# ParaGroup/WindFlow

Measured on NVIDIA H100. Metric: tuples/sec, Map_GPU->Filter_GPU->Ffat_Windows_GPU (CB win 4096 slide 64) pipeline, higher is better.
Workload: dtype i64+f64

## Files before the change

### windflow_b200/csrc/wfb_kernels.cuh

```cuda
#pragma once
#include <type_traits>
#include <cstdint>
#include <cstring>
#include <cuda.h>
#include <cuda_runtime.h>
#include "wfb_ptx.cuh"
#include "wfb_keys.cuh"

namespace wfb {

template <class P> using key_codec = KeyCodec<typename P::key_t>;
template <class P> using key_words_t = typename key_codec<P>::words_t;
template <class P>
__host__ __device__ __forceinline__ key_words_t<P> key_words(const typename P::tuple_t &t, const typename P::params_t &prm)
{
    return key_codec<P>::encode(P::key(t, prm));
}

constexpr int TILE = 256;
constexpr uint32_t OSW_TILE_POS = 4096;
#ifndef WFB_STAGES
#define WFB_STAGES 4
#endif
constexpr int STAGES = WFB_STAGES;
// ... 811 lines not shown
    __shared__ uint32_t cntw[OS_THREADS / 32][256];
    __shared__ uint32_t dig_off[256];
    __shared__ uint32_t bin_base[256];
    __shared__ uint32_t wsum[OS_THREADS / 32];
    __shared__ uint32_t s_tile;
    constexpr int OS_TILE = OS_THREADS * OS_ITEMS;
    __shared__ K skeys[OS_TILE];
    __shared__ uint32_t svals[OS_TILE];

    const uint32_t tid = threadIdx.x, lane = tid & 31, warp = tid >> 5;
    const uint32_t n = n_ptr ? *n_ptr : n_host;
    const uint32_t num_tiles = (n + OS_TILE - 1) / OS_TILE;
    const uint32_t shift = base_shift + 8 * pass;
    if (tid == 0) s_tile = atomicAdd(&ctl[passes * 256 + pass], 1u);
#pragma unroll
    for (int w = 0; w < OS_THREADS / 32; w++) cntw[w][tid] = 0;
    __syncthreads();
    const uint32_t tile = s_tile;
    if (tile >= num_tiles) return;
    const uint32_t start = tile * OS_TILE;

    K k[OS_ITEMS];
    uint32_t rk[OS_ITEMS];
#pragma unroll
    for (int r = 0; r < OS_ITEMS; r++) {
        const uint32_t idx = start + warp * (32 * OS_ITEMS) + r * 32 + lane;
        const bool valid = idx < n;
        k[r] = valid ? keys_in[idx] : K(0);
        const uint32_t d = valid ? (static_cast<uint32_t>(k[r] >> shift) & 255u) : 256u;
        const uint32_t mask = __match_any_sync(FULL, d);
        rk[r] = valid ? (cntw[warp][d] + __popc(mask & lanemask_lt())) : 0u;
        __syncwarp();
        if (valid && lane == static_cast<uint32_t>(__ffs(mask) - 1)) cntw[warp][d] += __popc(mask);
        __syncwarp();
    }
    __syncthreads();

    uint32_t total = 0;
#pragma unroll
    for (int w = 0; w < OS_THREADS / 32; w++) { const uint32_t c = cntw[w][tid]; cntw[w][tid] = total; total += c; }
    uint64_t *my_state = tile_state + static_cast<size_t>(tile) * 256 + tid;
    st_relaxed_u64(my_state, pack_state(epoch, tile == 0 ? ST_PREFIX : ST_AGG, total));
    const uint32_t gcount = ctl[pass * 256 + tid];
    uint32_t incl = gcount;
#pragma unroll
    for (int o = 1; o < 32; o <<= 1) { const uint32_t v = __shfl_up_sync(FULL, incl, o); if (lane >= o) incl += v; }
    if (lane == 31) wsum[warp] = incl;
    uint32_t tincl = total;
#pragma unroll
    for (int o = 1; o < 32; o <<= 1) { const uint32_t v = __shfl_up_sync(FULL, tincl, o); if (lane >= o) tincl += v; }
    __shared__ uint32_t twsum[OS_THREADS / 32];
    if (lane == 31) twsum[warp] = tincl;
    __syncthreads();
    uint32_t gbase = incl - gcount, tbase = tincl - total;
#pragma unroll
    for (uint32_t w = 0; w < OS_THREADS / 32; w++) if (w < warp) { gbase += wsum[w]; tbase += twsum[w]; }
    uint32_t excl = 0;
    if (tile > 0) {
        int64_t t2 = static_cast<int64_t>(tile) - 1;
        bool found = false;
        while (!found) {
            uint64_t w[8];
#pragma unroll
            for (int q = 0; q < 8; q++) w[q] = (t2 - q >= 0) ? ld_relaxed_u64(tile_state + static_cast<size_t>(t2 - q) * 256 + tid) : 0ull;
#pragma unroll
            for (int q = 0; q < 8; q++) {
                if (found || t2 - q < 0) continue;
                if ((w[q] >> 34) != (epoch & 0x3fffffffu) || ((w[q] >> 32) & 3u) == 0) { t2 -= q; goto next_round; }
                excl += static_cast<uint32_t>(w[q]);
                if (((w[q] >> 32) & 3u) == ST_PREFIX) found = true;
            }
            t2 -= 8;
        next_round:;
        }
        st_relaxed_u64(my_state, pack_state(epoch, ST_PREFIX, excl + total));
    }
    dig_off[tid] = tbase;
    bin_base[tid] = gbase + excl;
    __syncthreads();

#pragma unroll
    for (int r = 0; r < OS_ITEMS; r++) {
        const uint32_t idx = start + warp * (32 * OS_ITEMS) + r * 32 + lane;
        if (idx < n) {
            const uint32_t d = static_cast<uint32_t>(k[r] >> shift) & 255u;
            const uint32_t lp = dig_off[d] + cntw[warp][d] + rk[r];
            skeys[lp] = k[r];
            svals[lp] = vals_in ? vals_in[idx] : idx;
        }
    }
    __syncthreads();
    const uint32_t cnt = min(static_cast<uint32_t>(OS_TILE), n - start);
    for (uint32_t i = tid; i < cnt; i += OS_THREADS) {
        const K kk = skeys[i];
        const uint32_t d = static_cast<uint32_t>(kk >> shift) & 255u;
        const uint32_t dst = bin_base[d] + (i - dig_off[d]);
        keys_out[dst] = kk;
        vals_out[dst] = svals[i];
        if (seg_first != nullptr && static_cast<uint64_t>(kk) < seg_first_n) atomicMin(&seg_first[static_cast<uint32_t>(kk)], dst);
    }
}

template <class P>
__global__ void __launch_bounds__(256) k_slots_inplace(const TileArgs a, const typename P::params_t prm)
{
    using T = typename P::tuple_t;
    __shared__ uint32_t s_h[512];
    const uint32_t tid = threadIdx.x;
    const uint32_t npos = a.num_tiles * TILE;
    if (blockIdx.x == 0 && tid == 0 && a.ff.n_trig != nullptr) { *a.ff.n_trig = 0; *a.ff.n_heavy = 0; }
    auto slot_at = [&](uint32_t p) -> uint32_t {
        const uint32_t t = p / TILE;
        uint32_t lo = 0, hi = a.nbatches - 1;
        while (lo < hi) { const uint32_t mid = (lo + hi + 1) >> 1; if (a.batches[mid].tile_begin <= t) lo = mid; else hi = mid - 1; }
        const DevBatch &b = a.batches[lo];
        const uint32_t local = p - b.tile_begin * TILE;
        uint32_t slot = INVALID_SLOT;
        if (local < b.n) {
            if (a.ext_slots != nullptr) { slot = a.ext_slots[p]; if (slot >= a.ff.max_keys) slot = INVALID_SLOT; }
            else {
                const T *rec = reinterpret_cast<const T *>(b.tuples + static_cast<size_t>(local) * sizeof(T));
                slot = slot_of_key(a.ff, key_words<P>(*rec, prm));
            }
            if (slot != INVALID_SLOT && a.count_keys) atomicAdd(&a.ff.seg_cnt[slot], 1u);
        }
        return slot;
    };
    const uint32_t nwide = (npos + OSW_TILE_POS - 1) / OSW_TILE_POS;
    for (uint32_t wt = blockIdx.x; wt < nwide; wt += gridDim.x) {
        for (uint32_t i = tid; i < 512; i += blockDim.x) s_h[i] = 0;
        __syncthreads();
        for (uint32_t p = wt * OSW_TILE_POS + tid; p < min(npos, (wt + 1) * OSW_TILE_POS); p += blockDim.x) {
            uint32_t slot = slot_at(p);
            if (slot != INVALID_SLOT) {
                const uint32_t d = (slot >> a.sort_shift) & 1023u;
                const uint32_t before = atomicAdd(&s_h[d >> 1], 1u << ((d & 1u) * 16u));
                if (a.pack_rank) slot |= ((before >> ((d & 1u) * 16u)) & 0xffffu) << 16;
            }
            a.slots[p] = slot;
        }
        __syncthreads();
        for (uint32_t i = tid; i < 512; i += blockDim.x) reinterpret_cast<uint32_t *>(a.wide_h16 + static_cast<size_t>(wt) * 1024u)[i] = s_h[i];
        __syncthreads();
    }
}

#ifndef WFB_OSW_MINBLOCKS
#define WFB_OSW_MINBLOCKS 5
#endif
constexpr uint32_t OSW_BITS = 10, OSW_DIGITS = 1u << OSW_BITS;
constexpr uint32_t OSW_THREADS = 256, OSW_ITEMS = 16, OSW_TILE = OSW_THREADS * OSW_ITEMS;
static_assert(OSW_TILE == OSW_TILE_POS, "the tile pass files its digit counts per wide tile");
constexpr uint32_t OSR_GROUP = 4, OSR_GROUP_POS = OSR_GROUP * OSW_TILE;

template <class K>
__global__ void __launch_bounds__(OSW_THREADS) k_wide_tile_hist(const K *__restrict__ keys, const uint32_t *__restrict__ n_ptr, uint32_t n_host,
                                                                uint32_t shift, uint32_t chunk_shift, uint16_t *__restrict__ H,
                                                                uint32_t *__restrict__ C, uint32_t *__restrict__ ctl_counts, uint32_t skip_invalid)
{
    static_assert(OSW_THREADS * 4 == OSW_DIGITS, "four digits per thread");
    __shared__ __align__(16) uint32_t h[OSW_DIGITS];
    const uint32_t tid = threadIdx.x, tile = blockIdx.x;
    const uint32_t n = n_ptr ? *n_ptr : n_host;
    const uint32_t start = tile * OSW_TILE;
    if (start >= n) return;
    reinterpret_cast<uint4 *>(h)[tid] = make_uint4(0, 0, 0, 0);
    __syncthreads();
#pragma unroll
    for (uint32_t r = 0; r < OSW_ITEMS; r++) {
        const uint32_t idx = start + r * OSW_THREADS + tid;
        if (idx < n) { const K kk = keys[idx]; if (!(skip_invalid && kk == static_cast<K>(~K(0)))) atomicAdd(&h[static_cast<uint32_t>(kk >> shift) & (OSW_DIGITS - 1u)], 1u); }
    }
    __syncthreads();
    const uint4 c = reinterpret_cast<const uint4 *>(h)[tid];
    reinterpret_cast<ushort4 *>(H + static_cast<size_t>(tile) * OSW_DIGITS)[tid] =
        make_ushort4(static_cast<uint16_t>(c.x), static_cast<uint16_t>(c.y), static_cast<uint16_t>(c.z), static_cast<uint16_t>(c.w));
    uint32_t *crow = C + static_cast<size_t>(tile >> chunk_shift) * OSW_DIGITS + tid * 4;
    if (c.x) atomicAdd(crow + 0, c.x);
    if (c.y) atomicAdd(crow + 1, c.y);
    if (c.z) atomicAdd(crow + 2, c.z);
    if (c.w) atomicAdd(crow + 3, c.w);
    if (ctl_counts != nullptr) {
        if (c.x) atomicAdd(ctl_counts + tid * 4 + 0, c.x);
        if (c.y) atomicAdd(ctl_counts + tid * 4 + 1, c.y);
        if (c.z) atomicAdd(ctl_counts + tid * 4 + 2, c.z);
        if (c.w) atomicAdd(ctl_counts + tid * 4 + 3, c.w);
    }
}

static __global__ void __launch_bounds__(OSW_THREADS) k_wide_chunk_sums16(const uint16_t *__restrict__ H, uint32_t tiles, uint32_t chunk_shift, uint32_t *__restrict__ C,
                                                                          uint32_t *__restrict__ ctl_counts = nullptr)
{
    const uint32_t chunk = blockIdx.x, tid = threadIdx.x;
    const uint32_t t0 = chunk << chunk_shift, t1 = min(tiles, t0 + (1u << chunk_shift));
    uint4 acc = make_uint4(0, 0, 0, 0);
    const ushort4 *row = reinterpret_cast<const ushort4 *>(H) + tid;
#pragma unroll 16
    for (uint32_t t = t0; t < t1; t++) { const ushort4 v = row[static_cast<size_t>(t) * (OSW_DIGITS / 4)]; acc.x += v.x; acc.y += v.y; acc.z += v.z; acc.w += v.w; }
    reinterpret_cast<uint4 *>(C + static_cast<size_t>(chunk) * OSW_DIGITS)[tid] = acc;
    if (ctl_counts != nullptr) {
        if (acc.x) atomicAdd(ctl_counts + tid * 4 + 0, acc.x);
        if (acc.y) atomicAdd(ctl_counts + tid * 4 + 1, acc.y);
        if (acc.z) atomicAdd(ctl_counts + tid * 4 + 2, acc.z);
        if (acc.w) atomicAdd(ctl_counts + tid * 4 + 3, acc.w);
    }
}

static __global__ void __launch_bounds__(OSW_THREADS) k_wide_tile_bases(const uint16_t *__restrict__ H, uint32_t tiles, uint32_t chunk_shift, uint32_t chunks,
                                                                        uint32_t *__restrict__ C, uint32_t *__restrict__ T, uint32_t *__restrict__ ctl_counts,
                                                                        uint32_t *__restrict__ done, uint32_t gshift)
{
    static_assert(OSW_THREADS * 4 == OSW_DIGITS, "four digits per thread");
    constexpr uint32_t NW = OSW_THREADS / 32;
    __shared__ uint32_t wsum[NW];
    __shared__ uint32_t s_last;
    const uint32_t chunk = blockIdx.x, tid = threadIdx.x, lane = tid & 31, warp = tid >> 5;
    const uint32_t t0 = chunk << chunk_shift, t1 = min(tiles, t0 + (1u << chunk_shift));
    uint4 acc = make_uint4(0, 0, 0, 0);
    const ushort4 *row = reinterpret_cast<const ushort4 *>(H) + tid;
    uint4 *trow = reinterpret_cast<uint4 *>(T) + tid;
#pragma unroll 8
    for (uint32_t t = t0; t < t1; t++) {
        const ushort4 v = row[static_cast<size_t>(t) * (OSW_DIGITS / 4)];
        if ((t & ((1u << gshift) - 1u)) == 0) trow[static_cast<size_t>(t >> gshift) * (OSW_DIGITS / 4)] = acc;
        acc.x += v.x; acc.y += v.y; acc.z += v.z; acc.w += v.w;
    }
    uint4 *C4 = reinterpret_cast<uint4 *>(C);
    C4[static_cast<size_t>(chunk) * (OSW_DIGITS / 4) + tid] = acc;
    __threadfence();
    __syncthreads();
    if (tid == 0) s_last = atomicAdd(done, 1u) == chunks - 1u;
    __syncthreads();
    if (!s_last) return;
    __threadfence();
    uint4 tot = make_uint4(0, 0, 0, 0);
#pragma unroll 8
    for (uint32_t c = 0; c < chunks; c++) { const uint4 v = __ldcg(C4 + static_cast<size_t>(c) * (OSW_DIGITS / 4) + tid); tot.x += v.x; tot.y += v.y; tot.z += v.z; tot.w += v.w; }
    reinterpret_cast<uint4 *>(ctl_counts)[tid] = tot;
    const uint32_t sum = tot.x + tot.y + tot.z + tot.w;
    uint32_t incl = sum;
#pragma unroll
    for (int o = 1; o < 32; o <<= 1) { const uint32_t v = __shfl_up_sync(FULL, incl, o); if (lane >= static_cast<uint32_t>(o)) incl += v; }
    if (lane == 31) wsum[warp] = incl;
    __syncthreads();
    uint32_t base = incl - sum;
#pragma unroll
    for (uint32_t q = 0; q < NW; q++) if (q < warp) base += wsum[q];
    uint4 run = make_uint4(base, base + tot.x, base + tot.x + tot.y, base + tot.x + tot.y + tot.z);
#pragma unroll 8
    for (uint32_t c = 0; c < chunks; c++) {
        uint4 *p = C4 + static_cast<size_t>(c) * (OSW_DIGITS / 4) + tid;
        const uint4 v = __ldcg(p);
        *p = run;
        run.x += v.x; run.y += v.y; run.z += v.z; run.w += v.w;
    }
    if (tid == 0) *done = 0;
}

constexpr uint32_t OSR_SMEM = OSR_GROUP_POS * 2u * 2u + OSW_DIGITS * 8u + OSW_DIGITS * 2u;
static_assert(OSR_GROUP == 4 && OSR_GROUP_POS <= 0x8000u, "one ushort4 of part sizes per digit; 16-bit packed position compare");
static __global__ void __launch_bounds__(OSW_THREADS, 3) k_wide_scatter_ranked(const uint32_t *__restrict__ packed, uint32_t *__restrict__ keys_out,
                                                                            uint32_t *__restrict__ vals_out, uint32_t n, uint32_t shift, uint32_t chunk_shift,
                                                                            uint32_t tiles, const uint16_t *__restrict__ H, const uint32_t *__restrict__ Cx,
                                                                            const uint32_t *__restrict__ T)
{
    constexpr uint32_t NW = OSW_THREADS / 32;
    static_assert(OSW_THREADS * 4 == OSW_DIGITS, "four digits per thread");
    extern __shared__ __align__(16) unsigned char osr_smem_buf[];
    uint16_t *lpos = reinterpret_cast<uint16_t *>(osr_smem_buf);
    uint16_t *lslot = lpos + OSR_GROUP_POS;
    ushort4 *part = reinterpret_cast<ushort4 *>(lslot + OSR_GROUP_POS);
    uint16_t *cell = reinterpret_cast<uint16_t *>(part + OSW_DIGITS);
    __shared__ uint32_t wsum[NW];
    __shared__ uint32_t s_total;
    const uint32_t tid = threadIdx.x, lane = tid & 31, warp = tid >> 5, group = blockIdx.x, tile0 = group * OSR_GROUP;
    const uint32_t start = tile0 * OSW_TILE;
    if (start >= n) return;
    {
        ushort4 h[OSR_GROUP];
#pragma unroll
        for (uint32_t k = 0; k < OSR_GROUP; k++)
            h[k] = tile0 + k < tiles ? reinterpret_cast<const ushort4 *>(H)[static_cast<size_t>(tile0 + k) * (OSW_DIGITS / 4) + tid] : make_ushort4(0, 0, 0, 0);
        part[4 * tid + 0] = make_ushort4(h[0].x, h[1].x, h[2].x, h[3].x);
        part[4 * tid + 1] = make_ushort4(h[0].y, h[1].y, h[2].y, h[3].y);
        part[4 * tid + 2] = make_ushort4(h[0].z, h[1].z, h[2].z, h[3].z);
        part[4 * tid + 3] = make_ushort4(h[0].w, h[1].w, h[2].w, h[3].w);
        uint32_t c0 = 0, c1 = 0, c2 = 0, c3 = 0;
#pragma unroll
        for (uint32_t k = 0; k < OSR_GROUP; k++) { c0 += h[k].x; c1 += h[k].y; c2 += h[k].z; c3 += h[k].w; }
        const uint32_t sum = c0 + c1 + c2 + c3;
        uint32_t incl = sum;
#pragma unroll
        for (int o = 1; o < 32; o <<= 1) { const uint32_t v = __shfl_up_sync(FULL, incl, o); if (lane >= static_cast<uint32_t>(o)) incl += v; }
        if (lane == 31) wsum[warp] = incl;
        __syncthreads();
        uint32_t base = incl - sum;
#pragma unroll
        for (uint32_t q = 0; q < NW; q++) if (q < warp) base += wsum[q];
        if (tid == OSW_THREADS - 1) s_total = base + sum;
        reinterpret_cast<ushort4 *>(cell)[tid] = make_ushort4(static_cast<uint16_t>(base), static_cast<uint16_t>(base + c0), static_cast<uint16_t>(base + c0 + c1),
                                                               static_cast<uint16_t>(base + c0 + c1 + c2));
    }
    __syncthreads();
    auto part_start = [&](uint32_t d, uint32_t k, uint32_t *size) {
        const ushort4 p = part[d];
        *size = k == 0 ? p.x : k == 1 ? p.y : k == 2 ? p.z : p.w;
        return (k > 0 ? p.x : 0u) + (k > 1 ? p.y : 0u) + (k > 2 ? p.z : 0u);
    };
#pragma unroll 1
    for (uint32_t k = 0; k < OSR_GROUP; k++) {
        uint32_t w[OSW_ITEMS];
#pragma unroll
        for (uint32_t r = 0; r < OSW_ITEMS; r++) {
            const uint32_t idx = start + k * OSW_TILE + r * OSW_THREADS + tid;
            w[r] = idx < n ? packed[idx] : INVALID_SLOT;
        }
#pragma unroll
        for (uint32_t r = 0; r < OSW_ITEMS; r++)
            if (w[r] != INVALID_SLOT) {
                const uint32_t slot = w[r] & 0xffffu, d = (slot >> shift) & (OSW_DIGITS - 1u);
                uint32_t size;
                const uint32_t i = cell[d] + part_start(d, k, &size) + (w[r] >> 16);
                lpos[i] = static_cast<uint16_t>(k * OSW_TILE + r * OSW_THREADS + tid);
                lslot[i] = static_cast<uint16_t>(slot);
            }
    }
    __syncthreads();
    const uint32_t total = s_total;
    const uint32_t *cbase = Cx + static_cast<size_t>(tile0 >> chunk_shift) * OSW_DIGITS, *tbase = T + static_cast<size_t>(group) * OSW_DIGITS;
#pragma unroll 2
    for (uint32_t e = tid; e < total; e += OSW_THREADS) {
        const uint32_t mine = lpos[e], slot = lslot[e], d = (slot >> shift) & (OSW_DIGITS - 1u);
        uint32_t size;
        const uint32_t before = part_start(d, mine / OSW_TILE, &size);
        uint32_t j = cell[d] + before;
        const uint32_t end = j + size;
        uint32_t less = 0;
        if (j & 1u) { less += lpos[j] < mine ? 1u : 0u; j++; }
        const uint32_t mm = (mine | (mine << 16)) + 0x7fff7fffu;
        for (; j + 1 < end; j += 2) less += __popc((mm - *reinterpret_cast<const uint32_t *>(lpos + j)) & 0x80008000u);
        if (j < end) less += lpos[j] < mine ? 1u : 0u;
        const uint32_t dst = __ldg(cbase + d) + __ldg(tbase + d) + before + less;
        keys_out[dst] = slot;
        vals_out[dst] = start + mine;
    }
}

#ifndef WFB_OSR_MINBLOCKS
#define WFB_OSR_MINBLOCKS 6
#endif
template <int RBYTES>
static __global__ void __launch_bounds__(OSW_THREADS, WFB_OSR_MINBLOCKS) k_wide_scatter_ranked_tile(const uint32_t *__restrict__ packed, uint32_t *__restrict__ keys_out,
                                                                            uint32_t *__restrict__ vals_out, uint32_t n, uint32_t shift, uint32_t chunk_shift,
                                                                            const uint16_t *__restrict__ H, const uint32_t *__restrict__ Cx, const uint32_t *__restrict__ T,
                                                                            const unsigned char *__restrict__ payload_in, unsigned char *__restrict__ payload_out)
{
    constexpr uint32_t NW = OSW_THREADS / 32;
    constexpr uint32_t LPOS = OSW_TILE + OSW_DIGITS;
    constexpr uint32_t LPAD = 0x0fffu;
    static_assert(OSW_TILE <= 4096 && LPOS % (2 * OSW_THREADS) == 0, "16-bit packed position compare");
    __shared__ __align__(16) uint32_t sw[OSW_TILE];
    __shared__ __align__(16) uint32_t bin_base[OSW_DIGITS];
    __shared__ __align__(8) uint16_t cnt_row[OSW_DIGITS], cell_start[OSW_DIGITS];
    __shared__ __align__(4) uint16_t lpos[LPOS];
    __shared__ uint32_t wsum[NW];
    const uint32_t tid = threadIdx.x, lane = tid & 31, warp = tid >> 5, tile = blockIdx.x;
    const uint32_t start = tile * OSW_TILE;
    if (start >= n) return;
#pragma unroll
    for (uint32_t r = 0; r < OSW_ITEMS; r++) {
        const uint32_t i = r * OSW_THREADS + tid, idx = start + i;
        const uint32_t w = idx < n ? packed[idx] : INVALID_SLOT;
        sw[i] = w;
        if constexpr (RBYTES != 0)
            if (w != INVALID_SLOT) asm volatile("prefetch.global.L2 [%0];" ::"l"(payload_in + static_cast<size_t>(idx) * RBYTES));
    }
    {
        const uint4 cb = reinterpret_cast<const uint4 *>(Cx)[static_cast<size_t>(tile >> chunk_shift) * (OSW_DIGITS / 4) + tid];
        const uint4 tb = reinterpret_cast<const uint4 *>(T)[static_cast<size_t>(tile) * (OSW_DIGITS / 4) + tid];
        reinterpret_cast<uint4 *>(bin_base)[tid] = make_uint4(cb.x + tb.x, cb.y + tb.y, cb.z + tb.z, cb.w + tb.w);
        const ushort4 c = reinterpret_cast<const ushort4 *>(H)[static_cast<size_t>(tile) * (OSW_DIGITS / 4) + tid];
        reinterpret_cast<ushort4 *>(cnt_row)[tid] = c;
        const uint32_t p0 = (c.x + 1u) & ~1u, p1 = (c.y + 1u) & ~1u, p2 = (c.z + 1u) & ~1u, p3 = (c.w + 1u) & ~1u;
        const uint32_t sum = p0 + p1 + p2 + p3;
        uint32_t incl = sum;
#pragma unroll
        for (int o = 1; o < 32; o <<= 1) { const uint32_t v = __shfl_up_sync(FULL, incl, o); if (lane >= static_cast<uint32_t>(o)) incl += v; }
        if (lane == 31) wsum[warp] = incl;
#pragma unroll
        for (uint32_t i = 0; i < LPOS / (2 * OSW_THREADS); i++) reinterpret_cast<uint32_t *>(lpos)[i * OSW_THREADS + tid] = LPAD | (LPAD << 16);
        __syncthreads();
        uint32_t base = incl - sum;
#pragma unroll
        for (uint32_t q = 0; q < NW; q++) if (q < warp) base += wsum[q];
        reinterpret_cast<ushort4 *>(cell_start)[tid] = make_ushort4(static_cast<uint16_t>(base), static_cast<uint16_t>(base + p0), static_cast<uint16_t>(base + p0 + p1),
                                                                     static_cast<uint16_t>(base + p0 + p1 + p2));
    }
    __syncthreads();
#pragma unroll
    for (uint32_t r = 0; r < OSW_ITEMS; r++) {
        const uint32_t i = r * OSW_THREADS + tid, w = sw[i];
        if (w != INVALID_SLOT) lpos[cell_start[((w & 0xffffu) >> shift) & (OSW_DIGITS - 1u)] + (w >> 16)] = static_cast<uint16_t>(i);
    }
    __syncthreads();
#pragma unroll 2
    for (uint32_t e = tid; e < LPOS; e += OSW_THREADS) {
        const uint32_t mine = lpos[e], w = sw[mine];
        if (w == INVALID_SLOT) continue;
        const uint32_t slot = w & 0xffffu, d = (slot >> shift) & (OSW_DIGITS - 1u);
        const uint32_t cs = cell_start[d], cnt = cnt_row[d];
        if (e - cs >= cnt) continue;
        const uint32_t mm = (mine | (mine << 16)) + 0x7fff7fffu;
        const uint32_t *cell = reinterpret_cast<const uint32_t *>(lpos + cs);
        uint32_t less = 0;
        for (uint32_t j = 0; j < cnt; j += 2) less += __popc((mm - cell[j >> 1]) & 0x80008000u);
        const uint32_t dst = bin_base[d] + less;
        keys_out[dst] = slot;
        if (RBYTES == 0 || vals_out != nullptr) vals_out[dst] = start + mine;
        if constexpr (RBYTES != 0) {
            static_assert(RBYTES % 8 == 0, "record size");
            using W = typename std::conditional<RBYTES % 16 == 0, uint4, uint2>::type;
            const W *src = reinterpret_cast<const W *>(payload_in + static_cast<size_t>(start + mine) * RBYTES);
            W *dstp = reinterpret_cast<W *>(payload_out + static_cast<size_t>(dst) * RBYTES);
            W v[RBYTES / sizeof(W)];
#pragma unroll
            for (uint32_t q = 0; q < RBYTES / sizeof(W); q++) v[q] = src[q];
#pragma unroll
            for (uint32_t q = 0; q < RBYTES / sizeof(W); q++) dstp[q] = v[q];
        }
    }
}

static __global__ void k_shard_bin_counts(const uint32_t *__restrict__ bin_counts, uint32_t nshards, uint32_t bps, uint32_t *__restrict__ counts_out,
                                          uint64_t *__restrict__ send_meta, uint64_t watermark)
{
    const uint32_t d = threadIdx.x >> 5, lane = threadIdx.x & 31;
    uint32_t c = 0;
    if (d < nshards) for (uint32_t b = lane; b < bps; b += 32) c += bin_counts[d * bps + b];
#pragma unroll
    for (int o = 16; o > 0; o >>= 1) c += __shfl_xor_sync(FULL, c, o);
    if (lane == 0 && d < MAX_SHARDS) counts_out[d] = d < nshards ? c : 0u;
    if (lane == 0 && d < nshards && send_meta != nullptr) { send_meta[2 * d] = c; send_meta[2 * d + 1] = watermark; }
}

struct MgRuns { uint32_t off[MAX_SHARDS + 1]; };
constexpr uint32_t MG_THREADS = 256;
__device__ __forceinline__ uint32_t mg_run_start(const uint32_t *__restrict__ cnt, uint32_t s, uint32_t bps, uint32_t b, uint32_t *sh)
{
    uint32_t c = 0;
    for (uint32_t q = threadIdx.x; q < b; q += MG_THREADS) c += cnt[s * bps + q];
#pragma unroll
    for (int o = 16; o > 0; o >>= 1) c += __shfl_xor_sync(FULL, c, o);
    if ((threadIdx.x & 31) == 0) sh[threadIdx.x >> 5] = c;
    __syncthreads();
    uint32_t t = 0;
#pragma unroll
    for (uint32_t w = 0; w < MG_THREADS / 32; w++) t += sh[w];
    __syncthreads();
    return t;
}
static __global__ void __launch_bounds__(MG_THREADS) k_mg_count(const uint32_t *__restrict__ cnt, uint32_t nsrc, uint32_t bps, const MgRuns runs,
                                                                const uint32_t *__restrict__ recv_slots, uint32_t slot_mask, uint32_t shift2, uint32_t nsub,
                                                                uint32_t *__restrict__ cnt3, uint32_t *__restrict__ run_starts,
                                                                uint32_t *__restrict__ n_trig, uint32_t *__restrict__ n_heavy)
{
    __shared__ uint32_t sh[8], c[MAX_SHARDS];
    const uint32_t b = blockIdx.x, s = blockIdx.y, tid = threadIdx.x, lane = tid & 31;
    if (b == 0 && s == 0 && tid == 0) { *n_trig = 0; *n_heavy = 0; }
    if (tid < MAX_SHARDS) c[tid] = 0;
    const uint32_t rs = mg_run_start(cnt, s, bps, b, sh), m = cnt[s * bps + b];
    if (tid == 0) run_starts[s * bps + b] = rs;
    const uint32_t *sl = recv_slots + runs.off[s] + rs;
    for (uint32_t i0 = 0; i0 < m; i0 += MG_THREADS) {
        const uint32_t i = i0 + tid;
        const uint32_t j = i < m ? ((sl[i] & slot_mask) >> shift2) & (nsub - 1u) : nsub;
        for (uint32_t jj = 0; jj < nsub; jj++) { const uint32_t bal = __ballot_sync(FULL, j == jj); if (lane == 0 && bal) atomicAdd(&c[jj], __popc(bal)); }
    }
    __syncthreads();
    if (tid < nsub) cnt3[(b * nsub + tid) * nsrc + s] = c[tid];
}
static __global__ void __launch_bounds__(1024) k_mg_scan(const uint32_t *__restrict__ cnt3, uint32_t n, uint32_t nsrc, uint32_t *__restrict__ off3,
                                                         uint32_t *__restrict__ digit_counts)
{
    __shared__ uint32_t wsum[32];
    const uint32_t tid = threadIdx.x, lane = tid & 31, warp = tid >> 5;
    const uint32_t per = (n + 1023u) / 1024u, lo = tid * per;
    uint32_t v[MAX_SHARDS], sum = 0;
#pragma unroll
    for (uint32_t q = 0; q < MAX_SHARDS; q++) { v[q] = (q < per && lo + q < n) ? cnt3[lo + q] : 0u; sum += v[q]; }
    uint32_t incl = sum;
#pragma unroll
    for (int o = 1; o < 32; o <<= 1) { const uint32_t x = __shfl_up_sync(FULL, incl, o); if (lane >= static_cast<uint32_t>(o)) incl += x; }
    if (lane == 31) wsum[warp] = incl;
    __syncthreads();
    if (warp == 0) {
        uint32_t w = wsum[lane], wi = w;
#pragma unroll
        for (int o = 1; o < 32; o <<= 1) { const uint32_t x = __shfl_up_sync(FULL, wi, o); if (lane >= static_cast<uint32_t>(o)) wi += x; }
        wsum[lane] = wi - w;
    }
    __syncthreads();
    uint32_t run = wsum[warp] + incl - sum;
#pragma unroll
    for (uint32_t q = 0; q < MAX_SHARDS; q++) if (q < per && lo + q < n) { off3[lo + q] = run; run += v[q]; }
    for (uint32_t d = tid; d * nsrc < n; d += 1024) { uint32_t t = 0; for (uint32_t q = 0; q < nsrc; q++) t += cnt3[d * nsrc + q]; digit_counts[d] = t; }
}
static __global__ void __launch_bounds__(MG_THREADS) k_mg_split(const uint32_t *__restrict__ cnt, uint32_t nsrc, uint32_t bps, const MgRuns runs,
                                                                const uint32_t *__restrict__ recv_slots, uint32_t slot_mask, uint32_t shift2, uint32_t nsub,
                                                                const uint32_t *__restrict__ off3, const uint32_t *__restrict__ run_starts,
                                                                uint32_t *__restrict__ out_slots, uint32_t *__restrict__ out_pos)
{
    __shared__ uint32_t wc[MG_THREADS / 32][MAX_SHARDS], fill[MAX_SHARDS];
    const uint32_t b = blockIdx.x, s = blockIdx.y, tid = threadIdx.x, lane = tid & 31, warp = tid >> 5;
    const uint32_t m = cnt[s * bps + b], src0 = runs.off[s] + run_starts[s * bps + b];
    if (tid < nsub) fill[tid] = off3[(b * nsub + tid) * nsrc + s];
    __syncthreads();
    for (uint32_t i0 = 0; i0 < m; i0 += MG_THREADS) {
        const uint32_t i = i0 + tid;
        uint32_t slot = 0, j = nsub, before = 0;
        if (i < m) { slot = recv_slots[src0 + i] & slot_mask; j = (slot >> shift2) & (nsub - 1u); }
        for (uint32_t jj = 0; jj < nsub; jj++) {
            const uint32_t bal = __ballot_sync(FULL, j == jj);
            if (lane == 0) wc[warp][jj] = __popc(bal);
            if (j == jj) before = __popc(bal & lanemask_lt());
        }
        __syncthreads();
        if (i < m) {
            uint32_t dst = fill[j] + before;
            for (uint32_t w = 0; w < warp; w++) dst += wc[w][j];
            out_slots[dst] = slot; out_pos[dst] = src0 + i;
        }
        __syncthreads();
        if (tid < nsub) { uint32_t t = 0; for (uint32_t w = 0; w < MG_THREADS / 32; w++) t += wc[w][tid]; fill[tid] += t; }
        __syncthreads();
    }
}

template <class K, int RBYTES>
__global__ void __launch_bounds__(OSW_THREADS, WFB_OSW_MINBLOCKS) k_wide_scatter(const K *__restrict__ keys_in, K *__restrict__ keys_out, uint32_t *__restrict__ vals_out,
                                                              const uint32_t *__restrict__ n_ptr, uint32_t n_host, uint32_t shift,
                                                              uint32_t chunk_shift, const uint16_t *__restrict__ H, const uint32_t *__restrict__ C,
                                                              const uint32_t *__restrict__ ctl_counts,
                                                              const unsigned char *__restrict__ payload_in, unsigned char *__restrict__ payload_out,
                                                              uint32_t payload_bytes, uint32_t skip_invalid, uint32_t region_stride)
{
    constexpr uint32_t NW = OSW_THREADS / 32;
    __shared__ __align__(16) uint16_t cntw[NW][OSW_DIGITS];
    __shared__ uint32_t bin_base[OSW_DIGITS];
    __shared__ uint32_t wsum[NW];
    const uint32_t tid = threadIdx.x, lane = tid & 31, warp = tid >> 5, tile = blockIdx.x;
    const uint32_t n = n_ptr ? *n_ptr : n_host;
    const uint32_t start = tile * OSW_TILE;
    if (start >= n) return;
    {
        uint4 *z = reinterpret_cast<uint4 *>(&cntw[0][0]);
        for (uint32_t i = tid; i < NW * OSW_DIGITS / 8; i += OSW_THREADS) z[i] = make_uint4(0, 0, 0, 0);
    }
    uint32_t acc[4] = {0, 0, 0, 0};
    {
        const uint32_t chunk = tile >> chunk_shift;
        const uint4 *crow = reinterpret_cast<const uint4 *>(C) + tid;
#pragma unroll 8
        for (uint32_t c = 0; c < chunk; c++) { const uint4 v = crow[static_cast<size_t>(c) * (OSW_DIGITS / 4)]; acc[0] += v.x; acc[1] += v.y; acc[2] += v.z; acc[3] += v.w; }
        const ushort4 *hrow = reinterpret_cast<const ushort4 *>(H) + tid;
#pragma unroll 16
        for (uint32_t t = chunk << chunk_shift; t < tile; t++) { const ushort4 v = hrow[static_cast<size_t>(t) * (OSW_DIGITS / 4)]; acc[0] += v.x; acc[1] += v.y; acc[2] += v.z; acc[3] += v.w; }
    }
    const uint4 g4 = reinterpret_cast<const uint4 *>(ctl_counts)[tid];
    const uint32_t gsum = g4.x + g4.y + g4.z + g4.w;
    uint32_t incl = gsum;
#pragma unroll
    for (int o = 1; o < 32; o <<= 1) { const uint32_t v = __shfl_up_sync(FULL, incl, o); if (lane >= static_cast<uint32_t>(o)) incl += v; }
    if (lane == 31) wsum[warp] = incl;
    __syncthreads();

    K k[OSW_ITEMS];
    uint32_t rk[OSW_ITEMS];
#pragma unroll
    for (uint32_t r = 0; r < OSW_ITEMS; r++) {
        const uint32_t idx = start + warp * (32 * OSW_ITEMS) + r * 32 + lane;
        k[r] = idx < n ? keys_in[idx] : K(0);
    }
#pragma unroll
    for (uint32_t r = 0; r < OSW_ITEMS; r++) {
        const uint32_t idx = start + warp * (32 * OSW_ITEMS) + r * 32 + lane;
        const bool valid = idx < n && !(skip_invalid && k[r] == static_cast<K>(~K(0)));
        rk[r] = 0xffffffffu;
        if (!__any_sync(FULL, valid)) continue;
        const uint32_t d = valid ? (static_cast<uint32_t>(k[r] >> shift) & (OSW_DIGITS - 1u)) : OSW_DIGITS + lane;
        const uint32_t mask = __match_any_sync(FULL, d);
        const uint32_t leader = static_cast<uint32_t>(__ffs(mask) - 1);
        uint32_t before = 0;
        if (valid && lane == leader) { before = cntw[warp][d]; cntw[warp][d] = static_cast<uint16_t>(before + __popc(mask)); }
        before = __shfl_sync(FULL, before, leader);
        if (valid) rk[r] = before + __popc(mask & lanemask_lt());
        __syncwarp();
    }
    __syncthreads();
    {
        uint32_t gb = incl - gsum;
#pragma unroll
        for (uint32_t w = 0; w < NW; w++) if (w < warp) gb += wsum[w];
        uint32_t run[4] = {0, 0, 0, 0};
#pragma unroll
        for (uint32_t w = 0; w < NW; w++) {
            ushort4 *row = reinterpret_cast<ushort4 *>(&cntw[w][0]);
            const ushort4 c = row[tid];
            row[tid] = make_ushort4(static_cast<uint16_t>(run[0]), static_cast<uint16_t>(run[1]), static_cast<uint16_t>(run[2]), static_cast<uint16_t>(run[3]));
            run[0] += c.x; run[1] += c.y; run[2] += c.z; run[3] += c.w;
        }
        const uint32_t gc[4] = {g4.x, g4.y, g4.z, g4.w};
#pragma unroll
        for (int q = 0; q < 4; q++) { bin_base[tid * 4 + q] = (region_stride ? (tid * 4 + q) * region_stride : gb) + acc[q]; gb += gc[q]; }
    }
    __syncthreads();
#pragma unroll
    for (uint32_t r = 0; r < OSW_ITEMS; r++) {
        const uint32_t idx = start + warp * (32 * OSW_ITEMS) + r * 32 + lane;
        if (rk[r] != 0xffffffffu) {
            const uint32_t d = static_cast<uint32_t>(k[r] >> shift) & (OSW_DIGITS - 1u);
            const uint32_t dst = bin_base[d] + cntw[warp][d] + rk[r];
            if (region_stride && dst - d * region_stride >= region_stride) { rk[r] = 0xffffffffu; continue; }
            if (keys_out != nullptr) keys_out[dst] = k[r];
            if (vals_out != nullptr) vals_out[dst] = idx;
            rk[r] = dst;
        }
    }
    if constexpr (RBYTES > 0) {
        using V = typename std::conditional<RBYTES % 16 == 0, uint4, uint2>::type;
        constexpr uint32_t NV = RBYTES / sizeof(V);
#pragma unroll
        for (uint32_t r = 0; r < OSW_ITEMS; r++) {
            const uint32_t idx = start + warp * (32 * OSW_ITEMS) + r * 32 + lane;
            if (rk[r] != 0xffffffffu) {
                const V *src = reinterpret_cast<const V *>(payload_in + static_cast<size_t>(idx) * RBYTES);
                V *dstp = reinterpret_cast<V *>(payload_out + static_cast<size_t>(rk[r]) * RBYTES);
                V tmp[NV];
#pragma unroll
                for (uint32_t q = 0; q < NV; q++) tmp[q] = src[q];
#pragma unroll
                for (uint32_t q = 0; q < NV; q++) dstp[q] = tmp[q];
            }
        }
    } else if constexpr (RBYTES < 0) {
#pragma unroll 1
        for (uint32_t r = 0; r < OSW_ITEMS; r++) {
            const uint32_t idx = start + warp * (32 * OSW_ITEMS) + r * 32 + lane;
            if (rk[r] != 0xffffffffu) {
                const uint64_t *src = reinterpret_cast<const uint64_t *>(payload_in + static_cast<size_t>(idx) * payload_bytes);
                uint64_t *dstp = reinterpret_cast<uint64_t *>(payload_out + static_cast<size_t>(rk[r]) * payload_bytes);
                for (uint32_t q = 0; q < payload_bytes / 8; q++) dstp[q] = src[q];
            }
        }
    }
}

template <int RBYTES>
__global__ void __launch_bounds__(OSW_THREADS) k_shard_scatter(const uint32_t *__restrict__ dest, uint32_t n, uint32_t nbins, uint32_t chunk_shift,
                                                               const uint16_t *__restrict__ H, const uint32_t *__restrict__ C,
                                                               const unsigned char *__restrict__ payload_in, unsigned char *__restrict__ payload_out,
                                                               uint32_t region_stride)
{
    constexpr uint32_t NW = OSW_THREADS / 32;
    __shared__ uint32_t base[32];
    __shared__ uint32_t wtot[NW][32];
    const uint32_t tid = threadIdx.x, lane = tid & 31, warp = tid >> 5, tile = blockIdx.x;
    const uint32_t start = tile * OSW_TILE;
    if (start >= n) return;
    if (tid < 32) {
        uint32_t acc = 0;
        if (tid < nbins) {
            const uint32_t chunk = tile >> chunk_shift;
            for (uint32_t c = 0; c < chunk; c++) acc += C[static_cast<size_t>(c) * OSW_DIGITS + tid];
            for (uint32_t t = chunk << chunk_shift; t < tile; t++) acc += H[static_cast<size_t>(t) * OSW_DIGITS + tid];
        }
        base[tid] = tid * region_stride + acc;
    }
    uint32_t running = 0;
    uint16_t code[OSW_ITEMS];
#pragma unroll
    for (uint32_t r = 0; r < OSW_ITEMS; r++) {
        const uint32_t idx = start + warp * (32 * OSW_ITEMS) + r * 32 + lane;
        const uint32_t d = idx < n ? dest[idx] : INVALID_SLOT;
// ... 75 lines not shown
    if (d < MAX_SHARDS) counts_out[d] = c;
    const uint32_t over = __ballot_sync(FULL, c > region_cap);
    if (d == 0) counts_out[MAX_SHARDS] = over ? 1u : 0u;
}


__device__ __forceinline__ uint32_t level_off(uint32_t n_leaves, uint32_t level);
__device__ __forceinline__ uint64_t batch_watermark(const uint32_t *__restrict__ batch_off, const DevBatch *__restrict__ batches,
                                                    uint32_t nbatches, uint32_t pos);
template <class P>
__device__ __forceinline__ void ffat_eval_window(const FfatDev &ff, const unsigned char *tree, key_words_t<P> key, uint64_t gwid, uint64_t wm,
                                                 uint32_t opos, unsigned char *__restrict__ out_res, uint64_t *__restrict__ out_ts,
                                                 uint32_t out_cap, const typename P::params_t &prm);

template <class P>
__global__ void __launch_bounds__(128) k_ffat_update_lanes(const FfatDev ff, const unsigned char *__restrict__ lifted,
                                                           const uint32_t *__restrict__ sorted_pos,
                                                           const uint32_t *__restrict__ batch_off, const DevBatch *__restrict__ batches,
                                                           uint32_t nbatches, unsigned char *__restrict__ out_res,
                                                           uint64_t *__restrict__ out_ts, uint32_t out_cap, uint32_t *__restrict__ n_out,
                                                           const typename P::params_t prm)
{
    using R = typename P::result_t;
    constexpr uint32_t RB = sizeof(R);
    constexpr uint32_t U = 4;
    const uint32_t nslots = ff.dense ? ff.max_keys : min(*ff.n_slots, ff.max_keys);
    const uint32_t n = ff.n_leaves, logn = ff.log_leaves;
    const uint64_t P_ = ff.pane;
    const uint64_t group_items = ff.slide * ff.nb;
    const size_t tree_stride = static_cast<size_t>(2 * n - 1) * RB;

    for (uint32_t base = blockIdx.x * blockDim.x; base < nslots; base += gridDim.x * blockDim.x) {
        const uint32_t slot = base + threadIdx.x;
        uint32_t m = (slot < nslots) ? ff.seg_cnt[slot] : 0u;
        if (m > ff.light_max) {
            const uint32_t hi = atomicAdd(ff.n_heavy, 1u);
            if (hi < ff.max_keys) ff.heavy[hi] = slot;
            m = 0;
        }
        const bool act = m > 0;
        uint32_t off = 0; uint64_t c = 0, g = 0, trig = 0;
        key_words_t<P> key{};
        alignas(16) R acc;
        unsigned char *tree = ff.tree + static_cast<size_t>(slot) * tree_stride;
        if (act) {
            off = ff.seg_off[slot]; c = ff.cnt[slot];
            key = key_of_slot<P>(ff, slot);
            if (c % P_ != 0) ld_rec<R>(ff.acc + static_cast<size_t>(slot) * RB, acc);
            g = (c < ff.B) ? 0 : 1 + (c - ff.B) / group_items;
            trig = ff.B + g * group_items;
        }
        uint32_t j = 0;
        while (__any_sync(FULL, act && j < m)) {
            bool completed = false;
            while (act && j < m && !completed) {
                uint32_t p[U];
                alignas(16) R it[U];
                const uint32_t k = min(U, m - j);
#pragma unroll
                for (uint32_t q = 0; q < U; q++) if (q < k) p[q] = sorted_pos[off + j + q];
#pragma unroll
                for (uint32_t q = 0; q < U; q++) if (q < k) ld_rec<R>(lifted + static_cast<size_t>(p[q]) * RB, it[q]);
#pragma unroll
                for (uint32_t q = 0; q < U; q++) {
                    if (q < k && !completed) {
                        if (c % P_ == 0) acc = it[q]; else P::comb(acc, it[q], acc, prm);
                        c++; j++;
                        completed = (c % P_ == 0);
                    }
                }
            }
            if (completed) {
                const uint32_t leaf = static_cast<uint32_t>((c / P_ - 1) & (n - 1));
                const uint32_t plev = ff.lazy ? 0u : logn;
                for (uint32_t l = 0; l < plev; l++)
                    asm volatile("prefetch.global.L2 [%0];" ::"l"(tree + static_cast<size_t>(level_off(n, l) + ((leaf >> l) ^ 1u)) * RB));
                alignas(16) R cur = acc;
                st_rec<R>(tree + static_cast<size_t>(leaf) * RB, cur);
                for (uint32_t l = 0; l < plev; l++) {
                    alignas(16) R s;
                    ld_rec<R>(tree + static_cast<size_t>(level_off(n, l) + ((leaf >> l) ^ 1u)) * RB, s);
                    alignas(16) R parent = cur;
                    if ((leaf >> l) & 1u) P::comb(s, cur, parent, prm); else P::comb(cur, s, parent, prm);
                    cur = parent;
                    st_rec<R>(tree + static_cast<size_t>(level_off(n, l + 1) + (leaf >> (l + 1))) * RB, cur);
                }
                if (c == trig) {
                    const uint32_t last_pos = sorted_pos[off + j - 1];
                    const uint32_t obase = atomicAdd(n_out, ff.nb);
                    bool deferred = (m - j) < ff.defer_items;
                    if (deferred) {
                        const uint32_t ti = atomicAdd(ff.n_trig, 1u);
                        if (ti < ff.trig_cap) { Trigger tr; tr.key = trig_word(key); tr.g = g; tr.slot = slot; tr.last_pos = last_pos; tr.obase = obase; tr.pad = 0; ff.trig[ti] = tr; }
                        else deferred = false;
                    }
                    if (!deferred) {
                        const uint64_t wm = batch_watermark(batch_off, batches, nbatches, last_pos);
                        for (uint32_t i = 0; i < ff.nb; i++)
                            ffat_eval_window<P>(ff, tree, key, g * ff.nb + i, wm, obase + i, out_res, out_ts, out_cap, prm);
                    }
                    g++; trig += group_items;
                }
            }
        }
        if (act) {
            ff.cnt[slot] = c;
            if (c % P_ != 0) st_rec<R>(ff.acc + static_cast<size_t>(slot) * RB, acc);
            ff.seg_cnt[slot] = 0;
            ff.seg_off[slot] = 0xffffffffu;
        }
    }
}

#ifdef WFB_BK_TRACE
__device__ unsigned long long g_bk_trace[1024 * 8];
__device__ __forceinline__ unsigned long long bk_now() { unsigned long long t; asm volatile("mov.u64 %0, %%globaltimer;" : "=l"(t)); return t; }
#define BK_TRACE_STATE unsigned long long bk_t = 0
#define BK_MARK(i) do { if (threadIdx.x == 0) { const unsigned long long t_ = bk_now(); unsigned long long *r_ = g_bk_trace + blockIdx.x * 8; \
    if ((i) == 0) { r_[0] = t_; for (int q_ = 1; q_ < 8; q_++) r_[q_] = 0; } else if ((i) == 7) r_[7] = t_; else r_[i] += t_ - bk_t; bk_t = t_; } } while (0)
#else
#define BK_TRACE_STATE do { } while (0)
#define BK_MARK(i) do { } while (0)
#endif
constexpr uint32_t BK_KEYS = 64;
constexpr uint32_t BK_THREADS = 128;
#ifndef WFB_BK_REC_BYTES
#define WFB_BK_REC_BYTES 16384
#endif
constexpr uint32_t BK_REC_BYTES = WFB_BK_REC_BYTES;
constexpr uint32_t BK_CNT_U = 16;
__device__ __forceinline__ uint32_t bk_opaque(uint32_t v) { asm volatile("" : "+r"(v)); return v; }
template <uint32_t RB>
constexpr uint32_t bk_items_per_thread() { return BK_REC_BYTES / (BK_THREADS * RB) < 1 ? 1 : (BK_REC_BYTES / (BK_THREADS * RB) > 8 ? 8 : BK_REC_BYTES / (BK_THREADS * RB)); }
template <uint32_t RB>
constexpr uint32_t bk_sibl_levels() { return RB <= 32 ? 8 : (RB <= 48 ? 4 : (RB <= 128 ? 2 : 1)); }
template <uint32_t RB, bool LAZY>
constexpr uint32_t bk_smem_bytes()
{
    constexpr uint32_t IT = bk_items_per_thread<RB>(), CAP = BK_THREADS * IT, CS = IT * (BK_THREADS / 32) + 2;
    return CAP * RB + 3 * CAP * 4 + BK_KEYS * CS * 2 + 5 * BK_KEYS * 4 + 3 * BK_KEYS * 8 + BK_KEYS * RB
         + (LAZY ? 16 : BK_KEYS * bk_sibl_levels<RB>() * RB) + 2 * BK_KEYS * 4 + BK_THREADS * 4 + (BK_THREADS / 32 + 5) * 4 + 64;
}
template <uint32_t RB>
constexpr bool bk_fits() { return bk_smem_bytes<RB, false>() <= (48u << 10) && bk_smem_bytes<RB, true>() <= (48u << 10); }
#ifndef WFB_BK_MINBLOCKS
#define WFB_BK_MINBLOCKS 4
#endif
#ifndef WFB_BK_MINBLOCKS_LAZY
#define WFB_BK_MINBLOCKS_LAZY 4
#endif

template <class P, bool LAZY>
__global__ void __launch_bounds__(BK_THREADS, LAZY ? WFB_BK_MINBLOCKS_LAZY : WFB_BK_MINBLOCKS) k_ffat_update_buckets(const FfatDev ff, const unsigned char *__restrict__ lifted,
                                                                       const uint32_t *__restrict__ bk_slots, const uint32_t *__restrict__ bk_pos,
                                                                       const uint32_t *__restrict__ digit_counts, uint32_t shift, uint32_t moved,
                                                                       const uint32_t *__restrict__ batch_off, const DevBatch *__restrict__ batches,
                                                                       uint32_t nbatches, unsigned char *__restrict__ out_res,
                                                                       uint64_t *__restrict__ out_ts, uint32_t out_cap, uint32_t *__restrict__ n_out,
                                                                       const typename P::params_t prm)
{
    using R = typename P::result_t;
    constexpr uint32_t RB = sizeof(R);
    constexpr uint32_t NW = BK_THREADS / 32;
    constexpr uint32_t DPT = OSW_DIGITS / BK_THREADS;
    constexpr uint32_t IT = bk_items_per_thread<RB>();
    constexpr uint32_t CAP = BK_THREADS * IT;
    constexpr uint32_t NCOL = IT * NW;
    constexpr uint32_t CS = NCOL + 2;
    constexpr uint32_t CPB = (RB % 16 == 0) ? 16 : 8;
    constexpr uint32_t BK_SIBL = bk_sibl_levels<RB>();
    static_assert(DPT % 4 == 0 && BK_KEYS == 64 && BK_THREADS == 128 && RB % 8 == 0, "layout");
    static_assert(bk_fits<RB>(), "the arrays below exceed 48 KB of static shared memory (bk_smem_bytes)");
    __shared__ __align__(16) unsigned char s_rec[CAP * RB];
    __shared__ uint32_t s_idx[CAP];
    __shared__ uint32_t s_lslot[CAP], s_lpos[CAP];
    __shared__ __align__(16) uint16_t s_col[BK_KEYS][CS];
    __shared__ uint32_t kcnt[BK_KEYS], koff[BK_KEYS];
    __shared__ uint32_t kleft[BK_KEYS];
    __shared__ uint32_t kcp[BK_KEYS], kleaf[BK_KEYS];
    __shared__ uint64_t kc[BK_KEYS], kg[BK_KEYS], ktt[BK_KEYS];
    __shared__ __align__(16) unsigned char kacc[BK_KEYS * RB];
    __shared__ __align__(16) unsigned char s_sib[LAZY ? 16 : BK_KEYS * BK_SIBL * RB];
    __shared__ uint32_t s_heavy[BK_KEYS];
    __shared__ uint32_t ksegb[BK_KEYS];
    __shared__ uint32_t seg_desc[BK_THREADS];
    __shared__ uint32_t misc[NW], s_boff[2], s_nheavy, s_hnext, s_nseg;

    const uint32_t tid = threadIdx.x, lane = tid & 31, warp = tid >> 5;
    const uint32_t bucket = blockIdx.x;
    const uint32_t kpc = min(BK_KEYS, 1u << shift);
    const uint32_t key_lo = bucket << shift;
    const uint32_t n = ff.n_leaves, logn = ff.log_leaves;
    const uint32_t P32 = static_cast<uint32_t>(ff.pane);
    const uint64_t group_items = ff.slide * ff.nb;
    const size_t tree_stride = static_cast<size_t>(2 * n - 1) * RB;
    BK_TRACE_STATE;

    BK_MARK(0);
    uint32_t my_total = 0;
    uint64_t st_c = 0;
    const bool has_key = tid < kpc && key_lo + tid < ff.max_keys;
    if (has_key) {
        const uint32_t slot = key_lo + tid;
        st_c = ff.cnt[slot];
#pragma unroll
        for (uint32_t q = 0; q < RB / CPB; q++) cp_async<CPB>(kacc + tid * RB + q * CPB, ff.acc + static_cast<size_t>(slot) * RB + q * CPB);
    }
    if (tid < BK_KEYS) kleft[tid] = 0;
    {
        uint32_t cc[DPT];
#pragma unroll
        for (uint32_t q = 0; q < DPT / 4; q++) {
            const uint4 v = reinterpret_cast<const uint4 *>(digit_counts)[tid * (DPT / 4) + q];
            cc[4 * q] = v.x; cc[4 * q + 1] = v.y; cc[4 * q + 2] = v.z; cc[4 * q + 3] = v.w;
        }
        uint32_t sum = 0;
#pragma unroll
        for (uint32_t q = 0; q < DPT; q++) sum += cc[q];
        uint32_t incl = sum;
#pragma unroll
        for (int o = 1; o < 32; o <<= 1) { const uint32_t v = __shfl_up_sync(FULL, incl, o); if (lane >= static_cast<uint32_t>(o)) incl += v; }
        if (lane == 31) misc[warp] = incl;
        __syncthreads();
        if (tid == bucket / DPT) {
            uint32_t base = incl - sum;
            for (uint32_t w = 0; w < warp; w++) base += misc[w];
            for (uint32_t q = bucket - bucket % DPT; q < bucket; q++) base += digit_counts[q];
            s_boff[0] = base; s_boff[1] = base + digit_counts[bucket];
        }
        __syncthreads();
    }
    const uint32_t bbeg = s_boff[0], bend = s_boff[1];
    const auto fetch_list = [&](uint32_t at, uint32_t end) {
#pragma unroll
        for (uint32_t r = 0; r < IT; r++) {
            const uint32_t i = r * BK_THREADS + tid;
            if (at + i < end) {
                cp_async<4>(s_lslot + i, bk_slots + at + i);
                if (!moved) cp_async<4>(s_lpos + i, bk_pos + at + i);
            }
        }
    };
    fetch_list(bbeg, bend);
    for (uint32_t base = bbeg; base < bend; base += BK_CNT_U * BK_THREADS) {
        uint32_t lk[BK_CNT_U];
#pragma unroll
        for (uint32_t q = 0; q < BK_CNT_U; q++) {
            const uint32_t i = base + q * BK_THREADS + tid;
            lk[q] = i < bend ? bk_slots[i] - key_lo : 0xffffffffu;
        }
#pragma unroll
        for (uint32_t q = 0; q < BK_CNT_U; q++) if (lk[q] < kpc) atomicAdd(&kleft[lk[q]], 1u);
    }
    __syncthreads();
    if (tid < BK_KEYS) {
        const uint32_t m = has_key ? kleft[tid] : 0u;
        my_total = m;
        const uint64_t c = st_c;
        uint64_t g = 0, tt = 0; uint32_t cp = 0, leaf = 0;
        if (m) {
            cp = static_cast<uint32_t>(c % P32); leaf = static_cast<uint32_t>((c / P32) & (n - 1));
            if (c < ff.B) { g = 0; tt = ff.B - c; }
            else { g = 1 + (c - ff.B) / group_items; tt = ff.B + g * group_items - c; }
        }
        kleft[tid] = m; kc[tid] = c; kg[tid] = g; ktt[tid] = tt; kcp[tid] = cp; kleaf[tid] = leaf;
    }
    const uint32_t any_items = __syncthreads_or(my_total != 0);
    BK_MARK(1);
    if (!any_items) { cp_async_wait_all(); BK_MARK(7); return; }
    if (moved)
        for (size_t o = static_cast<size_t>(tid) * 128; o < static_cast<size_t>(bend - bbeg) * RB; o += BK_THREADS * 128)
            asm volatile("prefetch.global.L2 [%0];" ::"l"(lifted + static_cast<size_t>(bbeg) * RB + o));

    for (uint32_t cursor = s_boff[0]; cursor < s_boff[1]; cursor = s_boff[0]) {
        const uint32_t nsel = min(CAP, s_boff[1] - cursor);
        uint32_t ek[IT], ep[IT];
        cp_async_wait_all();
#pragma unroll
        for (uint32_t r = 0; r < IT; r++) {
            const uint32_t i = r * BK_THREADS + tid;
            ek[r] = BK_KEYS; ep[r] = cursor + i;
            if (i < nsel) {
                const uint32_t lk = s_lslot[i] - key_lo;
                if (!moved) ep[r] = s_lpos[i];
                if (lk < kpc) ek[r] = lk;
            }
        }
        {
            uint32_t *z = reinterpret_cast<uint32_t *>(&s_col[0][0]);
            for (uint32_t i = tid; i < BK_KEYS * CS / 2; i += BK_THREADS) z[i] = 0;
        }
        __syncthreads();
        fetch_list(cursor + CAP, s_boff[1]);
#pragma unroll
        for (uint32_t r = 0; r < IT; r++) {
            const uint32_t k = ek[r];
            const uint32_t peers = __match_any_sync(FULL, k);
            const uint32_t rank = __popc(peers & lanemask_lt());
            if (k < BK_KEYS && rank == 0) s_col[k][r * NW + warp] = static_cast<uint16_t>(__popc(peers));
            ek[r] = k | rank << 8;
        }
        __syncthreads();
        BK_MARK(2);
        if (warp == 0) {
            uint32_t a0 = 0, a1 = 0;
#pragma unroll
            for (uint32_t c = 0; c < NCOL; c++) {
                const uint32_t v0 = s_col[lane][c], v1 = s_col[lane + 32][c];
                s_col[lane][c] = static_cast<uint16_t>(a0); s_col[lane + 32][c] = static_cast<uint16_t>(a1);
                a0 += v0; a1 += v1;
            }
            uint32_t i0 = a0, i1 = a1;
#pragma unroll
            for (int o = 1; o < 32; o <<= 1) {
                const uint32_t v0 = __shfl_up_sync(FULL, i0, o), v1 = __shfl_up_sync(FULL, i1, o);
                if (lane >= static_cast<uint32_t>(o)) { i0 += v0; i1 += v1; }
            }
            const uint32_t t0 = __shfl_sync(FULL, i0, 31);
            kcnt[lane] = a0; kcnt[lane + 32] = a1;
            koff[lane] = i0 - a0; koff[lane + 32] = t0 + i1 - a1;
            const uint32_t c0 = kcp[lane], c1 = kcp[lane + 32];
            const uint32_t f0 = min(a0, P32 - c0), f1 = min(a1, P32 - c1);
            const uint32_t n0 = a0 ? 1u + (a0 - f0 + P32 - 1) / P32 : 0u, n1 = a1 ? 1u + (a1 - f1 + P32 - 1) / P32 : 0u;
            uint32_t s0 = n0, s1 = n1;
#pragma unroll
            for (int o = 1; o < 32; o <<= 1) {
                const uint32_t v0 = __shfl_up_sync(FULL, s0, o), v1 = __shfl_up_sync(FULL, s1, o);
                if (lane >= static_cast<uint32_t>(o)) { s0 += v0; s1 += v1; }
            }
            const uint32_t st0 = __shfl_sync(FULL, s0, 31), nseg = st0 + __shfl_sync(FULL, s1, 31);
            ksegb[lane] = s0 - n0; ksegb[lane + 32] = st0 + s1 - n1;
            const bool fallback = nseg > BK_THREADS;
            const bool h0 = fallback && a0 != 0, h1 = fallback && a1 != 0;
            const uint32_t b0 = __ballot_sync(FULL, h0), b1 = __ballot_sync(FULL, h1);
            if (h0) s_heavy[__popc(b0 & lanemask_lt())] = lane;
            if (h1) s_heavy[__popc(b0) + __popc(b1 & lanemask_lt())] = lane + 32;
            if (lane == 0) { s_nheavy = __popc(b0) + __popc(b1); s_hnext = 0; s_nseg = fallback ? 0u : nseg; }
        }
        __syncthreads();
#pragma unroll
        for (uint32_t r = 0; r < IT; r++) {
            const uint32_t k = ek[r] & 255u;
            if (k < BK_KEYS) {
                const uint32_t at = koff[k] + s_col[k][r * NW + warp] + (ek[r] >> 8);
                s_idx[at] = ep[r];
                const unsigned char *src = lifted + static_cast<size_t>(ep[r]) * RB;
#pragma unroll
                for (uint32_t q = 0; q < RB / CPB; q++) {
                    if constexpr (CPB == 16) cp_async_cg16(s_rec + at * RB + q * CPB, src + q * CPB);
                    else cp_async<CPB>(s_rec + at * RB + q * CPB, src + q * CPB);
                }
            }
        }
        const uint32_t nseg = s_nseg;
        bool sib_staged = false;
        if (tid < BK_KEYS && nseg != 0) {
            const uint32_t m = kcnt[tid];
            if (m != 0) {
                const uint32_t cp0 = kcp[tid], first = min(m, P32 - cp0), ns = 1u + (m - first + P32 - 1) / P32, sb = ksegb[tid];
                for (uint32_t j = 0; j < ns; j++) seg_desc[sb + j] = tid | (j << 8);
                if (!LAZY && cp0 + first == P32) {
                    const uint32_t leaf = kleaf[tid];
                    const unsigned char *tr = ff.tree + static_cast<size_t>(key_lo + tid) * tree_stride;
                    for (uint32_t l = 0; l < min(logn, BK_SIBL); l++) {
                        const unsigned char *src = tr + static_cast<size_t>(level_off(n, l) + ((leaf >> l) ^ 1u)) * RB;
                        unsigned char *dst = s_sib + (tid * BK_SIBL + l) * RB;
#pragma unroll
                        for (uint32_t q = 0; q < RB / CPB; q++) cp_async<CPB>(dst + q * CPB, src + q * CPB);
                    }
                    sib_staged = true;
                }
            }
        }
        cp_async_wait_all();
        __syncthreads();
        BK_MARK(3);
        if (tid < nseg) {
            const uint32_t d = seg_desc[tid], k = d & 255u, j = d >> 8;
            const uint32_t m = kcnt[k], cp0 = kcp[k], first = min(m, P32 - cp0);
            const uint32_t start = j == 0 ? 0u : first + (j - 1) * P32;
            const uint32_t seg = j == 0 ? first : min(P32, m - start);
            unsigned char *rp = s_rec + (koff[k] + start) * RB;
            alignas(16) R acc;
            uint32_t i = 1;
            if (j == 0 && cp0 != 0) { ld_rec<R>(kacc + k * RB, acc); i = 0; }
            else ld_rec<R>(rp, acc);
#pragma unroll 4
            for (; i < seg; i++) { alignas(16) R it; ld_rec<R>(rp + i * RB, it); P::comb(acc, it, acc, prm); }
            st_rec<R>(rp, acc);
        }
        __syncthreads();
        BK_MARK(4);
        if (tid < BK_KEYS && nseg != 0) {
            const uint32_t k = bk_opaque(tid), m = kcnt[k];
            const uint32_t cp0 = kcp[k];
            uint32_t leafi = kleaf[k], new_cp = cp0, consumed = 0;
            uint64_t g = kg[k], tt = ktt[k];
            while (__any_sync(FULL, consumed < m)) {
                bool eval_now = false;
                uint32_t ev_obase = 0, ev_pos = 0;
                uint64_t ev_g = 0;
                if (consumed < m) {
                    const uint32_t open = consumed == 0 ? cp0 : 0u;
                    const uint32_t len = min(m - consumed, P32 - open);
                    alignas(16) R cur;
                    ld_rec<R>(s_rec + (koff[k] + consumed) * RB, cur);
                    consumed += len;
                    const bool completes = open + len == P32;
                    if (!completes) { st_rec<R>(kacc + k * RB, cur); new_cp = open + len; }
                    else {
                        new_cp = 0;
                        const uint32_t slot = key_lo + k, leaf = leafi;
                        unsigned char *tree = ff.tree + static_cast<size_t>(slot) * tree_stride;
                        leafi = (leafi + 1) & (n - 1);
                        st_rec<R>(tree + static_cast<size_t>(leaf) * RB, cur);
                        for (uint32_t l0 = 0; l0 < (LAZY ? 0u : logn); l0 += 4) {
                            alignas(16) R sbl[4];
#pragma unroll
                            for (uint32_t q = 0; q < 4; q++) {
                                const uint32_t l = l0 + q;
                                if (l < logn) {
                                    if (sib_staged && l < BK_SIBL) ld_rec<R>(s_sib + (k * BK_SIBL + l) * RB, sbl[q]);
                                    else ld_rec<R>(tree + static_cast<size_t>(level_off(n, l) + ((leaf >> l) ^ 1u)) * RB, sbl[q]);
                                }
                            }
#pragma unroll
                            for (uint32_t q = 0; q < 4; q++) {
                                const uint32_t l = l0 + q;
                                if (l < logn) {
                                    alignas(16) R parent = cur;
                                    if ((leaf >> l) & 1u) P::comb(sbl[q], cur, parent, prm); else P::comb(cur, sbl[q], parent, prm);
                                    cur = parent;
                                    st_rec<R>(tree + static_cast<size_t>(level_off(n, l + 1) + (leaf >> (l + 1))) * RB, cur);
                                }
                            }
                        }
                        sib_staged = false;
                        if (consumed == tt) {
                            const uint32_t lp = s_idx[koff[k] + consumed - 1];
                            const uint32_t last_pos = moved ? bk_pos[lp] : lp;
                            const uint32_t obase = atomicAdd(n_out, ff.nb);
                            bool deferred = (kleft[k] - consumed) < ff.defer_items;
                            if (deferred) {
                                const uint32_t ti = atomicAdd(ff.n_trig, 1u);
                                if (ti < ff.trig_cap) { Trigger tr; tr.key = trig_word(key_of_slot<P>(ff, slot)); tr.g = g; tr.slot = slot; tr.last_pos = last_pos; tr.obase = obase; tr.pad = 0; ff.trig[ti] = tr; }
                                else deferred = false;
                            }
                            if (!deferred) { eval_now = true; ev_obase = obase; ev_pos = last_pos; ev_g = g; }
                            g++; tt += group_items;
                        }
                    }
                }
                uint32_t pend = __ballot_sync(FULL, eval_now);
                while (pend) {
                    const int src = __ffs(pend) - 1;
                    pend &= pend - 1;
                    const uint32_t e_slot = key_lo + (warp << 5) + src, e_obase = __shfl_sync(FULL, ev_obase, src), e_pos = __shfl_sync(FULL, ev_pos, src);
                    const key_words_t<P> e_key = key_of_slot<P>(ff, e_slot);
                    const uint64_t e_g = __shfl_sync(FULL, ev_g, src);
                    const unsigned char *e_tree = ff.tree + static_cast<size_t>(e_slot) * tree_stride;
                    const uint64_t wm = batch_watermark(batch_off, batches, nbatches, e_pos);
                    for (uint32_t i = lane; i < ff.nb; i += 32)
                        ffat_eval_window<P>(ff, e_tree, e_key, e_g * ff.nb + i, wm, e_obase + i, out_res, out_ts, out_cap, prm);
                }
                __syncwarp();
            }
            if (m != 0) { kc[k] += m; kg[k] = g; ktt[k] = tt - m; kcp[k] = new_cp; kleaf[k] = leafi; kleft[k] -= m; }
        }
        BK_MARK(5);
        if (s_nheavy != 0) {
            __syncthreads();
            for (;;) {
                uint32_t h = 0;
                if (lane == 0) h = atomicAdd(&s_hnext, 1u);
                h = __shfl_sync(FULL, h, 0);
                if (h >= s_nheavy) break;
                const uint32_t k = s_heavy[h];
                const uint32_t m = kcnt[k], off = koff[k], slot = key_lo + k;
                uint64_t g = kg[k], tt = ktt[k];
                uint32_t cp = kcp[k], leafi = kleaf[k], left = kleft[k];
                unsigned char *tree = ff.tree + static_cast<size_t>(slot) * tree_stride;
                alignas(16) R acc;
                if (cp) ld_rec<R>(kacc + k * RB, acc);
                uint32_t j = 0;
                while (j < m) {
                    const uint32_t cnt = min(32u, m - j);
                    alignas(16) R cur_rec;
                    if (lane < cnt) ld_rec<R>(s_rec + (off + j + lane) * RB, cur_rec);
                    uint32_t lo = 0;
                    while (lo < cnt) {
                        const uint32_t hi = min(cnt, lo + (P32 - cp));
                        alignas(16) R r = cur_rec;
#pragma unroll
                        for (uint32_t o = 1; o < 32; o <<= 1) {
                            const R other = shfl_down_rec<R>(r, o);
                            if (lane >= lo && lane + o < hi) P::comb(r, other, r, prm);
                        }
                        r = shfl_rec<R>(r, lo);
                        if (cp == 0) acc = r; else P::comb(acc, r, acc, prm);
                        const uint32_t take = hi - lo;
                        cp += take; left -= take; tt -= take;
                        if (cp == P32) {
                            cp = 0;
                            const uint32_t leaf = leafi;
                            leafi = (leafi + 1) & (n - 1);
                            alignas(16) R sib;
                            const uint32_t plev = LAZY ? 0u : logn;
                            if (lane < plev) ld_rec<R>(tree + static_cast<size_t>(level_off(n, lane) + ((leaf >> lane) ^ 1u)) * RB, sib);
                            alignas(16) R cur = acc;
                            if (lane == 0) st_rec<R>(tree + static_cast<size_t>(leaf) * RB, cur);
                            for (uint32_t l = 0; l < plev; l++) {
                                const R sb = shfl_rec<R>(sib, l);
                                alignas(16) R parent = cur;
                                if ((leaf >> l) & 1u) P::comb(sb, cur, parent, prm); else P::comb(cur, sb, parent, prm);
                                cur = parent;
                                if (lane == 0) st_rec<R>(tree + static_cast<size_t>(level_off(n, l + 1) + (leaf >> (l + 1))) * RB, cur);
                            }
                            __syncwarp();
                            if (tt == 0) {
                                const uint32_t last_pos = moved ? bk_pos[s_idx[off + j + hi - 1]] : s_idx[off + j + hi - 1];
                                uint32_t obase = 0;
                                if (lane == 0) obase = atomicAdd(n_out, ff.nb);
                                obase = __shfl_sync(FULL, obase, 0);
                                bool deferred = left < ff.defer_items;
                                if (deferred) {
                                    uint32_t ti = 0;
                                    if (lane == 0) ti = atomicAdd(ff.n_trig, 1u);
                                    ti = __shfl_sync(FULL, ti, 0);
                                    if (ti < ff.trig_cap) {
                                        if (lane == 0) { Trigger tr; tr.key = trig_word(key_of_slot<P>(ff, slot)); tr.g = g; tr.slot = slot; tr.last_pos = last_pos; tr.obase = obase; tr.pad = 0; ff.trig[ti] = tr; }
                                    } else deferred = false;
                                }
                                if (!deferred) {
                                    const uint64_t wm = batch_watermark(batch_off, batches, nbatches, last_pos);
                                    const key_words_t<P> key = key_of_slot<P>(ff, slot);
                                    for (uint32_t i = lane; i < ff.nb; i += 32)
                                        ffat_eval_window<P>(ff, tree, key, g * ff.nb + i, wm, obase + i, out_res, out_ts, out_cap, prm);
                                }
                                g++; tt = group_items;
                                __syncwarp();
                            }
                        }
                        lo = hi;
                    }
                    j += cnt;
                }
                if (lane == 0) {
                    kc[k] += m; kg[k] = g; ktt[k] = tt; kcp[k] = cp; kleaf[k] = leafi; kleft[k] = left;
                    if (cp) st_rec<R>(kacc + k * RB, acc);
                }
            }
        }
        if (tid == 0) s_boff[0] += CAP;
        __syncthreads();
        BK_MARK(6);
    }
    if (tid < kpc && key_lo + tid < ff.max_keys) {
        const uint32_t k = bk_opaque(tid), slot = key_lo + k;
        ff.cnt[slot] = kc[k];
        if (kcp[k]) { alignas(16) R a; ld_rec<R>(kacc + k * RB, a); st_rec<R>(ff.acc + static_cast<size_t>(slot) * RB, a); }
    }
    BK_MARK(7);
}

__device__ __forceinline__ uint32_t level_off(uint32_t n_leaves, uint32_t level) { return 2u * n_leaves - ((2u * n_leaves) >> level); }

__device__ __forceinline__ uint64_t batch_watermark(const uint32_t *__restrict__ batch_off, const DevBatch *__restrict__ batches,
                                                    uint32_t nbatches, uint32_t pos)
{
    uint32_t lo = 0, hi = nbatches - 1;
    while (lo < hi) { const uint32_t mid = (lo + hi + 1) >> 1; if (batch_off[mid] <= pos) lo = mid; else hi = mid - 1; }
    return batches[lo].watermark;
}

template <class P>
__device__ __forceinline__ void ffat_eval_window(const FfatDev &ff, const unsigned char *tree, key_words_t<P> key, uint64_t gwid, uint64_t wm,
                                                 uint32_t opos, unsigned char *__restrict__ out_res, uint64_t *__restrict__ out_ts,
                                                 uint32_t out_cap, const typename P::params_t &prm)
{
    using R = typename P::result_t;
    constexpr uint32_t RB = sizeof(R);
    const uint32_t n = ff.n_leaves;
    alignas(16) R res = P::make_result(key_codec<P>::decode(key), gwid, prm);
    uint32_t ws = static_cast<uint32_t>((gwid * ff.sp) & (n - 1));
    uint32_t remaining = ff.wp;
    if (ff.lazy) {
        for (; remaining > 0; remaining--) {
            alignas(16) R node;
            ld_rec<R>(tree + static_cast<size_t>(ws) * RB, node);
            P::comb(res, node, res, prm);
            ws = (ws + 1) & (n - 1);
        }
    }
    while (remaining > 0) {
        uint32_t range = (ws == 0) ? n : (ws & (0u - ws));
        const uint32_t pw = 1u << (31 - __clz(remaining));
        range = min(range, pw);
        const uint32_t level = 31 - __clz(range);
        alignas(16) R node;
        ld_rec<R>(tree + static_cast<size_t>(level_off(n, level) + (ws >> level)) * RB, node);
        P::comb(res, node, res, prm);
        ws = (ws + range) & (n - 1);
        remaining -= range;
    }
    if (opos < out_cap) {
        st_rec<R>(out_res + static_cast<size_t>(opos) * RB, res);
        if (out_ts != nullptr) out_ts[opos] = wm;
    } else atomicOr(ff.err_flags, 2u);
}

template <class P>
__global__ void __launch_bounds__(256) k_ffat_windows(const FfatDev ff, const uint32_t *__restrict__ batch_off,
                                                      const DevBatch *__restrict__ batches, uint32_t nbatches,
                                                      unsigned char *__restrict__ out_res, uint64_t *__restrict__ out_ts, uint32_t out_cap,
                                                      const typename P::params_t prm, uint32_t *__restrict__ n_out)
{
    using R = typename P::result_t;
    if (blockIdx.x == 0 && threadIdx.x == 0 && n_out != nullptr) {
        if (*n_out > out_cap) { *n_out = out_cap; atomicOr(ff.err_flags, 2u); }
        if (ff.results_total != nullptr) *ff.results_total += *n_out;
    }
    const uint32_t nt = min(*ff.n_trig, ff.trig_cap);
    const uint64_t total = static_cast<uint64_t>(nt) * ff.nb;
    const size_t tree_stride = static_cast<size_t>(2 * ff.n_leaves - 1) * sizeof(R);
    for (uint64_t w = blockIdx.x * static_cast<uint64_t>(blockDim.x) + threadIdx.x; w < total; w += static_cast<uint64_t>(gridDim.x) * blockDim.x) {
        const uint32_t ti = static_cast<uint32_t>(w / ff.nb), i = static_cast<uint32_t>(w % ff.nb);
        const Trigger tr = ff.trig[ti];
        const uint64_t wm = batch_watermark(batch_off, batches, nbatches, tr.last_pos);
        ffat_eval_window<P>(ff, ff.tree + static_cast<size_t>(tr.slot) * tree_stride, trig_key<P>(ff, tr), tr.g * ff.nb + i, wm, tr.obase + i,
                            out_res, out_ts, out_cap, prm);
    }
}

template <class P>
__global__ void __launch_bounds__(128) k_ffat_windows_lazy(const FfatDev ff, const uint32_t *__restrict__ batch_off,
                                                           const DevBatch *__restrict__ batches, uint32_t nbatches,
                                                           unsigned char *__restrict__ out_res, uint64_t *__restrict__ out_ts, uint32_t out_cap,
                                                           const typename P::params_t prm, uint32_t *__restrict__ n_out)
{
    using R = typename P::result_t;
    constexpr uint32_t RB = sizeof(R);
    extern __shared__ __align__(16) unsigned char lazy_smem[];
    if (blockIdx.x == 0 && threadIdx.x == 0 && n_out != nullptr) {
        if (*n_out > out_cap) { *n_out = out_cap; atomicOr(ff.err_flags, 2u); }
        if (ff.results_total != nullptr) *ff.results_total += *n_out;
    }
    const uint32_t lane = threadIdx.x & 31, warp = threadIdx.x >> 5, wpb = blockDim.x >> 5;
    const uint32_t n = ff.n_leaves, logn = ff.log_leaves;
    unsigned char *t = lazy_smem + static_cast<size_t>(warp) * 2u * n * RB;
    const uint32_t nt = min(*ff.n_trig, ff.trig_cap);
    const size_t tree_stride = static_cast<size_t>(2 * n - 1) * RB;
    FfatDev fs = ff; fs.lazy = 0;
    for (uint32_t ti = blockIdx.x * wpb + warp; ti < nt; ti += gridDim.x * wpb) {
        const Trigger tr = ff.trig[ti];
        const unsigned char *leaves = ff.tree + static_cast<size_t>(tr.slot) * tree_stride;
        for (uint32_t i = lane; i < n * (RB / 8); i += 32) reinterpret_cast<uint64_t *>(t)[i] = reinterpret_cast<const uint64_t *>(leaves)[i];
        __syncwarp();
        for (uint32_t l = 0; l < logn; l++) {
            const unsigned char *src = t + static_cast<size_t>(level_off(n, l)) * RB;
            unsigned char *dst = t + static_cast<size_t>(level_off(n, l + 1)) * RB;
            for (uint32_t i = lane; i < (n >> (l + 1)); i += 32) {
                alignas(16) R a, b, o;
                ld_rec<R>(src + static_cast<size_t>(2 * i) * RB, a); ld_rec<R>(src + static_cast<size_t>(2 * i + 1) * RB, b);
                o = a;
                P::comb(a, b, o, prm);
                st_rec<R>(dst + static_cast<size_t>(i) * RB, o);
            }
            __syncwarp();
        }
        const uint64_t wm = batch_watermark(batch_off, batches, nbatches, tr.last_pos);
        for (uint32_t i = lane; i < ff.nb; i += 32)
            ffat_eval_window<P>(fs, t, trig_key<P>(ff, tr), tr.g * ff.nb + i, wm, tr.obase + i, out_res, out_ts, out_cap, prm);
        __syncwarp();
// ... 972 lines not shown
```

### windflow_b200/csrc/wfb_launch.cuh

```cuda
#pragma once
#include <type_traits>
#include <algorithm>
#include <cstring>
#include <cuda.h>
#include <cuda_runtime.h>
#include "../../include/wfb200.h"
#include "wfb_kernels.cuh"

#define WFB_CK(call) do { cudaError_t e__ = (call); if (e__ != cudaSuccess) return static_cast<int>(e__); } while (0)

namespace wfb {

inline int num_sms()
{
    static int n = 0;
    if (n == 0) { int dev = 0; if (cudaGetDevice(&dev) == cudaSuccess) cudaDeviceGetAttribute(&n, cudaDevAttrMultiProcessorCount, dev); }
    return n;
}


typedef CUresult (*PFN_encodeTiled)(CUtensorMap *, CUtensorMapDataType, cuuint32_t, void *, const cuuint64_t *, const cuuint64_t *,
                                    const cuuint32_t *, const cuuint32_t *, CUtensorMapInterleave, CUtensorMapSwizzle,
                                    CUtensorMapL2promotion, CUtensorMapFloatOOBfill);
inline PFN_encodeTiled get_encode_tiled()
{
    static PFN_encodeTiled fn = nullptr;
    static bool tried = false;
    if (!tried) {
        tried = true;
        void *p = nullptr;
        cudaDriverEntryPointQueryResult q;
        if (cudaGetDriverEntryPoint("cuTensorMapEncodeTiled", &p, cudaEnableDefault, &q) == cudaSuccess && q == cudaDriverEntryPointSuccess)
            fn = reinterpret_cast<PFN_encodeTiled>(p);
        cudaGetLastError();
    }
    return fn;
}

inline bool make_tuple_tmap(CUtensorMap *m, uint64_t base, uint64_t end)
{
    std::memset(m, 0, sizeof(*m));
    PFN_encodeTiled enc = get_encode_tiled();
    if (!enc || (base & 63u) || end <= base) return false;
    const uint64_t rows = (end - base) / 64;
    if (rows == 0 || rows > 0xffffffffull) return false;
    cuuint64_t gdim[2] = {64, rows};
    cuuint64_t gstr[1] = {64};
    cuuint32_t box[2] = {64, TILE};
    cuuint32_t estr[2] = {1, 1};
    return enc(m, CU_TENSOR_MAP_DATA_TYPE_UINT8, 2, reinterpret_cast<void *>(base), gdim, gstr, box, estr, CU_TENSOR_MAP_INTERLEAVE_NONE,
               CU_TENSOR_MAP_SWIZZLE_64B, CU_TENSOR_MAP_L2_PROMOTION_L2_128B, CU_TENSOR_MAP_FLOAT_OOB_FILL_NONE) == CUDA_SUCCESS;
}

struct ProgramOps {
    uint32_t tuple_bytes, result_bytes, params_bytes, reserved;
    int (*tile_pass)(int mode, TileArgs &a, const void *params, uint32_t want_grid, cudaStream_t s, uint32_t *grid_used,
                     uint64_t span_begin, uint64_t span_end);
    int (*ffat_update)(const FfatDev &ff, const unsigned char *lifted, const uint32_t *sorted_pos, const uint32_t *batch_off,
                       const DevBatch *batches, uint32_t nbatches, unsigned char *out_res, uint64_t *out_ts,
                       uint32_t out_cap, uint32_t *n_out, uint32_t grid, cudaStream_t s, const void *params, uint32_t lanes_grid);
    int (*ffat_buckets)(const FfatDev &ff, const unsigned char *lifted, const uint32_t *bk_slots, const uint32_t *bk_pos,
                        const uint32_t *digit_counts, uint32_t shift, uint32_t moved, const uint32_t *batch_off, const DevBatch *batches,
                        uint32_t nbatches, unsigned char *out_res, uint64_t *out_ts, uint32_t out_cap, uint32_t *n_out, cudaStream_t s,
                        const void *params);
    int (*ffat_windows)(const FfatDev &ff, const uint32_t *batch_off, const DevBatch *batches, uint32_t nbatches,
                        unsigned char *out_res, uint64_t *out_ts, uint32_t out_cap, uint32_t grid, cudaStream_t s, const void *params, uint32_t *n_out);
    int (*extract_keys)(const unsigned char *tuples, uint32_t n, uint64_t *keys, uint32_t *dest, uint32_t num_shards, cudaStream_t s,
                        const void *params);
    int (*reduce_segments)(const unsigned char *tuples, const uint64_t *ts, const uint32_t *sidx, const uint32_t *seg_begin,
                           const uint32_t *n_keys, unsigned char *out_tuples, uint64_t *out_ts, uint32_t n, cudaStream_t s, const void *params);
    int (*reduce_all)(const unsigned char *tuples, const uint64_t *ts, uint32_t n, unsigned char *out_tuple, uint64_t *out_ts, cudaStream_t s,
                      const void *params);
    int (*gather)(const unsigned char *tuples, const uint64_t *ts, const uint32_t *perm, uint32_t n, unsigned char *out_tuples,
                  uint64_t *out_ts, cudaStream_t s);
    int (*tb_lift)(const unsigned char *tuples, const uint64_t *ts, uint32_t n, const FfatDev &ff, const TbDev &tb, uint64_t first_incomplete,
                   unsigned char *lifted, uint64_t *ckeys, cudaStream_t s, const void *params);
    int (*tb_reduce)(const unsigned char *lifted, const uint64_t *skeys, const uint32_t *sidx, const uint32_t *seg_begin, const uint32_t *n_segs,
                     unsigned char *part, uint32_t n, uint32_t kbits, uint32_t max_keys, cudaStream_t s, const void *params);
    int (*tb_merge)(const uint64_t *skeys, const uint32_t *seg_begin, const uint32_t *n_segs, const unsigned char *part, const FfatDev &ff,
                    const TbDev &tb, uint32_t n, cudaStream_t s, const void *params);
    int (*tb_pop_write)(const FfatDev &ff, const TbDev &tb, uint64_t first_incomplete, const uint32_t *offs, unsigned char *popped,
                        uint32_t *popped_slots, uint32_t popped_cap, uint32_t max_present, cudaStream_t s, const void *params);
    const void *(*lifted_ops)();
    int (*slots_inplace)(const TileArgs &a, const void *params, cudaStream_t s);
    uint32_t state_bytes, reserved2;
    int (*ks_slots)(const DevBatch *batches, const uint32_t *boff, uint32_t nb, uint32_t total, const FfatDev &ff, uint32_t *slots, cudaStream_t s,
                    const void *params);
    int (*ks_apply)(int filter, const FfatDev &ff, const DevBatch *batches, const uint32_t *boff, uint32_t nb, const uint32_t *bk_slots,
                    const uint32_t *bk_pos, const uint32_t *digit_counts, uint32_t shift, unsigned char *states, unsigned char *keep, cudaStream_t s,
                    const void *params);
    int (*ks_apply_runs)(int filter, const FfatDev &ff, const DevBatch *batches, const uint32_t *boff, uint32_t nb, uint32_t n,
                         const uint32_t *sorted_slots, const uint32_t *sorted_pos, unsigned char *states, unsigned char *keep, cudaStream_t s,
                         const void *params);
    int (*flag_scatter)(const unsigned char *keep, const uint32_t *tile_base, const uint32_t *boff, uint32_t nb, uint32_t n,
                        const uint32_t *rank_start, const DevBatch *batches, cudaStream_t s);
    int (*extract_keys_batches)(const DevBatch *batches, const uint32_t *boff, uint32_t nb, uint32_t total, uint32_t key_bits, uint64_t *keys,
                                cudaStream_t s, const void *params);
    int (*reduce_segments_batches)(const DevBatch *batches, const uint32_t *boff, const uint64_t *skeys, const uint32_t *sidx,
                                   const uint32_t *seg_begin, const uint32_t *first_seg, const uint32_t *n_segs, uint32_t key_bits,
                                   uint32_t total, uint32_t *long_list, uint32_t *n_long, cudaStream_t s, const void *params);
    uint32_t key_bytes, key_kind, key_size;
    int (*key_order_words)(const DevBatch *batches, const uint32_t *boff, uint32_t nb, const unsigned char *tuples, uint32_t total, uint64_t *lo,
                           uint64_t *hi, cudaStream_t s, const void *params);
    int (*flatmap)(TileArgs &a, const void *params, uint32_t want_grid, cudaStream_t s, uint32_t *grid_used, uint64_t span_begin, uint64_t span_end);
};

template <class P, class = void> struct program_passthrough : std::false_type {};
template <class P> struct program_passthrough<P, std::void_t<decltype(P::passthrough)>> : std::integral_constant<bool, P::passthrough && std::is_same<typename P::tuple_t, typename P::result_t>::value> {};

template <class P>
inline typename P::params_t load_params(const void *params)
{
    typename P::params_t prm;
    if (params) std::memcpy(&prm, params, sizeof(prm)); else std::memset(&prm, 0, sizeof(prm));
    return prm;
}

template <class P, int MODE>
int launch_tile_pass(TileArgs &a, const void *params, uint32_t want_grid, cudaStream_t s, uint32_t *grid_used,
                     uint64_t span_begin, uint64_t span_end)
{
    static_assert(TilePassSmem<P, MODE>::total <= TP_SMEM_MAX, "tuple_t / result_t too large for the tile pass: two stages of 256 records "
                  "must fit TP_SMEM_MAX (232448 bytes) of shared memory (records of up to about 430 bytes)");
    static int max_grid = -1;
    constexpr uint32_t smem = TilePassSmem<P, MODE>::total;
    if (max_grid < 0) {
        WFB_CK(cudaFuncSetAttribute(k_tile_pass<P, MODE>, cudaFuncAttributeMaxDynamicSharedMemorySize, static_cast<int>(smem)));
        int per_sm = 0;
        WFB_CK(cudaOccupancyMaxActiveBlocksPerMultiprocessor(&per_sm, k_tile_pass<P, MODE>, TP_THREADS, smem));
        if (per_sm < 1) per_sm = 1;
        max_grid = per_sm * wfb::num_sms();
    }
    uint32_t grid = std::max(1u, std::min(want_grid, static_cast<uint32_t>(max_grid)));
    if (a.max_ctas_per_sm) grid = std::max(1u, std::min(grid, a.max_ctas_per_sm * static_cast<uint32_t>(wfb::num_sms())));
    const typename P::params_t prm = load_params<P>(params);
    alignas(64) CUtensorMap tmap;
    a.use_tmap = 0; a.tmap_base = span_begin;
    if (sizeof(typename P::tuple_t) == 64 && make_tuple_tmap(&tmap, span_begin, span_end)) a.use_tmap = 1;
    else std::memset(&tmap, 0, sizeof(tmap));
    k_tile_pass<P, MODE><<<grid, TP_THREADS, smem, s>>>(tmap, a, prm);
    WFB_CK(cudaGetLastError());
    *grid_used = grid;
    return 0;
}

template <class P>
int tile_pass_dispatch(int mode, TileArgs &a, const void *params, uint32_t want_grid, cudaStream_t s, uint32_t *grid_used,
                       uint64_t span_begin, uint64_t span_end)
{
    switch (mode) {
    case MODE_MAP: return launch_tile_pass<P, MODE_MAP>(a, params, want_grid, s, grid_used, span_begin, span_end);
    case MODE_FILTER: return launch_tile_pass<P, MODE_FILTER>(a, params, want_grid, s, grid_used, span_begin, span_end);
    case MODE_INGEST: return launch_tile_pass<P, MODE_INGEST>(a, params, want_grid, s, grid_used, span_begin, span_end);
    }
    return WFB_E_BADARG;
}

template <class P>
int ffat_update_dispatch(const FfatDev &ff, const unsigned char *lifted, const uint32_t *sorted_pos, const uint32_t *batch_off,
                         const DevBatch *batches, uint32_t nbatches, unsigned char *out_res, uint64_t *out_ts,
                         uint32_t out_cap, uint32_t *n_out, uint32_t grid, cudaStream_t s, const void *params, uint32_t lanes_grid)
{
    const typename P::params_t prm = load_params<P>(params);
    k_ffat_update_lanes<P><<<lanes_grid, 128, 0, s>>>(ff, lifted, sorted_pos, batch_off, batches, nbatches, out_res, out_ts, out_cap, n_out, prm);
    k_ffat_update<P><<<std::max(1u, std::min(grid, static_cast<uint32_t>(wfb::num_sms()) * 2u)), 256, 0, s>>>(
        ff, lifted, sorted_pos, batch_off, batches, nbatches, out_res, out_ts, out_cap, n_out, prm);
    WFB_CK(cudaGetLastError());
    return 0;
}

template <class P>
int ffat_buckets_dispatch(const FfatDev &ff, const unsigned char *lifted, const uint32_t *bk_slots, const uint32_t *bk_pos,
                          const uint32_t *digit_counts, uint32_t shift, uint32_t moved, const uint32_t *batch_off, const DevBatch *batches,
                          uint32_t nbatches, unsigned char *out_res, uint64_t *out_ts, uint32_t out_cap, uint32_t *n_out, cudaStream_t s,
                          const void *params)
{
    if (ff.lazy) k_ffat_update_buckets<P, true><<<OSW_DIGITS, BK_THREADS, 0, s>>>(ff, lifted, bk_slots, bk_pos, digit_counts, shift, moved, batch_off, batches,
                                                                                 nbatches, out_res, out_ts, out_cap, n_out, load_params<P>(params));
    else k_ffat_update_buckets<P, false><<<OSW_DIGITS, BK_THREADS, 0, s>>>(ff, lifted, bk_slots, bk_pos, digit_counts, shift, moved, batch_off, batches,
                                                                          nbatches, out_res, out_ts, out_cap, n_out, load_params<P>(params));
    WFB_CK(cudaGetLastError());
    return 0;
}
template <class P>
constexpr decltype(ProgramOps::ffat_buckets) ffat_buckets_of()
{
    if constexpr (bk_fits<sizeof(typename P::result_t)>()) return &ffat_buckets_dispatch<P>; else return nullptr;
}

template <class P>
int ffat_windows_dispatch(const FfatDev &ff, const uint32_t *batch_off, const DevBatch *batches, uint32_t nbatches,
                          unsigned char *out_res, uint64_t *out_ts, uint32_t out_cap, uint32_t grid, cudaStream_t s, const void *params, uint32_t *n_out)
{
    if (ff.lazy) {
        const size_t per_warp = static_cast<size_t>(2) * ff.n_leaves * sizeof(typename P::result_t);
        const uint32_t wpb = static_cast<uint32_t>(std::max<size_t>(1, std::min<size_t>(4, (32u << 10) / per_warp)));
        k_ffat_windows_lazy<P><<<grid, 32 * wpb, wpb * per_warp, s>>>(ff, batch_off, batches, nbatches, out_res, out_ts, out_cap, load_params<P>(params), n_out);
    } else
    k_ffat_windows<P><<<grid, 256, 0, s>>>(ff, batch_off, batches, nbatches, out_res, out_ts, out_cap, load_params<P>(params), n_out);
    WFB_CK(cudaGetLastError());
    return 0;
}

inline uint32_t grid_for(uint32_t n, uint32_t per_block) { return std::max(1u, std::min((n + per_block - 1) / per_block, static_cast<uint32_t>(wfb::num_sms()) * 16u)); }

template <class P>
int extract_keys_dispatch(const unsigned char *tuples, uint32_t n, uint64_t *keys, uint32_t *dest, uint32_t num_shards, cudaStream_t s,
                          const void *params)
{
    k_extract_keys<P><<<grid_for(n, 256), 256, 0, s>>>(tuples, n, keys, dest, num_shards, load_params<P>(params));
    WFB_CK(cudaGetLastError());
    return 0;
}
template <class P>
int reduce_segments_dispatch(const unsigned char *tuples, const uint64_t *ts, const uint32_t *sidx, const uint32_t *seg_begin,
                             const uint32_t *n_keys, unsigned char *out_tuples, uint64_t *out_ts, uint32_t n, cudaStream_t s,
                             const void *params)
{
    k_reduce_segments<P><<<grid_for(n, 8), 256, 0, s>>>(tuples, ts, sidx, seg_begin, n_keys, out_tuples, out_ts, load_params<P>(params));
    WFB_CK(cudaGetLastError());
    return 0;
}
template <class P>
int slots_inplace_dispatch(const TileArgs &a, const void *params, cudaStream_t s)
{
    const uint32_t npos = a.num_tiles * TILE;
    k_slots_inplace<P><<<std::max(1u, std::min((npos + 2047u) / 2048u, static_cast<uint32_t>(wfb::num_sms()) * 8u)), 256, 0, s>>>(a, load_params<P>(params));
    WFB_CK(cudaGetLastError());
    return 0;
}

template <class P, class = void> struct program_has_state : std::false_type {};
template <class P> struct program_has_state<P, std::void_t<typename P::state_t>> : std::true_type {};

template <class P>
int ks_slots_dispatch(const DevBatch *batches, const uint32_t *boff, uint32_t nb, uint32_t total, const FfatDev &ff, uint32_t *slots, cudaStream_t s,
                      const void *params)
{
    k_ks_slots<P><<<grid_for(total, 256), 256, 0, s>>>(batches, boff, nb, total, ff, slots, load_params<P>(params));
    WFB_CK(cudaGetLastError());
    return 0;
}
template <class P>
int ks_apply_dispatch(int filter, const FfatDev &ff, const DevBatch *batches, const uint32_t *boff, uint32_t nb, const uint32_t *bk_slots,
                      const uint32_t *bk_pos, const uint32_t *digit_counts, uint32_t shift, unsigned char *states, unsigned char *keep, cudaStream_t s,
                      const void *params)
{
    if constexpr (program_has_state<P>::value) {
        if (filter) k_ks_apply<P, true><<<OSW_DIGITS, KS_THREADS, 0, s>>>(ff, batches, boff, nb, bk_slots, bk_pos, digit_counts, shift, states, keep, load_params<P>(params));
        else k_ks_apply<P, false><<<OSW_DIGITS, KS_THREADS, 0, s>>>(ff, batches, boff, nb, bk_slots, bk_pos, digit_counts, shift, states, keep, load_params<P>(params));
        WFB_CK(cudaGetLastError());
        return 0;
    } else return WFB_E_UNSUPPORTED;
}
template <class P>
int ks_apply_runs_dispatch(int filter, const FfatDev &ff, const DevBatch *batches, const uint32_t *boff, uint32_t nb, uint32_t n,
                           const uint32_t *sorted_slots, const uint32_t *sorted_pos, unsigned char *states, unsigned char *keep, cudaStream_t s,
                           const void *params)
{
    if constexpr (program_has_state<P>::value) {
        if (filter) k_ks_apply_runs<P, true><<<grid_for(n, 256), 256, 0, s>>>(ff, batches, boff, nb, n, sorted_slots, sorted_pos, states, keep, load_params<P>(params));
        else k_ks_apply_runs<P, false><<<grid_for(n, 256), 256, 0, s>>>(ff, batches, boff, nb, n, sorted_slots, sorted_pos, states, keep, load_params<P>(params));
        WFB_CK(cudaGetLastError());
        return 0;
    } else return WFB_E_UNSUPPORTED;
}
template <class P>
int flag_scatter_dispatch(const unsigned char *keep, const uint32_t *tile_base, const uint32_t *boff, uint32_t nb, uint32_t n,
                          const uint32_t *rank_start, const DevBatch *batches, cudaStream_t s)
{
    k_flag_scatter<P><<<(n + SEGT - 1) / SEGT, 256, 0, s>>>(keep, tile_base, boff, nb, n, rank_start, batches);
    WFB_CK(cudaGetLastError());
    return 0;
}
template <class P> constexpr uint32_t program_state_bytes() { if constexpr (program_has_state<P>::value) return sizeof(typename P::state_t); else return 0; }

template <class P, class = void> struct program_has_flatmap : std::false_type {};
template <class P> struct program_has_flatmap<P, std::void_t<decltype(P::flatmap(std::declval<const typename P::tuple_t &>(),
    std::declval<Shipper<typename P::result_t> &>(), std::declval<const typename P::params_t &>()))>> : std::true_type {};
template <class P>
int flatmap_dispatch(TileArgs &a, const void *params, uint32_t want_grid, cudaStream_t s, uint32_t *grid_used, uint64_t span_begin, uint64_t span_end)
{
    return launch_tile_pass<P, MODE_FLATMAP>(a, params, want_grid, s, grid_used, span_begin, span_end);
}

template <class P>
int tb_lift_dispatch(const unsigned char *tuples, const uint64_t *ts, uint32_t n, const FfatDev &ff, const TbDev &tb, uint64_t first_incomplete,
                     unsigned char *lifted, uint64_t *ckeys, cudaStream_t s, const void *params)
{
    k_tb_lift<P><<<grid_for(n, 256), 256, 0, s>>>(tuples, ts, n, ff, tb, first_incomplete, lifted, ckeys, load_params<P>(params));
    WFB_CK(cudaGetLastError());
    return 0;
}
template <class P>
int tb_reduce_dispatch(const unsigned char *lifted, const uint64_t *skeys, const uint32_t *sidx, const uint32_t *seg_begin, const uint32_t *n_segs,
                       unsigned char *part, uint32_t n, uint32_t kbits, uint32_t max_keys, cudaStream_t s, const void *params)
{
    k_tb_reduce<P><<<grid_for(n, 128), 128, 0, s>>>(lifted, skeys, sidx, seg_begin, n_segs, part, kbits, max_keys, load_params<P>(params));
    WFB_CK(cudaGetLastError());
    return 0;
}
template <class P>
int tb_merge_dispatch(const uint64_t *skeys, const uint32_t *seg_begin, const uint32_t *n_segs, const unsigned char *part, const FfatDev &ff,
                      const TbDev &tb, uint32_t n, cudaStream_t s, const void *params)
{
    k_tb_merge<P><<<grid_for(n, 128), 128, 0, s>>>(skeys, seg_begin, n_segs, part, ff, tb, load_params<P>(params));
    WFB_CK(cudaGetLastError());
    return 0;
}
template <class P>
int tb_pop_write_dispatch(const FfatDev &ff, const TbDev &tb, uint64_t first_incomplete, const uint32_t *offs, unsigned char *popped,
                          uint32_t *popped_slots, uint32_t popped_cap, uint32_t max_present, cudaStream_t s, const void *params)
{
    k_tb_pop_write<P><<<grid_for(max_present, 128), 128, 0, s>>>(ff, tb, first_incomplete, offs, popped, popped_slots, popped_cap, load_params<P>(params));
    WFB_CK(cudaGetLastError());
    return 0;
}
template <class P>
int extract_keys_batches_dispatch(const DevBatch *batches, const uint32_t *boff, uint32_t nb, uint32_t total, uint32_t key_bits, uint64_t *keys,
                                  cudaStream_t s, const void *params)
{
    k_extract_keys_batches<P><<<grid_for(total, 256), 256, 0, s>>>(batches, boff, nb, total, key_bits, keys, load_params<P>(params));
    WFB_CK(cudaGetLastError());
    return 0;
}
template <class P>
int key_order_words_dispatch(const DevBatch *batches, const uint32_t *boff, uint32_t nb, const unsigned char *tuples, uint32_t total, uint64_t *lo,
                             uint64_t *hi, cudaStream_t s, const void *params)
{
    k_key_order_words<P><<<grid_for(total, 256), 256, 0, s>>>(batches, boff, nb, tuples, total, lo, hi, load_params<P>(params));
    WFB_CK(cudaGetLastError());
    return 0;
// ... 115 lines not shown
```

### windflow_b200/csrc/wfb_lib.cu

```cuda
#include <cstdio>
#include <cstdlib>
#include <cstring>
#include <ctime>
#include <mutex>
#include <vector>
#include <algorithm>
#include <atomic>
#include <new>
#include <cuda.h>
#include <cuda_runtime.h>
#include "../../include/wfb200.h"
#include "wfb_kernels.cuh"
#include "wfb_launch.cuh"
#include "wfb_programs.cuh"
#include "wfb_scratch.h"

using namespace wfb;

#define CK(call) do { cudaError_t e__ = (call); if (e__ != cudaSuccess) return static_cast<int>(e__); } while (0)

namespace {

int g_num_sms = 0;

// ... 6 lines not shown
        if (cudaGetDevice(&dev) != cudaSuccess) return WFB_E_NOGPU;
        cudaDeviceGetAttribute(&g_num_sms, cudaDevAttrMultiProcessorCount, dev);
    }
    return 0;
}

std::mutex &registry_mutex() { static std::mutex m; return m; }

std::vector<ProgramOps> &registry()
{
    static std::vector<ProgramOps> table; if (table.empty()) { table.reserve(4096); table = { make_ops<ProgTuple64>(), make_ops<ProgWfTest16>(), make_ops<ProgWfWin24>(), make_ops<ProgLifted32>(),
                                                                 make_ops<ProgTuple64FKey>(), make_ops<ProgTuple64K16>() }; table.reserve(4096); }
    return table;
}

const ProgramOps *program(int prog)
{
    std::lock_guard<std::mutex> lock(registry_mutex());
    std::vector<ProgramOps> &t = registry();
    if (prog < 0 || prog >= static_cast<int>(t.size())) return nullptr;
    return &t[prog];
}

struct PinnedStage {
    static constexpr int SLOTS = 8;
    PinnedScratch<unsigned char> buf[SLOTS]; cudaEvent_t ev[SLOTS] = {}; bool used[SLOTS] = {}; int next = 0;
    int h2d(void *dst, const void *src, size_t bytes, cudaStream_t s)
    {
        if (bytes == 0) return 0;
        const int i = next; next = (next + 1) % SLOTS;
        if (used[i]) CK(cudaEventSynchronize(ev[i]));
        CK(buf[i].ensure(bytes, ScratchWaits(), std::max<size_t>(bytes, 4096) * 2));
        if (!ev[i]) CK(cudaEventCreateWithFlags(&ev[i], cudaEventDisableTiming));
        std::memcpy(buf[i], src, bytes);
        CK(cudaMemcpyAsync(dst, buf[i], bytes, cudaMemcpyHostToDevice, s));
        CK(cudaEventRecord(ev[i], s)); used[i] = true;
        return 0;
    }
    void destroy() { for (int i = 0; i < SLOTS; i++) { if (ev[i]) cudaEventDestroy(ev[i]); ev[i] = nullptr; } }
};

struct StreamOrder {
    cudaStream_t last_stream = nullptr; bool used = false; cudaEvent_t ev = nullptr;

    int init() { CK(cudaEventCreateWithFlags(&ev, cudaEventDisableTiming)); return 0; }
    void destroy() { if (ev) cudaEventDestroy(ev); ev = nullptr; }
    int enter(cudaStream_t s)
    {
        if (used && s != last_stream) { CK(cudaEventRecord(ev, last_stream)); CK(cudaStreamWaitEvent(s, ev, 0)); }
        last_stream = s; used = true;
        return 0;
    }
};

struct TileScratch {
    PinnedStage stage;
    Scratch<uint64_t> tile_state;
    Scratch<uint32_t> ticket; uint32_t ticket_base = 0; uint32_t epoch = 0;
    Scratch<DevBatch> d_batches;
    StreamOrder order;

    int init()
    {
        CK(ticket.ensure(1));
        CK(cudaMemset(ticket, 0, sizeof(uint32_t)));
        return order.init();
    }
    void destroy()
    {
        stage.destroy();
        order.destroy();
    }
    int enter(cudaStream_t s) { return order.enter(s); }
    int ensure_tiles(uint32_t num_tiles) { return tile_state.ensure_zeroed(num_tiles, order.last_stream, order.last_stream); }
    int ensure_batches(uint32_t nb) { return d_batches.ensure(nb, order.last_stream); }
    void next_launch(TileArgs &a) { epoch = (epoch + 1) & 0x3fffffffu; if (epoch == 0) epoch = 1; a.epoch = epoch; a.ticket = ticket; a.ticket_base = ticket_base; a.tile_state = tile_state; }
    void launched(uint32_t num_claims, uint32_t grid) { ticket_base += num_claims + grid; }
};

inline uint32_t tiles_of(uint32_t n) { return (n + TILE - 1) / TILE; }

inline uint32_t osr_group(uint32_t tiles, bool payload) { return !payload && tiles >= OSR_GROUP * static_cast<uint32_t>(g_num_sms) ? OSR_GROUP : 1u; }

cudaError_t osr_smem_attr()
{
    static std::atomic<uint64_t> done{0};
    int dev = 0;
    cudaError_t e = cudaGetDevice(&dev);
    if (e != cudaSuccess) return e;
    const uint64_t bit = 1ull << (dev & 63);
    if (done.load(std::memory_order_relaxed) & bit) return cudaSuccess;
    e = cudaFuncSetAttribute(k_wide_scatter_ranked, cudaFuncAttributeMaxDynamicSharedMemorySize, static_cast<int>(OSR_SMEM));
    if (e == cudaSuccess) done.fetch_or(bit, std::memory_order_relaxed);
    return e;
}

struct RadixSorter {
    Scratch<uint32_t> ctl;
    Scratch<uint64_t> state;
    uint32_t epoch = 0;
    uint64_t launches = 0;

    static constexpr size_t CTL_WORDS = OS_MAX_PASSES * 256 + OS_MAX_PASSES > OSW_DIGITS + 1 ? OS_MAX_PASSES * 256 + OS_MAX_PASSES : OSW_DIGITS + 1;
    static int prepare(uint32_t *ctl_buf, uint32_t passes, cudaStream_t s)
    {
        passes = std::min<uint32_t>(std::max(1u, passes), OS_MAX_PASSES);
        WFB_CK(cudaMemsetAsync(ctl_buf, 0, sizeof(uint32_t) * (passes * 256 + passes), s));
        return 0;
    }

    static int prepare_wide(uint32_t *ctl_buf, cudaStream_t s)
    {
        WFB_CK(cudaMemsetAsync(ctl_buf, 0, sizeof(uint32_t) * (OSW_DIGITS + 1), s));
        return 0;
    }
    Scratch<uint16_t> wideH; Scratch<uint32_t> wideC;
    Scratch<uint32_t> wideT;
    Scratch<uint32_t> wideDone;
    static void wide_geometry(uint32_t cap, bool prefix, uint32_t *tiles, uint32_t *chunk_shift, uint32_t *chunks)
    {
        *tiles = std::max(1u, (cap + OSW_TILE - 1) / OSW_TILE);
        uint32_t cs = prefix ? 5 : 4;
        if (!prefix) while ((1u << (2 * cs)) < *tiles) cs++;
        *chunk_shift = cs;
        *chunks = (*tiles + (1u << cs) - 1) >> cs;
    }
    int ensure_wide_buffers(uint32_t tiles, uint32_t chunks, ScratchWaits waits)
    {
        const size_t rows = static_cast<size_t>(OSW_DIGITS) * tiles, chunk_rows = static_cast<size_t>(OSW_DIGITS) * chunks;
        CK(wideH.ensure(rows, waits, rows));
        CK(wideT.ensure(rows, waits, rows));
        CK(wideC.ensure(chunk_rows, waits, chunk_rows));
        return 0;
    }
    int ensure_wide(uint32_t cap, ScratchWaits waits, uint16_t **rows)
    {
        uint32_t tiles, chunk_shift, chunks;
        wide_geometry(cap, true, &tiles, &chunk_shift, &chunks);
        { int rc = ensure_wide_buffers(tiles, chunks, waits); if (rc) return rc; }
        *rows = wideH;
        return 0;
    }
    template <class K, int RBYTES>
    void launch_wide_scatter(uint32_t tiles, const K *kin, K *kout, uint32_t *vout, const uint32_t *n_ptr, uint32_t n_host, uint32_t shift,
                             uint32_t chunk_shift, const uint32_t *c, cudaStream_t s, const unsigned char *pin, unsigned char *pout, uint32_t pbytes,
                             uint32_t skip_invalid, uint32_t region_stride)
    {
        k_wide_scatter<K, RBYTES><<<tiles, OSW_THREADS, 0, s>>>(kin, kout, vout, n_ptr, n_host, shift, chunk_shift, wideH, wideC, c, pin, pout, pbytes, skip_invalid, region_stride);
    }
    template <class K>
    int sort_wide(const K *kin, K *kout, uint32_t *vout, const uint32_t *n_ptr, uint32_t n_host, uint32_t cap, uint32_t shift,
                  cudaStream_t s, uint32_t *ready_ctl, const uint32_t **counts, const unsigned char *payload_in = nullptr,
                  unsigned char *payload_out = nullptr, uint32_t payload_bytes = 0, bool skip_invalid = false, uint32_t region_stride = 0, uint32_t few_bins = 0,
                  const uint16_t *h16_rows = nullptr)
    {
        if (payload_in && (payload_bytes == 0 || (payload_bytes & 7u))) return WFB_E_BADARG;
        CK(ctl.ensure(CTL_WORDS));
        const bool ranked = ready_ctl && !few_bins;
        const uint16_t *rows = h16_rows ? h16_rows : wideH;
        uint32_t tiles, chunk_shift, chunks;
        wide_geometry(cap, ranked, &tiles, &chunk_shift, &chunks);
        { int rc = ensure_wide_buffers(tiles, chunks, s); if (rc) return rc; }
        uint32_t *c = ready_ctl ? ready_ctl : ctl;
        if (!ready_ctl) { int rc = prepare_wide(c, s); if (rc) return rc; }
        if (ranked) {
            CK(wideDone.ensure_zeroed(1, s));
            k_wide_tile_bases<<<chunks, OSW_THREADS, 0, s>>>(rows, tiles, chunk_shift, chunks, wideC, wideT, c, wideDone,
                                                             osr_group(tiles, payload_in != nullptr) == OSR_GROUP ? 2u : 0u);
        } else if (ready_ctl) {
            k_wide_chunk_sums16<<<chunks, OSW_THREADS, 0, s>>>(rows, tiles, chunk_shift, wideC, c);
        } else {
            CK(cudaMemsetAsync(wideC, 0, sizeof(uint32_t) * OSW_DIGITS * chunks, s));
            k_wide_tile_hist<K><<<tiles, OSW_THREADS, 0, s>>>(kin, n_ptr, n_host, shift, chunk_shift, wideH, wideC, c, skip_invalid ? 1u : 0u);
        }
        if (region_stride && few_bins && payload_in && few_bins <= 32 && (payload_bytes == 16 || payload_bytes == 24 || payload_bytes == 32 || payload_bytes == 64)) {
            const uint32_t *d32 = reinterpret_cast<const uint32_t *>(kin);
            static_assert(sizeof(K) == 4 || sizeof(K) == 8, "key width");
            if (sizeof(K) == 4) {
                switch (payload_bytes) {
                    case 16: k_shard_scatter<16><<<tiles, OSW_THREADS, 0, s>>>(d32, n_host, few_bins, chunk_shift, wideH, wideC, payload_in, payload_out, region_stride); break;
                    case 24: k_shard_scatter<24><<<tiles, OSW_THREADS, 0, s>>>(d32, n_host, few_bins, chunk_shift, wideH, wideC, payload_in, payload_out, region_stride); break;
                    case 32: k_shard_scatter<32><<<tiles, OSW_THREADS, 0, s>>>(d32, n_host, few_bins, chunk_shift, wideH, wideC, payload_in, payload_out, region_stride); break;
                    default: k_shard_scatter<64><<<tiles, OSW_THREADS, 0, s>>>(d32, n_host, few_bins, chunk_shift, wideH, wideC, payload_in, payload_out, region_stride); break;
                }
                CK(cudaGetLastError());
                launches += 2;
                *counts = c;
                return 0;
            }
        }
        if (ranked) {
            if (sizeof(K) != 4 || !kout || (payload_in ? !payload_out || region_stride : !vout)) return WFB_E_UNSUPPORTED;
            if (!payload_in && osr_group(tiles, false) == OSR_GROUP) {
                CK(osr_smem_attr());
                k_wide_scatter_ranked<<<(tiles + OSR_GROUP - 1) / OSR_GROUP, OSW_THREADS, OSR_SMEM, s>>>(reinterpret_cast<const uint32_t *>(kin), reinterpret_cast<uint32_t *>(kout),
                                                                                                       vout, n_host, shift, chunk_shift, tiles, rows, wideC, wideT);
            }
#define WFB_WSRT(RB_) k_wide_scatter_ranked_tile<RB_><<<tiles, OSW_THREADS, 0, s>>>(reinterpret_cast<const uint32_t *>(kin), reinterpret_cast<uint32_t *>(kout), vout, n_host, shift, \
                                                                                  chunk_shift, rows, wideC, wideT, payload_in, payload_out)
            else if (!payload_in) WFB_WSRT(0);
            else switch (payload_bytes) {
                case 16: WFB_WSRT(16); break; case 24: WFB_WSRT(24); break; case 32: WFB_WSRT(32); break; case 48: WFB_WSRT(48); break; case 64: WFB_WSRT(64); break;
                default: return WFB_E_UNSUPPORTED;
            }
#undef WFB_WSRT
            CK(cudaGetLastError());
            launches += 2;
            *counts = c;
            return 0;
        }
#define WFB_WS(RB_) launch_wide_scatter<K, RB_>(tiles, kin, kout, vout, n_ptr, n_host, shift, chunk_shift, c, s, payload_in, payload_out, payload_bytes, skip_invalid ? 1u : 0u, region_stride)
        if (!payload_in) WFB_WS(0);
        else switch (payload_bytes) {
            case 8: WFB_WS(8); break;   case 16: WFB_WS(16); break; case 24: WFB_WS(24); break; case 32: WFB_WS(32); break;
            case 48: WFB_WS(48); break; case 64: WFB_WS(64); break; default: WFB_WS(-1); break;
        }
#undef WFB_WS
        CK(cudaGetLastError());
        launches += 2;
        *counts = c;
        return 0;
    }

    template <class K>
    int sort(K *kA, K *kB, uint32_t *vA, uint32_t *vB, const uint32_t *n_ptr, uint32_t n_host, uint32_t cap, uint32_t passes,
             cudaStream_t s, const K **skeys, const uint32_t **svals, uint32_t *ready_ctl = nullptr, uint32_t *seg_first = nullptr, uint32_t seg_first_n = 0, uint32_t base_shift = 0)
    {
        const bool hist_ready = ready_ctl != nullptr;
        if (!hist_ready) CK(ctl.ensure(CTL_WORDS));
        uint32_t *const c = hist_ready ? ready_ctl : static_cast<uint32_t *>(ctl);
        const uint32_t TE = OS_THREADS * OS_ITEMS;
        const uint64_t state_words = static_cast<uint64_t>((cap + OS_THREADS * 4 - 1) / (OS_THREADS * 4)) * 256;
        CK(state.ensure_zeroed(state_words, s, s, state_words));
        passes = std::min<uint32_t>(std::max(1u, passes), OS_MAX_PASSES);
        const uint32_t tiles = std::max(1u, (cap + TE - 1) / TE);
        if (!hist_ready) {
            CK(cudaMemsetAsync(c, 0, sizeof(uint32_t) * (passes * 256 + passes), s));
            k_radix_ghist<K><<<std::min(tiles, static_cast<uint32_t>(g_num_sms) * 4u), 256, 0, s>>>(kA, n_ptr, n_host, passes, c, base_shift);
            launches++;
        }
        const K *kin = kA; const uint32_t *vin = nullptr;
        K *kout = kB; uint32_t *vout = vB;
        for (uint32_t p = 0; p < passes; p++) {
            epoch = (epoch + 1) & 0x3fffffffu; if (epoch == 0) epoch = 1;
            uint32_t *sf = (p + 1 == passes) ? seg_first : nullptr;
            k_onesweep_pass<K><<<tiles, OS_THREADS, 0, s>>>(kin, vin, kout, vout, n_ptr, n_host, p, passes, c, state, epoch, sf, seg_first_n, base_shift);
            kin = kout; vin = vout;
            if (kout == kB) { kout = kA; vout = vA; } else { kout = kB; vout = vB; }
        }
        CK(cudaGetLastError());
        launches += passes;
        *skeys = kin; *svals = vin;
        return 0;
    }
};

struct GrowPlan {
    struct Array { void **ptr; size_t old_bytes, bytes; bool copy; int fill; bool counted; void *fresh; };
    std::vector<Array> arrays;
    template <class T> void add(T *&p, size_t old_bytes, size_t bytes, bool copy, int fill, bool counted = true)
    {
        arrays.push_back({reinterpret_cast<void **>(&p), old_bytes, bytes, copy, fill, counted, nullptr});
    }
    template <class T> T *fresh(T *const &p) const
    {
        for (const Array &a : arrays) if (a.ptr == reinterpret_cast<void *const *>(&p)) return static_cast<T *>(a.fresh);
        return nullptr;
    }
    int64_t grown_bytes() const { int64_t d = 0; for (const Array &a : arrays) if (a.counted) d += static_cast<int64_t>(a.bytes) - static_cast<int64_t>(a.old_bytes); return d; }
    int alloc()
    {
        for (Array &a : arrays)
            if (cudaMalloc(&a.fresh, a.bytes) != cudaSuccess) { cudaGetLastError(); release(); return WFB_E_CAPACITY; }
        return 0;
    }
    void release() { for (Array &a : arrays) { cudaFree(a.fresh); a.fresh = nullptr; } }
    int fill(cudaStream_t s)
    {
        for (Array &a : arrays) {
            const size_t keep = a.copy ? a.old_bytes : 0;
            if (keep) CK(cudaMemcpyAsync(a.fresh, *a.ptr, keep, cudaMemcpyDeviceToDevice, s));
            if (a.fill >= 0 && a.bytes > keep) CK(cudaMemsetAsync(static_cast<unsigned char *>(a.fresh) + keep, a.fill, a.bytes - keep, s));
        }
        return 0;
    }
    void commit() { for (Array &a : arrays) { cudaFree(*a.ptr); *a.ptr = a.fresh; a.fresh = nullptr; } }
};

struct GrowCheck {
    uint32_t *host = nullptr; cudaEvent_t ev = nullptr;
    int init() { CK(cudaMallocHost(reinterpret_cast<void **>(&host), 2 * sizeof(uint32_t))); CK(cudaEventCreateWithFlags(&ev, cudaEventDisableTiming)); return 0; }
    void destroy() { if (host) cudaFreeHost(host); if (ev) cudaEventDestroy(ev); host = nullptr; ev = nullptr; }
};

template <class AddState, class Derive>
int grow_keys(FfatDev &ff, uint32_t key_bytes, GrowCheck &gc, uint32_t ceiling, uint32_t limit, cudaStream_t s, bool *grew, AddState add_state,
              Derive derive)
{
    *grew = false;
    CK(cudaMemcpyAsync(gc.host, ff.n_slots, 2 * sizeof(uint32_t), cudaMemcpyDeviceToHost, s));
    CK(cudaEventRecord(gc.ev, s));
    CK(cudaEventSynchronize(gc.ev));
    if (!(gc.host[1] & KEYS_GROW_FLAG)) return 0;
    const uint32_t old = ff.max_keys;
    uint64_t cap = 1; while (cap < 2ull * std::max(gc.host[0], old)) cap <<= 1;
    if (cap > ceiling && old < ceiling && gc.host[0] <= ceiling) cap = ceiling;
    if (cap > limit) return WFB_E_CAPACITY;
    uint64_t entries = 1; while (entries < 2 * cap) entries <<= 1;
    GrowPlan plan;
    plan.add(ff.ht_keys, static_cast<size_t>(key_bytes) * (ff.ht_mask + 1ull), key_bytes * entries, false, 0xff);
    plan.add(ff.ht_slots, sizeof(uint32_t) * (ff.ht_mask + 1ull), sizeof(uint32_t) * entries, false, 0xff);
    plan.add(ff.slot_key, static_cast<size_t>(key_bytes) * old, static_cast<size_t>(key_bytes) * cap, true, -1);
    int rc = add_state(plan, static_cast<uint32_t>(cap)); if (rc) return rc;
    rc = plan.alloc(); if (rc) return rc;
    rc = plan.fill(s);
    if (!rc) {
        k_key_table_rebuild<<<grid_for(ff.ht_mask + 1, 256), 256, 0, s>>>(ff.ht_keys, ff.ht_slots, ff.ht_mask, plan.fresh(ff.ht_keys), plan.fresh(ff.ht_slots),
                                                                        static_cast<uint32_t>(entries - 1), plan.fresh(ff.slot_key), old, key_bytes / 8, ff.err_flags);
        rc = static_cast<int>(cudaGetLastError());
    }
    if (!rc) rc = static_cast<int>(cudaStreamSynchronize(s));
    if (rc) { cudaStreamSynchronize(s); plan.release(); return rc; }
    plan.commit();
    ff.ht_mask = static_cast<uint32_t>(entries - 1); ff.max_keys = static_cast<uint32_t>(cap);
    rc = derive(static_cast<uint32_t>(cap), plan); if (rc) return rc;
    *grew = true;
    return 0;
}

}

struct wfb_engine {
    int prog = 0;
    const ProgramOps *ops = nullptr;
    std::vector<unsigned char> params;
    const void *pp() const { return params.empty() ? nullptr : params.data(); }
    TileScratch ts;
    uint64_t launches = 0;
    uint32_t key_bits = 64;
    Scratch<uint64_t> keysA, keysB;
    Scratch<uint32_t> idxA, idxB, destA, destB;
    Scratch<uint32_t> head, seg_begin;
    Scratch<unsigned char> sh_lifted; Scratch<uint32_t> sh_dest, sh_ctl;
    Scratch<uint32_t> rb_off, rb_first, rb_total;
    Scratch<uint32_t> rb_long;
    RadixSorter sorter;
    Scratch<uint64_t> wlo, whi; Scratch<uint32_t> wperm;

    int ensure_sort(uint32_t n, cudaStream_t s)
    {
        CK(keysA.ensure(n, s));
        const size_t cap = keysA.capacity();
// ... 914 lines not shown
        CK(h->tb_popped.ensure(RB * total));
        const size_t pop_cap = h->tb_popped.capacity() / RB, slots_cap = (pop_cap + TILE - 1) / TILE * TILE;
        CK(h->tb_popped_slots.ensure(slots_cap, ScratchWaits(), slots_cap));
        rc = h->ops->tb_pop_write(h->ff, h->tb, F, h->tb.cnt, h->tb_popped, h->tb_popped_slots, static_cast<uint32_t>(pop_cap), maxp, s, prm); if (rc) return rc;
        h->launches += 10 + (h->sorter.launches - before);
        if (total) {
            wfb_batch_t pb; std::memset(&pb, 0, sizeof(pb));
            pb.tuples = h->tb_popped; pb.ts = nullptr; pb.watermark = wm; pb.n = total;
            const uint64_t lb = h->cb->launches;
            rc = ffat_process_cb_impl(h->cb, prm, &pb, 1, static_cast<unsigned char *>(out_results) + static_cast<size_t>(produced) * RB,
                                      out_ts ? out_ts + produced : nullptr, out_capacity - produced, n_out_dev, s, h->tb_popped_slots);
            if (rc) return rc;
            h->launches += h->cb->launches - lb;
            uint32_t got = 0;
            CK(cudaMemcpyAsync(&got, n_out_dev, sizeof(uint32_t), cudaMemcpyDeviceToHost, s));
            CK(cudaStreamSynchronize(s));
            produced += std::min(got, out_capacity - produced);
        }
    }
    CK(cudaMemcpyAsync(n_out_dev, &produced, sizeof(uint32_t), cudaMemcpyHostToDevice, s));
    CK(cudaStreamSynchronize(s));
    return 0;
}

int wfb_ffat_create(wfb_ffat_t **hh, int prog, uint64_t win, uint64_t slide, uint32_t wins_per_batch,
                    uint32_t max_keys, int win_type, uint64_t lateness, uint32_t flags)
{
    if (!hh || win == 0 || slide == 0 || wins_per_batch == 0 || max_keys == 0) return WFB_E_BADARG;
    if ((flags & WFB_KEYS_GROW) && (flags & (WFB_FFAT_DENSE_KEYS | WFB_FFAT_PIPELINED))) return WFB_E_BADARG;
    if (win_type == 1) return tb_create(hh, prog, win, slide, wins_per_batch, max_keys, lateness, flags);
    if (win_type != 0) return WFB_E_UNSUPPORTED;
    const ProgramOps *o = program(prog);
    if (!o) return WFB_E_NOPROG;
    if ((flags & WFB_FFAT_DENSE_KEYS) && o->key_kind != KEY_KIND_INTEGRAL) return WFB_E_BADARG;
    int rc = device_ready(); if (rc) return rc;
    wfb_ffat *h = new (std::nothrow) wfb_ffat();
    if (!h) return WFB_E_BADARG;
    h->prog = prog; h->ops = o; h->win_type = win_type;
    rc = h->ts.init(); if (rc) { delete h; return rc; }
    FfatDev &ff = h->ff;
    ff.win = win; ff.slide = slide; ff.nb = wins_per_batch;
    ff.B = static_cast<uint64_t>(wins_per_batch - 1) * slide + win;
    const uint64_t pane = gcd_u64(win, slide);
    const uint64_t bp = ff.B / pane;
    if (pane > 0xffffffffull || bp > (1ull << 30)) { delete h; return WFB_E_BADARG; }
    ff.pane = static_cast<uint32_t>(pane); ff.wp = static_cast<uint32_t>(win / pane); ff.sp = static_cast<uint32_t>(slide / pane);
    const uint64_t spare_min = std::min<uint64_t>(bp, 32);
    uint32_t n = 1, lg = 0; while (n < bp + spare_min) { n <<= 1; lg++; }
    ff.n_leaves = n; ff.log_leaves = lg;
    ff.defer_items = (static_cast<uint64_t>(n) - bp + 1) * pane;
    ff.max_keys = max_keys; ff.dense = (flags & WFB_FFAT_DENSE_KEYS) ? 1u : 0u;
    uint32_t cap = 1; while (cap < 2ull * max_keys) cap <<= 1;
    ff.ht_mask = cap - 1;
    const size_t RB = o->result_bytes;
    const size_t tree_bytes = static_cast<size_t>(max_keys) * (2ull * n - 1) * RB;
    size_t total = 0;
#define ALLOC(ptr, bytes) do { cudaError_t e_ = cudaMalloc(reinterpret_cast<void **>(&(ptr)), (bytes)); if (e_ != cudaSuccess) { wfb_ffat_destroy(h); return static_cast<int>(e_); } total += (bytes); } while (0)
    if (!ff.dense) {
        ALLOC(ff.ht_keys, static_cast<size_t>(o->key_bytes) * cap);
        ALLOC(ff.ht_slots, sizeof(uint32_t) * cap);
        CK(cudaMemset(ff.ht_keys, 0xff, static_cast<size_t>(o->key_bytes) * cap));
        CK(cudaMemset(ff.ht_slots, 0xff, sizeof(uint32_t) * cap));
    }
    ALLOC(ff.n_slots, sizeof(uint32_t) * 4);
    h->own_n_slots = ff.n_slots;
    ff.err_flags = ff.n_slots + 1;
    ff.results_total = reinterpret_cast<unsigned long long *>(ff.n_slots + 2);
    CK(cudaMemset(ff.n_slots, 0, sizeof(uint32_t) * 4));
    ALLOC(ff.slot_key, static_cast<size_t>(o->key_bytes) * max_keys);
    ALLOC(ff.cnt, sizeof(uint64_t) * max_keys);
    CK(cudaMemset(ff.cnt, 0, sizeof(uint64_t) * max_keys));
    ALLOC(ff.acc, RB * max_keys);
    CK(cudaMemset(ff.acc, 0, RB * max_keys));
    ALLOC(ff.tree, tree_bytes);
    CK(cudaMemset(ff.tree, 0, tree_bytes));
    ALLOC(ff.seg_off, sizeof(uint32_t) * (static_cast<size_t>(max_keys) + 1));
    CK(cudaMemset(ff.seg_off, 0xff, sizeof(uint32_t) * (static_cast<size_t>(max_keys) + 1)));
    ALLOC(ff.heavy, sizeof(uint32_t) * max_keys);
    ff.light_max = 256;
    h->pipelined = (flags & WFB_FFAT_PIPELINED) != 0;
    for (int p = 0; p < (h->pipelined ? 2 : 1); p++) {
        SegScratch &g = h->seg[p];
        ALLOC(g.seg_cnt, sizeof(uint32_t) * max_keys);
        CK(cudaMemset(g.seg_cnt, 0, sizeof(uint32_t) * max_keys));
        ALLOC(g.n_total, sizeof(uint32_t) * 4);
        CK(cudaMemset(g.n_total, 0, sizeof(uint32_t) * 4));
        g.n_trig = g.n_total + 1; g.res_n = h->pipelined ? g.n_total + 2 : nullptr; g.n_heavy = g.n_total + 3;
        ALLOC(g.sort_ctl, sizeof(uint32_t) * RadixSorter::CTL_WORDS);
        CK(cudaEventCreateWithFlags(&g.ev_ingest, cudaEventDisableTiming));
        CK(cudaEventCreateWithFlags(&g.ev_done, cudaEventDisableTiming));
    }
    if (h->pipelined) CK(cudaStreamCreateWithFlags(&h->s2, cudaStreamNonBlocking));
#undef ALLOC
    if (flags & WFB_KEYS_GROW) { ff.grow = 1; rc = h->growc.init(); if (rc) { wfb_ffat_destroy(h); return rc; } }
    { const char *e = std::getenv("WFB_BUCKET_MOVE"); h->bucket_move = e && std::atoi(e) != 0; }
    ffat_derive_paths(h);
    {
        const bool fits = h->buckets && static_cast<size_t>(2) * ff.n_leaves * RB <= (32u << 10);
        const bool pays = static_cast<uint64_t>(ff.n_leaves) <= 2ull * std::max(1u, ff.log_leaves) * ff.sp * ff.nb;
        ff.lazy = (fits && pays) ? 1u : 0u;
    }
    h->state_bytes = total;
    *hh = h;
    return 0;
}

int wfb_ffat_destroy(wfb_ffat_t *h)
{
    if (!h) return 0;
    cudaDeviceSynchronize();
    FfatDev &ff = h->ff;
    cudaFree(ff.ht_keys); cudaFree(ff.ht_slots); cudaFree(h->own_n_slots); if (!h->shares_slot_key) cudaFree(ff.slot_key); cudaFree(ff.cnt);
    cudaFree(ff.acc); cudaFree(ff.tree); cudaFree(ff.seg_off); cudaFree(ff.heavy);
    for (SegScratch &g : h->seg) { cudaFree(g.n_total); cudaFree(g.seg_cnt); cudaFree(g.sort_ctl); g.destroy(); }
    if (h->cb) wfb_ffat_destroy(h->cb);
    cudaFree(h->tb.first); cudaFree(h->tb.num); cudaFree(h->tb.num_new); cudaFree(h->tb.trig); cudaFree(h->tb.done); cudaFree(h->tb.ring);
    cudaFree(h->tb.present); cudaFree(h->tb.cnt); cudaFree(h->tb_misc);
    if (h->s2) cudaStreamDestroy(h->s2);
    for (auto &e : h->tev) cudaEventDestroy(e);
    h->ts.destroy(); h->growc.destroy();
    delete h;
    cudaGetLastError();
    return 0;
}

uint64_t wfb_ffat_launches(const wfb_ffat_t *h) { return h ? h->launches : 0; }

int wfb_ffat_set_params(wfb_ffat_t *h, const void *params, size_t bytes)
{
    if (!h || !params || bytes != h->ops->params_bytes) return WFB_E_BADARG;
    h->params.assign(static_cast<const unsigned char *>(params), static_cast<const unsigned char *>(params) + bytes);
    if (h->cb) h->cb->params = h->params;
    return 0;
}
uint64_t wfb_ffat_state_bytes(const wfb_ffat_t *h) { return h ? h->state_bytes : 0; }
uint32_t wfb_ffat_key_capacity(const wfb_ffat_t *h) { return h ? h->ff.max_keys : 0; }
int wfb_ffat_set_key_shard(wfb_ffat_t *h, uint32_t num_shards, uint32_t shard)
{
    if (!h || num_shards == 0 || shard >= num_shards || !h->ff.dense || h->call_no != 0) return WFB_E_BADARG;
    if (h->win_type == 1) {
        if (h->cb == nullptr || h->cb->call_no != 0) return WFB_E_BADARG;
        h->cb->ff.key_div = num_shards; h->cb->ff.key_rem = shard;
    }
    h->ff.key_div = num_shards; h->ff.key_rem = shard;
    return 0;
}

static double host_now_us() { timespec t; clock_gettime(CLOCK_MONOTONIC, &t); return t.tv_sec * 1e6 + t.tv_nsec * 1e-3; }
static int ffat_ensure_segment(wfb_ffat *h, SegScratch &g, uint32_t total, uint32_t nbatches, cudaStream_t s)
{
    const ScratchWaits w = h->s2 ? ScratchWaits(s, h->s2) : ScratchWaits(s);
    CK(g.slotsA.ensure(total, w));
    const size_t cap = g.slotsA.capacity(), RB = h->ops->result_bytes;
    CK(g.slotsB.ensure(total, w, cap)); CK(g.posA.ensure(total, w, cap)); CK(g.posB.ensure(total, w, cap));
    CK(g.lifted.ensure(RB * total, w, RB * cap));
    if (h->bucket_move) CK(g.lifted_sorted.ensure(RB * total, w, RB * cap));
    const uint32_t trig_cap = ffat_trig_cap(h, static_cast<uint32_t>(cap), h->ff.max_keys);
    CK(g.trig.ensure(trig_cap, w, trig_cap));
    if (h->pipelined) {
        const size_t res_cap = std::min<uint64_t>(static_cast<uint64_t>(trig_cap) * h->ff.nb, 0x7fffffffull);
        CK(g.res_ts.ensure(res_cap, w, res_cap)); CK(g.res.ensure(RB * res_cap, w, RB * res_cap));
    }
    CK(g.batch_off.ensure(nbatches + 1ull, w));
    CK(g.d_batches.ensure(nbatches + 1ull, w, g.batch_off.capacity()));
    return 0;
}

static int ffat_window_phase(wfb_ffat *h, SegScratch &g, const FfatDev &ff, unsigned char *out, uint64_t *out_ts, uint32_t out_cap,
                             uint32_t *n_out, cudaStream_t s)
{
    const uint32_t *sorted_slots, *sorted_pos;
    const uint64_t before = h->sorter.launches;
    int rc;
    if (h->buckets) {
        const uint32_t *counts = nullptr;
        rc = h->sorter.sort_wide<uint32_t>(g.slotsA, g.slotsB, g.posB, nullptr, g.total, g.total, h->bucket_shift, s, g.sort_ctl, &counts,
                                           h->bucket_move ? static_cast<unsigned char *>(g.lifted) : nullptr,
                                           h->bucket_move ? static_cast<unsigned char *>(g.lifted_sorted) : nullptr,
                                           static_cast<uint32_t>(h->ops->result_bytes), true, 0, 0, h->pipelined ? static_cast<uint16_t *>(g.h16) : nullptr);
        if (rc) return rc;
        h->launches += h->sorter.launches - before;
        h->mark(2, s);
        rc = h->ops->ffat_buckets(ff, h->bucket_move ? g.lifted_sorted : g.lifted_src, g.slotsB, g.posB, counts, h->bucket_shift, h->bucket_move ? 1u : 0u, g.batch_off, g.d_batches, g.nbatches, out, out_ts,
                                  out_cap, n_out, s, h->pp());
        if (rc) return rc;
        h->launches += 1;
    } else {
        rc = h->sorter.sort<uint32_t>(g.slotsA, g.slotsB, g.posA, g.posB, g.n_total, 0, g.total, h->sort_passes, s, &sorted_slots,
                                      &sorted_pos, g.sort_ctl, ff.seg_off, ff.max_keys);
        if (rc) return rc;
        h->launches += h->sorter.launches - before;
        h->mark(2, s);
        uint32_t ugrid = std::max(1u, std::min((ff.max_keys + 7) / 8, static_cast<uint32_t>(g_num_sms) * 8u));
        rc = h->ops->ffat_update(ff, g.lifted, sorted_pos, g.batch_off, g.d_batches, g.nbatches, out, out_ts, out_cap, n_out, ugrid, s, h->pp(),
                                 std::max(1u, std::min((ff.max_keys + 127u) / 128u, static_cast<uint32_t>(g_num_sms) * 16u)));
        if (rc) return rc;
        h->launches += 2;
    }
    rc = h->ops->ffat_windows(ff, g.batch_off, g.d_batches, g.nbatches, out, out_ts, out_cap, static_cast<uint32_t>(g_num_sms) * 4u, s, h->pp(), n_out);
    if (rc) return rc;
    h->launches += 1;
    return 0;
}

static int ffat_deliver(wfb_ffat *h, SegScratch &g, unsigned char *out, uint64_t *out_ts, uint32_t out_cap, uint32_t *n_out, cudaStream_t s)
{
    if (!g.pending) { CK(cudaMemsetAsync(n_out, 0, sizeof(uint32_t), s)); return 0; }
    CK(cudaStreamWaitEvent(s, g.ev_done, 0));
    k_copy_results<<<static_cast<uint32_t>(g_num_sms) * 2u, 256, 0, s>>>(g.res, g.res_ts, g.res_n, h->ops->result_bytes, out, out_ts,
                                                                          out_cap, n_out, h->ff.err_flags);
    CK(cudaGetLastError());
    h->launches++;
    g.pending = false;
    return 0;
}

int wfb_ffat_process_cb(wfb_ffat_t *h, const wfb_functors_t *pre, const wfb_batch_t *batches_h, uint32_t nbatches,
                        void *out_results, uint64_t *out_ts, uint32_t out_capacity, uint32_t *n_out_dev, void *stream)
{
    return ffat_process_cb_impl(h, pre, batches_h, nbatches, out_results, out_ts, out_capacity, n_out_dev, stream, nullptr);
}

static int ffat_process_cb_impl(wfb_ffat_t *h, const void *pre, const wfb_batch_t *batches_h, uint32_t nbatches,
                                void *out_results, uint64_t *out_ts, uint32_t out_capacity, uint32_t *n_out_dev, void *stream,
                                const uint32_t *ext_slots)
{
    if (!h || !n_out_dev || (nbatches && !batches_h) || (out_capacity && !out_results)) return WFB_E_BADARG;
    if (h->win_type != 0) return WFB_E_BADARG;
    cudaStream_t s = static_cast<cudaStream_t>(stream);
    int rc = h->ts.enter(s); if (rc) return rc;
    unsigned char *out = static_cast<unsigned char *>(out_results);
    const uint32_t par = h->pipelined ? static_cast<uint32_t>(h->call_no & 1u) : 0u;
    SegScratch &g = h->seg[par];
    SegScratch &prev = h->seg[h->pipelined ? (par ^ 1u) : 0u];

    std::vector<DevBatch> hb;
    hb.reserve(nbatches);
    uint64_t total = 0; uint32_t tiles = 0;
    uint64_t span_begin = ~0ull, span_end = 0;
    for (uint32_t i = 0; i < nbatches; i++) {
        if (batches_h[i].n == 0) continue;
        if (!batches_h[i].tuples) return WFB_E_BADARG;
        DevBatch b; std::memset(&b, 0, sizeof(b));
        b.tuples = static_cast<const unsigned char *>(batches_h[i].tuples); b.ts = batches_h[i].ts;
        b.watermark = batches_h[i].watermark; b.n = batches_h[i].n; b.tile_begin = tiles;
        tiles += tiles_of(b.n); total += b.n;
        const uint64_t p0 = reinterpret_cast<uint64_t>(b.tuples);
        span_begin = std::min(span_begin, p0); span_end = std::max(span_end, p0 + static_cast<uint64_t>(b.n) * h->ops->tuple_bytes);
        hb.push_back(b);
    }
    if (total > 0x7fffffffull) return WFB_E_BADARG;
    if (total == 0) {
        if (h->pipelined) return ffat_deliver(h, prev, out, out_ts, out_capacity, n_out_dev, s);
        if (!h->append_results) CK(cudaMemsetAsync(n_out_dev, 0, sizeof(uint32_t), s));
        return 0;
    }
    nbatches = static_cast<uint32_t>(hb.size());
    FfatDev ff;
    const auto ingest = [&]() -> int {
        const bool sparse = h->buckets;
        const uint64_t seg_cap = sparse ? static_cast<uint64_t>(tiles) * TILE : total;
        if (seg_cap > 0x7fffffffull) return WFB_E_BADARG;
        rc = ffat_ensure_segment(h, g, static_cast<uint32_t>(seg_cap), nbatches, s); if (rc) return rc;
        rc = h->ts.ensure_tiles(tiles); if (rc) return rc;
        { int rc_ = h->ts.stage.h2d(g.d_batches, hb.data(), sizeof(DevBatch) * nbatches, s); if (rc_) return rc_; }
        g.nbatches = nbatches; g.total = static_cast<uint32_t>(seg_cap);
        if (sparse) {
            std::vector<uint32_t> boff(nbatches + 1);
            for (uint32_t i = 0; i < nbatches; i++) boff[i] = hb[i].tile_begin * TILE;
            boff[nbatches] = tiles * TILE;
            { int rc_ = h->ts.stage.h2d(g.batch_off, boff.data(), sizeof(uint32_t) * (nbatches + 1), s); if (rc_) return rc_; }
        }

        ff = h->ff;
        ff.seg_cnt = g.seg_cnt; ff.trig = g.trig; ff.n_trig = g.n_trig; ff.trig_cap = static_cast<uint32_t>(g.trig.capacity()); ff.n_heavy = g.n_heavy;

        const uint32_t npasses = h->buckets ? 1u : h->sort_passes;
        rc = h->buckets ? RadixSorter::prepare_wide(g.sort_ctl, s) : RadixSorter::prepare(g.sort_ctl, npasses, s); if (rc) return rc;
        h->mark(0, s);
        TileArgs a; std::memset(&a, 0, sizeof(a));
        a.sort_ctl = g.sort_ctl; a.sort_passes = npasses; a.sort_shift = h->buckets ? h->bucket_shift : 0u; a.sort_dbits = h->buckets ? OSW_BITS : 8u;
        a.batches = g.d_batches; a.nbatches = nbatches; a.num_tiles = tiles;
        a.lifted = g.lifted; a.slots = g.slotsA; a.batch_off = g.batch_off; a.n_total = g.n_total; a.ff = ff;
        g.lifted_src = g.lifted;
        if (sparse && !h->pipelined && !h->bucket_move && (h->ops->reserved & 1u)) {
            const unsigned char *base = hb[0].tuples;
            bool ok = (reinterpret_cast<uintptr_t>(base) & 15u) == 0;
            for (uint32_t i = 0; ok && i < nbatches; i++) ok = hb[i].tuples == base + static_cast<size_t>(hb[i].tile_begin) * TILE * h->ops->tuple_bytes;
            if (ok) { a.inplace = 1; g.lifted_src = base; a.ext_slots = ext_slots; }
        }
        if (ext_slots != nullptr && !a.inplace) {
            if (sparse) return WFB_E_UNSUPPORTED;
            if (nbatches != 1 || !(h->ops->reserved & 1u)) return WFB_E_BADARG;
            a.ext_slots = ext_slots;
        }
        h->ts.next_launch(a);
        a.max_ctas_per_sm = h->pipelined ? 2u : 0u;
        a.l2_hints = 1;
        a.sparse = sparse ? 1u : 0u;
        a.count_keys = h->buckets ? 0u : 1u;
        uint32_t claims = tiles;
        if (sparse) {
            const ScratchWaits w = h->pipelined ? ScratchWaits(s, h->s2) : ScratchWaits(s);
            rc = h->sorter.ensure_wide(g.total, w, &a.wide_h16); if (rc) return rc;
            if (h->pipelined) {
                const size_t wt = (g.total + OSW_TILE - 1) / OSW_TILE;
                CK(g.h16.ensure(OSW_DIGITS * wt, w));
                a.wide_h16 = g.h16;
            }
            a.tiles_per_ticket = OSW_TILE_POS / TILE;
            a.sort_ctl = nullptr;
            a.pack_rank = 1;
            claims = (tiles + a.tiles_per_ticket - 1) / a.tiles_per_ticket;
        }
        if (a.inplace && h->ops->slots_inplace) {
            rc = h->ops->slots_inplace(a, pre ? static_cast<const void *>(pre) : h->pp(), s); if (rc) return rc;
        } else {
            uint32_t grid = 0;
            rc = h->ops->tile_pass(MODE_INGEST, a, pre ? static_cast<const void *>(pre) : h->pp(), claims, s, &grid, span_begin, span_end); if (rc) return rc;
            h->ts.launched(claims, grid);
        }
        h->launches++;
        h->mark(1, s);
        return 0;
    };
    rc = ingest(); if (rc) return rc;
    for (bool grew = h->ff.grow != 0; grew; ) {
        rc = ffat_grow(h, s, &grew); if (rc) return rc;
        if (grew) { rc = ingest(); if (rc) return rc; h->launches++; }
    }

    if (!h->pipelined) {
        if (!h->append_results) CK(cudaMemsetAsync(n_out_dev, 0, sizeof(uint32_t), s));
        rc = ffat_window_phase(h, g, ff, out, out_ts, out_capacity, n_out_dev, s); if (rc) return rc;
        h->mark(3, s);
    } else {
        CK(cudaEventRecord(g.ev_ingest, s));
        rc = ffat_deliver(h, prev, out, out_ts, out_capacity, n_out_dev, s); if (rc) return rc;
        CK(cudaStreamWaitEvent(h->s2, g.ev_ingest, 0));
        CK(cudaMemsetAsync(g.res_n, 0, sizeof(uint32_t), h->s2));
        rc = ffat_window_phase(h, g, ff, g.res, g.res_ts, static_cast<uint32_t>(g.res_ts.capacity()), g.res_n, h->s2); if (rc) return rc;
        h->mark(3, h->s2);
        CK(cudaEventRecord(g.ev_done, h->s2));
        g.pending = true;
    }
    if (h->timing && h->tev_used < wfb_ffat::TEV_MAX) h->tev_used++;
    h->call_no++;
    return 0;
}

static int ffat_process_prebucketed(wfb_ffat *h, const unsigned char *records, const uint32_t *recv_slots, const uint32_t *bins, uint32_t nsrc,
                                    uint32_t bps, const uint32_t *offs_h, const uint64_t *wms_h, uint32_t slot_mask, uint32_t shift,
                                    void *out_results, uint64_t *out_ts, uint32_t out_capacity, uint32_t *n_out_dev, cudaStream_t s, bool append, uint32_t items)
{
    if (!h || !n_out_dev || nsrc == 0 || nsrc > MAX_SHARDS || bps == 0 || bps > OSW_DIGITS || (1u << shift) > BK_KEYS) return WFB_E_BADARG;
    if (h->win_type != 0 || h->pipelined || !h->buckets) return WFB_E_UNSUPPORTED;
    int rc = h->ts.enter(s); if (rc) return rc;
    SegScratch &g = h->seg[0];
    const uint32_t total = items;
    if (!append) CK(cudaMemsetAsync(n_out_dev, 0, sizeof(uint32_t), s));
    if (total == 0) return 0;
    rc = ffat_ensure_segment(h, g, total, nsrc, s); if (rc) return rc;
    std::vector<DevBatch> hb(nsrc);
    for (uint32_t i = 0; i < nsrc; i++) {
        std::memset(&hb[i], 0, sizeof(DevBatch));
        hb[i].tuples = records + static_cast<size_t>(offs_h[i]) * h->ops->result_bytes; hb[i].n = offs_h[i + 1] - offs_h[i]; hb[i].watermark = wms_h[i];
    }
    { int rc_ = h->ts.stage.h2d(g.d_batches, hb.data(), sizeof(DevBatch) * nsrc, s); if (rc_) return rc_; }
    { int rc_ = h->ts.stage.h2d(g.batch_off, offs_h, sizeof(uint32_t) * (nsrc + 1), s); if (rc_) return rc_; }
    g.nbatches = nsrc; g.total = total; g.lifted_src = records;
    FfatDev ff = h->ff;
    ff.seg_cnt = g.seg_cnt; ff.trig = g.trig; ff.n_trig = g.n_trig; ff.trig_cap = static_cast<uint32_t>(g.trig.capacity()); ff.n_heavy = g.n_heavy;
    rc = RadixSorter::prepare_wide(g.sort_ctl, s); if (rc) return rc;
    h->mark(0, s); h->mark(1, s);
    MgRuns runs;
    for (uint32_t i = 0; i <= MAX_SHARDS; i++) runs.off[i] = offs_h[std::min(i, nsrc)];
    uint32_t nsub = 1, shift2 = shift;
    while (nsub * 2 * bps <= OSW_DIGITS && nsub * 2 <= MAX_SHARDS && shift2 > 0) { nsub *= 2; shift2--; }
    CK(h->mg_scratch.ensure(3 * OSW_DIGITS * MAX_SHARDS));
    uint32_t *cnt3 = h->mg_scratch, *off3 = cnt3 + OSW_DIGITS * MAX_SHARDS, *run_starts = off3 + OSW_DIGITS * MAX_SHARDS;
    const dim3 grid(bps, nsrc);
    k_mg_count<<<grid, MG_THREADS, 0, s>>>(bins, nsrc, bps, runs, recv_slots, slot_mask, shift2, nsub, cnt3, run_starts, g.n_trig, g.n_heavy);
    k_mg_scan<<<1, 1024, 0, s>>>(cnt3, bps * nsub * nsrc, nsrc, off3, g.sort_ctl);
    k_mg_split<<<grid, MG_THREADS, 0, s>>>(bins, nsrc, bps, runs, recv_slots, slot_mask, shift2, nsub, off3, run_starts, g.slotsB, g.posB);
    CK(cudaGetLastError());
    h->mark(2, s);
    rc = h->ops->ffat_buckets(ff, records, g.slotsB, g.posB, g.sort_ctl, shift2, 0u, g.batch_off, g.d_batches, nsrc, static_cast<unsigned char *>(out_results), out_ts,
                              out_capacity, n_out_dev, s, h->pp());
    if (rc) return rc;
    rc = h->ops->ffat_windows(ff, g.batch_off, g.d_batches, nsrc, static_cast<unsigned char *>(out_results), out_ts, out_capacity, static_cast<uint32_t>(g_num_sms) * 4u, s,
                              h->pp(), n_out_dev);
    if (rc) return rc;
    h->mark(3, s);
    h->launches += 5;
    if (h->timing && h->tev_used < wfb_ffat::TEV_MAX) h->tev_used++;
    h->call_no++;
    return 0;
}

int wfb_ffat_flush(wfb_ffat_t *h, void *out_results, uint64_t *out_ts, uint32_t out_capacity, uint32_t *n_out_dev, void *stream)
{
    if (!h || !n_out_dev || (out_capacity && !out_results)) return WFB_E_BADARG;
    cudaStream_t s = static_cast<cudaStream_t>(stream);
    if (!h->pipelined) { CK(cudaMemsetAsync(n_out_dev, 0, sizeof(uint32_t), s)); return 0; }
    int rc = h->ts.enter(s); if (rc) return rc;
    SegScratch &last = h->seg[(h->call_no + 1) & 1u];
    return ffat_deliver(h, last, static_cast<unsigned char *>(out_results), out_ts, out_capacity, n_out_dev, s);
}

int wfb_ffat_timing(wfb_ffat_t *h, int enable, float *ms_h, uint32_t *calls_h)
{
    if (!h) return WFB_E_BADARG;
    float acc[4] = {0, 0, 0, 0};
    if (h->tev_used) {
        CK(cudaEventSynchronize(h->tev[(h->tev_used - 1) * 4 + 3]));
        for (uint32_t i = 0; i < h->tev_used; i++) {
            float a = 0, b = 0, c = 0, d = 0;
            cudaEvent_t *e = &h->tev[i * 4];
            CK(cudaEventElapsedTime(&a, e[0], e[1]));
            CK(cudaEventElapsedTime(&b, e[1], e[2]));
            CK(cudaEventElapsedTime(&c, e[2], e[3]));
            CK(cudaEventElapsedTime(&d, e[0], e[3]));
            acc[0] += a; acc[1] += b; acc[2] += c; acc[3] += d;
        }
    }
    if (ms_h) for (int i = 0; i < 4; i++) ms_h[i] = acc[i];
    if (calls_h) *calls_h = h->tev_used;
    h->tev_used = 0;
    if (enable && h->tev.empty()) {
        h->tev.resize(wfb_ffat::TEV_MAX * 4);
        for (auto &e : h->tev) CK(cudaEventCreate(&e));
    }
    h->timing = enable != 0;
    return 0;
}

int wfb_ffat_stats(wfb_ffat_t *h, uint32_t *n_keys_h, uint32_t *err_flags_h, void *stream)
{
    if (!h) return WFB_E_BADARG;
    uint32_t v[2] = {0, 0};
    int rc = h->ts.enter(static_cast<cudaStream_t>(stream)); if (rc) return rc;
    if (h->s2) CK(cudaStreamSynchronize(h->s2));
    CK(cudaMemcpyAsync(v, h->ff.n_slots, sizeof(v), cudaMemcpyDeviceToHost, static_cast<cudaStream_t>(stream)));
    CK(cudaStreamSynchronize(static_cast<cudaStream_t>(stream)));
    if (n_keys_h) *n_keys_h = v[0];
    if (err_flags_h) *err_flags_h = v[1];
    if (h->cb && err_flags_h) { uint32_t e2 = 0; rc = wfb_ffat_stats(h->cb, nullptr, &e2, stream); if (rc) return rc; *err_flags_h |= e2; }
    return 0;
}

int wfb_ffat_results_total(wfb_ffat_t *h, uint64_t *total_h, void *stream)
{
    if (!h || !total_h) return WFB_E_BADARG;
    wfb_ffat *src = h->cb ? h->cb : h;
    int rc = h->ts.enter(static_cast<cudaStream_t>(stream)); if (rc) return rc;
    if (src != h) { rc = src->ts.enter(static_cast<cudaStream_t>(stream)); if (rc) return rc; }
    unsigned long long v = 0;
    if (src->s2) CK(cudaStreamSynchronize(src->s2));
    if (src->ff.results_total == nullptr) { *total_h = 0; return 0; }
    CK(cudaMemcpyAsync(&v, src->ff.results_total, sizeof(v), cudaMemcpyDeviceToHost, static_cast<cudaStream_t>(stream)));
    CK(cudaStreamSynchronize(static_cast<cudaStream_t>(stream)));
    *total_h = v;
    return 0;
}

}
#include <dlfcn.h>
namespace {
struct Nccl {
    struct Id { char b[128]; };
    typedef int (*GetUniqueId_t)(void *);
    typedef int (*CommInitRank_t)(void **, int, Id, int);
    typedef int (*CommDestroy_t)(void *);
    typedef int (*SendRecv_t)(void *, size_t, int, int, void *, cudaStream_t);
    typedef int (*Group_t)();
    typedef const char *(*ErrStr_t)(int);
    void *lib = nullptr;
    GetUniqueId_t GetUniqueId = nullptr; CommInitRank_t CommInitRank = nullptr; CommDestroy_t CommDestroy = nullptr;
    SendRecv_t Send = nullptr, Recv = nullptr; Group_t GroupStart = nullptr, GroupEnd = nullptr;
    bool ok = false;
    Nccl()
    {
        const char *names[] = {std::getenv("WFB_NCCL_LIB"), "libnccl.so.2", "libnccl.so"};
        for (const char *n : names) { if (n && (lib = dlopen(n, RTLD_NOW | RTLD_GLOBAL))) break; }
        if (!lib) return;
        GetUniqueId = reinterpret_cast<GetUniqueId_t>(dlsym(lib, "ncclGetUniqueId"));
        CommInitRank = reinterpret_cast<CommInitRank_t>(dlsym(lib, "ncclCommInitRank"));
        CommDestroy = reinterpret_cast<CommDestroy_t>(dlsym(lib, "ncclCommDestroy"));
        Send = reinterpret_cast<SendRecv_t>(dlsym(lib, "ncclSend")); Recv = reinterpret_cast<SendRecv_t>(dlsym(lib, "ncclRecv"));
        GroupStart = reinterpret_cast<Group_t>(dlsym(lib, "ncclGroupStart")); GroupEnd = reinterpret_cast<Group_t>(dlsym(lib, "ncclGroupEnd"));
        ok = GetUniqueId && CommInitRank && CommDestroy && Send && Recv && GroupStart && GroupEnd;
    }
};
Nccl &nccl() { static Nccl n; return n; }
constexpr int NCCL_UINT8 = 1;
#define NK(call) do { int r__ = (call); if (r__ != 0) return 1000 + r__; } while (0)

__global__ void k_mg_meta(const uint32_t *__restrict__ counts, uint64_t watermark, uint32_t nranks, uint64_t *__restrict__ send_meta)
{
    const uint32_t d = threadIdx.x;
    if (d < nranks) { send_meta[2 * d] = counts[d]; send_meta[2 * d + 1] = watermark; }
}

__global__ void k_mg_pre_append(unsigned long long *results_total, const uint32_t *n_out) { if (results_total) *results_total -= *n_out; }

struct MgSlot {
    Scratch<unsigned char> regions;
    uint32_t region_cap = 0;
    Scratch<uint32_t> vslots;
    uint32_t *bins = nullptr;
    uint32_t *recv_slots = nullptr, *recv_bins = nullptr; size_t recv_slots_cap = 0;
    unsigned char *ce_buf = nullptr;
    unsigned char *peer[MAX_SHARDS] = {};
    uint32_t offs[MAX_SHARDS + 1] = {}; uint64_t wms[MAX_SHARDS] = {};
    uint32_t *counts = nullptr;
    uint64_t *send_meta = nullptr, *recv_meta = nullptr;
    uint32_t *h_counts = nullptr; uint64_t *h_recv = nullptr;
    unsigned char *recv = nullptr; size_t recv_bytes = 0;
    cudaEvent_t ev_src = nullptr, ev_meta = nullptr, ev_a2a = nullptr, ev_done = nullptr, ev_self = nullptr, ev_fork = nullptr;
    bool used = false, done_recorded = false, exchanged = false;
    cudaEvent_t tr[8] = {}; bool tr_valid = false;
};
}

struct wfb_mg {
    int nranks = 1, rank = 0;
    void *comm = nullptr;
    wfb_engine_t *eng = nullptr;
    wfb_ffat_t *ffat = nullptr;
    size_t rb = 0;
    MgSlot slot[4];
    cudaStream_t cs = nullptr;
    cudaStream_t cs2 = nullptr;
    uint64_t step_no = 0;
    MgSlot *pend[3] = {nullptr, nullptr, nullptr}; int npend = 0;
    std::vector<wfb_batch_t> chunks;
    bool ce = false, ce_tried = false; uint64_t ce_cap = 0, peer_cap[MAX_SHARDS] = {};
    unsigned char *ce_msg = nullptr;
    cudaEvent_t ev_flush = nullptr;
    static constexpr int CE_STREAMS = 4;
    cudaStream_t ce_s[CE_STREAMS] = {}; cudaEvent_t ce_ev[CE_STREAMS] = {};
    uint32_t *tok = nullptr;
    cudaEvent_t last_done = nullptr;
    double host_acc[3] = {}; uint64_t host_n = 0;
    bool trace = false; double tr_acc[8] = {}; uint64_t tr_n = 0;
    bool bucketed = false;
    uint32_t shard_slots = 0, shard_keys = 0, shift = 0, bps = 0;
};

extern "C" {

int wfb_mg_unique_id(void *id128_h)
{
    if (!id128_h) return WFB_E_BADARG;
    if (!nccl().ok) return WFB_E_UNSUPPORTED;
    NK(nccl().GetUniqueId(id128_h));
    return 0;
}

int wfb_mg_destroy(wfb_mg_t *h)
{
    if (!h) return 0;
    cudaDeviceSynchronize();
    if (h->comm && nccl().ok) nccl().CommDestroy(h->comm);
    if (h->eng) wfb_engine_destroy(h->eng);
    if (h->ffat) wfb_ffat_destroy(h->ffat);
    for (MgSlot &sl : h->slot) {
        cudaFree(sl.counts); cudaFree(sl.send_meta); cudaFree(sl.recv_meta); if (!sl.ce_buf) cudaFree(sl.recv);
        cudaFree(sl.bins);
        if (sl.ce_buf) {
            for (int p = 0; p < h->nranks; p++) if (p != h->rank && sl.peer[p]) cudaIpcCloseMemHandle(sl.peer[p]);
            cudaFree(sl.ce_buf); sl.recv = nullptr;
        } else { cudaFree(sl.recv_slots); cudaFree(sl.recv_bins); }
        if (sl.h_counts) cudaFreeHost(sl.h_counts);
        if (sl.h_recv) cudaFreeHost(sl.h_recv);
        for (cudaEvent_t e : {sl.ev_src, sl.ev_meta, sl.ev_a2a, sl.ev_done, sl.ev_self, sl.ev_fork}) if (e) cudaEventDestroy(e);
        for (cudaEvent_t e : sl.tr) if (e) cudaEventDestroy(e);
    }
    if (h->cs) cudaStreamDestroy(h->cs);
    if (h->cs2) cudaStreamDestroy(h->cs2);
    cudaFree(h->ce_msg); cudaFree(h->tok);
    if (h->ev_flush) cudaEventDestroy(h->ev_flush);
    for (cudaStream_t st : h->ce_s) if (st) cudaStreamDestroy(st);
    for (cudaEvent_t e : h->ce_ev) if (e) cudaEventDestroy(e);
    delete h;
    cudaGetLastError();
    return 0;
}

int wfb_mg_create(wfb_mg_t **hh, int prog, int nranks, int rank, const void *id128_h, uint64_t win, uint64_t slide, uint32_t wins_per_batch,
                  uint32_t max_keys_total)
{
    if (!hh || nranks < 1 || nranks > static_cast<int>(MAX_SHARDS) || rank < 0 || rank >= nranks || (nranks > 1 && !id128_h) || max_keys_total == 0) return WFB_E_BADARG;
    const ProgramOps *o = program(prog);
    if (!o) return WFB_E_NOPROG;
    const int lp = lifted_program_of(prog);
    if (lp < 0 || !(program(lp)->reserved2 & 1u)) return WFB_E_UNSUPPORTED;
    if (o->key_kind != KEY_KIND_INTEGRAL) return WFB_E_UNSUPPORTED;
    int rc = device_ready(); if (rc) return rc;
    if (nranks > 1 && !nccl().ok) return WFB_E_UNSUPPORTED;
    wfb_mg *h = new (std::nothrow) wfb_mg();
    if (!h) return WFB_E_BADARG;
    h->nranks = nranks; h->rank = rank; h->rb = o->result_bytes;
    h->trace = std::getenv("WFB_MG_TRACE") && std::atoi(std::getenv("WFB_MG_TRACE")) != 0;
#define MGCK(call) do { int r__ = (call); if (r__) { wfb_mg_destroy(h); return r__; } } while (0)
    MGCK(wfb_engine_create(&h->eng, prog));
    MGCK(wfb_ffat_create(&h->ffat, lp, win, slide, wins_per_batch, (max_keys_total + nranks - 1) / nranks, 0, 0, WFB_FFAT_DENSE_KEYS));
    if (nranks > 1) MGCK(wfb_ffat_set_key_shard(h->ffat, static_cast<uint32_t>(nranks), static_cast<uint32_t>(rank)));
    MGCK(static_cast<int>(cudaStreamCreateWithFlags(&h->cs, cudaStreamNonBlocking)));
    MGCK(static_cast<int>(cudaStreamCreateWithFlags(&h->cs2, cudaStreamNonBlocking)));
    MGCK(static_cast<int>(cudaEventCreateWithFlags(&h->ev_flush, cudaEventDisableTiming)));
    {
        const uint32_t keys = (max_keys_total + nranks - 1) / nranks;
        uint32_t L = 1; while (L < keys) L <<= 1;
        static const bool off = std::getenv("WFB_MG_BUCKETED") && std::atoi(std::getenv("WFB_MG_BUCKETED")) == 0;
        const size_t rb = o->result_bytes;
        if (!off && static_cast<uint64_t>(L) * nranks <= 65536u && h->ffat->buckets && (rb == 16 || rb == 24 || rb == 32 || rb == 48 || rb == 64)) {
            uint32_t span = 1; while (span < L * static_cast<uint32_t>(nranks)) span <<= 1;
            uint32_t sh = 0; while ((span >> sh) > OSW_DIGITS) sh++;
            if ((L >> sh) >= 1) { h->bucketed = true; h->shard_slots = L; h->shard_keys = keys; h->shift = sh; h->bps = L >> sh; }
        }
    }
    for (MgSlot &sl : h->slot) {
        if (h->bucketed) {
            MGCK(static_cast<int>(cudaMalloc(&sl.bins, sizeof(uint32_t) * (OSW_DIGITS + 1))));
            MGCK(static_cast<int>(cudaMalloc(&sl.recv_bins, sizeof(uint32_t) * MAX_SHARDS * OSW_DIGITS)));
        }
        MGCK(static_cast<int>(cudaMalloc(&sl.counts, sizeof(uint32_t) * (MAX_SHARDS + 1))));
        MGCK(static_cast<int>(cudaMalloc(&sl.send_meta, sizeof(uint64_t) * 2 * MAX_SHARDS)));
        MGCK(static_cast<int>(cudaMalloc(&sl.recv_meta, sizeof(uint64_t) * 2 * MAX_SHARDS)));
        MGCK(static_cast<int>(cudaMallocHost(&sl.h_counts, sizeof(uint32_t) * (MAX_SHARDS + 1))));
        MGCK(static_cast<int>(cudaMallocHost(&sl.h_recv, sizeof(uint64_t) * 2 * MAX_SHARDS)));
        for (cudaEvent_t *e : {&sl.ev_src, &sl.ev_meta, &sl.ev_a2a, &sl.ev_done, &sl.ev_self, &sl.ev_fork}) MGCK(static_cast<int>(cudaEventCreateWithFlags(e, cudaEventDisableTiming)));
        if (h->trace) for (cudaEvent_t &e : sl.tr) MGCK(static_cast<int>(cudaEventCreate(&e)));
    }
    if (nranks > 1) {
        Nccl::Id id; std::memcpy(id.b, id128_h, sizeof(id.b));
        int r = nccl().CommInitRank(&h->comm, nranks, id, rank);
        if (r != 0) { wfb_mg_destroy(h); return 1000 + r; }
    }
#undef MGCK
    *hh = h;
    return 0;
}

int wfb_mg_set_params(wfb_mg_t *h, const void *params, size_t bytes)
{
    if (!h) return WFB_E_BADARG;
    int rc = wfb_engine_set_params(h->eng, params, bytes); if (rc) return rc;
    return wfb_ffat_set_params(h->ffat, params, bytes);
}

struct CeLayout { size_t slots_off, bins_off, bytes; };
static CeLayout ce_layout(uint64_t cap, int n, size_t rb, uint32_t bps)
{
    CeLayout l; l.slots_off = static_cast<size_t>(n) * cap * rb; l.bins_off = (l.slots_off + static_cast<size_t>(n) * cap * 4 + 255) & ~static_cast<size_t>(255);
    l.bytes = l.bins_off + static_cast<size_t>(n) * bps * 4; return l;
// ... 143 lines not shown
        uint64_t tot = 0;
        for (int p = 0; p < n; p++) { sl.offs[p] = static_cast<uint32_t>(tot); tot += sl.h_recv[2 * p]; sl.wms[p] = sl.h_recv[2 * p + 1]; }
        if (tot > 0x7fffffffull) return WFB_E_CAPACITY;
        sl.offs[n] = static_cast<uint32_t>(tot);
        if (h->ce) {
            const uint64_t cap = h->ce_cap;
            if (static_cast<uint64_t>(n) * cap > 0x7fffffffull) return WFB_E_CAPACITY;
            for (int p = 0; p <= n; p++) sl.offs[p] = static_cast<uint32_t>(p * cap);
            size_t send_off[MAX_SHARDS + 1]; send_off[0] = 0;
            for (int p = 0; p < n; p++) {
                send_off[p + 1] = send_off[p] + sl.h_counts[p];
                if (sl.h_recv[2 * p] > cap || sl.h_counts[p] > h->peer_cap[p]) return WFB_E_CAPACITY;
            }
            const int slot_idx = static_cast<int>(&sl - h->slot);
            const size_t bin_bytes = sizeof(uint32_t) * h->bps;
            if (h->trace) CK(cudaEventRecord(sl.tr[4], h->cs));
            CK(cudaStreamWaitEvent(h->cs2, sl.ev_src, 0));
            if (sl.done_recorded) CK(cudaStreamWaitEvent(h->cs2, sl.ev_done, 0));
            static const char *push_env = std::getenv("WFB_MG_PUSH");
            const bool use_sm = push_env && std::strcmp(push_env, "sm") == 0 && h->rb % 16 == 0;
            {
                const int p = h->rank;
                const CeLayout l = ce_layout(h->peer_cap[p], n, h->rb, h->bps);
                unsigned char *dst = h->slot[slot_idx].peer[p];
                const uint64_t me = static_cast<uint64_t>(h->rank), pc = h->peer_cap[p];
                CK(cudaMemcpyAsync(dst + me * pc * h->rb, sl.regions + send_off[p] * h->rb, static_cast<size_t>(sl.h_counts[p]) * h->rb, cudaMemcpyDeviceToDevice, h->cs2));
                CK(cudaMemcpyAsync(dst + l.slots_off + me * pc * 4, sl.vslots + send_off[p], static_cast<size_t>(sl.h_counts[p]) * 4, cudaMemcpyDeviceToDevice, h->cs2));
                CK(cudaMemcpyAsync(dst + l.bins_off + me * bin_bytes, sl.bins + static_cast<size_t>(p) * h->bps, bin_bytes, cudaMemcpyDeviceToDevice, h->cs2));
                CK(cudaEventRecord(sl.ev_self, h->cs2));
            }
            if (use_sm) {
                MgPush a; std::memset(&a, 0, sizeof(a));
                int k = 0;
                for (int p = 0; p < n; p++) {
                    if (p == h->rank) continue;
                    const CeLayout l = ce_layout(h->peer_cap[p], n, h->rb, h->bps);
                    unsigned char *dst = h->slot[slot_idx].peer[p];
                    const uint64_t me = static_cast<uint64_t>(h->rank), pc = h->peer_cap[p];
                    a.rec_src[k] = reinterpret_cast<const uint4 *>(sl.regions + send_off[p] * h->rb); a.rec_dst[k] = reinterpret_cast<uint4 *>(dst + me * pc * h->rb);
                    a.rec_n16[k] = static_cast<uint32_t>(static_cast<size_t>(sl.h_counts[p]) * h->rb / 16);
                    a.slot_src[k] = sl.vslots + send_off[p]; a.slot_dst[k] = reinterpret_cast<uint32_t *>(dst + l.slots_off + me * pc * 4); a.slot_n[k] = sl.h_counts[p];
                    a.bin_src[k] = sl.bins + static_cast<size_t>(p) * h->bps; a.bin_dst[k] = reinterpret_cast<uint32_t *>(dst + l.bins_off + me * bin_bytes);
                    k++;
                }
                a.bin_n = h->bps;
                k_mg_push<<<static_cast<uint32_t>(k) * MG_PUSH_CTAS, MG_PUSH_THREADS, 0, h->cs>>>(a);
                CK(cudaGetLastError());
            } else {
                CK(cudaEventRecord(sl.ev_fork, h->cs));
                const int nst = std::min(wfb_mg::CE_STREAMS, n - 1);
                for (int i = 0; i < nst; i++) CK(cudaStreamWaitEvent(h->ce_s[i], sl.ev_fork, 0));
                int k = 0;
                for (int p = 0; p < n; p++) {
                    if (p == h->rank) continue;
                    const CeLayout l = ce_layout(h->peer_cap[p], n, h->rb, h->bps);
                    unsigned char *dst = h->slot[slot_idx].peer[p];
                    const uint64_t me = static_cast<uint64_t>(h->rank), pc = h->peer_cap[p];
                    cudaStream_t st = h->ce_s[k++ % nst];
                    CK(cudaMemcpyAsync(dst + me * pc * h->rb, sl.regions + send_off[p] * h->rb, static_cast<size_t>(sl.h_counts[p]) * h->rb, cudaMemcpyDeviceToDevice, st));
                    CK(cudaMemcpyAsync(dst + l.slots_off + me * pc * 4, sl.vslots + send_off[p], static_cast<size_t>(sl.h_counts[p]) * 4, cudaMemcpyDeviceToDevice, st));
                    CK(cudaMemcpyAsync(dst + l.bins_off + me * bin_bytes, sl.bins + static_cast<size_t>(p) * h->bps, bin_bytes, cudaMemcpyDeviceToDevice, st));
                }
                for (int i = 0; i < nst; i++) { CK(cudaEventRecord(h->ce_ev[i], h->ce_s[i])); CK(cudaStreamWaitEvent(h->cs, h->ce_ev[i], 0)); }
            }
            if (h->trace) CK(cudaEventRecord(sl.tr[5], h->cs));
            if (h->last_done) CK(cudaStreamWaitEvent(h->cs, h->last_done, 0));
            NK(nccl().GroupStart());
            for (int p = 0; p < n; p++) {
                if (p == h->rank) continue;
                NK(nccl().Send(h->tok, 4, NCCL_UINT8, p, h->comm, h->cs));
                NK(nccl().Recv(h->tok + 1 + p, 4, NCCL_UINT8, p, h->comm, h->cs));
            }
            NK(nccl().GroupEnd());
            CK(cudaEventRecord(sl.ev_a2a, h->cs));
            return 0;
        }
        const size_t need = std::max<size_t>(1, tot);
        if (sl.recv_bytes < need * h->rb || sl.recv_slots_cap < need) {
            CK(cudaDeviceSynchronize());
            cudaFree(sl.recv); cudaFree(sl.recv_slots);
            sl.recv = nullptr; sl.recv_slots = nullptr; sl.recv_bytes = 0; sl.recv_slots_cap = 0;
            const size_t cap = need * 5 / 4;
            CK(cudaMalloc(&sl.recv, cap * h->rb)); sl.recv_bytes = cap * h->rb;
            CK(cudaMalloc(&sl.recv_slots, sizeof(uint32_t) * cap)); sl.recv_slots_cap = cap;
        }
        if (sl.done_recorded) CK(cudaStreamWaitEvent(h->cs, sl.ev_done, 0));
        if (h->trace) CK(cudaEventRecord(sl.tr[4], h->cs));
        size_t send_off[MAX_SHARDS + 1]; send_off[0] = 0;
        for (int p = 0; p < n; p++) send_off[p + 1] = send_off[p] + sl.h_counts[p];
        const size_t bin_bytes = sizeof(uint32_t) * h->bps;
        if (n > 1) {
            {
                const int p = h->rank;
                CK(cudaStreamWaitEvent(h->cs2, sl.ev_src, 0));
                if (sl.done_recorded) CK(cudaStreamWaitEvent(h->cs2, sl.ev_done, 0));
                CK(cudaMemcpyAsync(sl.recv + static_cast<size_t>(sl.offs[p]) * h->rb, sl.regions + send_off[p] * h->rb, static_cast<size_t>(sl.h_counts[p]) * h->rb, cudaMemcpyDeviceToDevice, h->cs2));
                CK(cudaMemcpyAsync(sl.recv_slots + sl.offs[p], sl.vslots + send_off[p], static_cast<size_t>(sl.h_counts[p]) * 4, cudaMemcpyDeviceToDevice, h->cs2));
                CK(cudaMemcpyAsync(sl.recv_bins + static_cast<size_t>(p) * h->bps, sl.bins + static_cast<size_t>(p) * h->bps, bin_bytes, cudaMemcpyDeviceToDevice, h->cs2));
                CK(cudaEventRecord(sl.ev_self, h->cs2));
            }
            NK(nccl().GroupStart());
            for (int p = 0; p < n; p++) {
                if (p == h->rank) continue;
                NK(nccl().Send(sl.regions + send_off[p] * h->rb, static_cast<size_t>(sl.h_counts[p]) * h->rb, NCCL_UINT8, p, h->comm, h->cs));
                NK(nccl().Recv(sl.recv + static_cast<size_t>(sl.offs[p]) * h->rb, static_cast<size_t>(sl.h_recv[2 * p]) * h->rb, NCCL_UINT8, p, h->comm, h->cs));
                NK(nccl().Send(sl.vslots + send_off[p], static_cast<size_t>(sl.h_counts[p]) * 4, NCCL_UINT8, p, h->comm, h->cs));
                NK(nccl().Recv(sl.recv_slots + sl.offs[p], static_cast<size_t>(sl.h_recv[2 * p]) * 4, NCCL_UINT8, p, h->comm, h->cs));
                NK(nccl().Send(sl.bins + static_cast<size_t>(p) * h->bps, bin_bytes, NCCL_UINT8, p, h->comm, h->cs));
                NK(nccl().Recv(sl.recv_bins + static_cast<size_t>(p) * h->bps, bin_bytes, NCCL_UINT8, p, h->comm, h->cs));
            }
            NK(nccl().GroupEnd());
        } else {
            CK(cudaMemcpyAsync(sl.recv, sl.regions, static_cast<size_t>(sl.h_counts[0]) * h->rb, cudaMemcpyDeviceToDevice, h->cs));
            CK(cudaMemcpyAsync(sl.recv_slots, sl.vslots, static_cast<size_t>(sl.h_counts[0]) * 4, cudaMemcpyDeviceToDevice, h->cs));
            CK(cudaMemcpyAsync(sl.recv_bins, sl.bins, bin_bytes, cudaMemcpyDeviceToDevice, h->cs));
        }
        CK(cudaEventRecord(sl.ev_a2a, h->cs));
        if (h->trace) CK(cudaEventRecord(sl.tr[5], h->cs));
        return 0;
    }
    size_t tiles = 0;
    for (int p = 0; p < n; p++) { sl.offs[p] = static_cast<uint32_t>(tiles * TILE); tiles += (static_cast<size_t>(sl.h_recv[2 * p]) + TILE - 1) / TILE; sl.wms[p] = sl.h_recv[2 * p + 1]; }
    if (tiles * TILE > 0x7fffffffull) return WFB_E_CAPACITY;
    const size_t need = std::max<size_t>(1, tiles * TILE) * h->rb;
    if (sl.recv_bytes < need) {
        CK(cudaDeviceSynchronize());
        cudaFree(sl.recv);
        sl.recv = nullptr; sl.recv_bytes = 0;
        CK(cudaMalloc(&sl.recv, need * 5 / 4)); sl.recv_bytes = need * 5 / 4;
    }
    if (sl.done_recorded) CK(cudaStreamWaitEvent(h->cs, sl.ev_done, 0));
    if (h->trace) CK(cudaEventRecord(sl.tr[4], h->cs));
    if (n > 1) {
        NK(nccl().GroupStart());
        for (int p = 0; p < n; p++) {
            NK(nccl().Send(sl.regions + static_cast<size_t>(p) * sl.region_cap * h->rb, static_cast<size_t>(sl.h_counts[p]) * h->rb, NCCL_UINT8, p, h->comm, h->cs));
            NK(nccl().Recv(sl.recv + static_cast<size_t>(sl.offs[p]) * h->rb, static_cast<size_t>(sl.h_recv[2 * p]) * h->rb, NCCL_UINT8, p, h->comm, h->cs));
        }
        NK(nccl().GroupEnd());
    } else CK(cudaMemcpyAsync(sl.recv, sl.regions, static_cast<size_t>(sl.h_counts[0]) * h->rb, cudaMemcpyDeviceToDevice, h->cs));
    CK(cudaEventRecord(sl.ev_a2a, h->cs));
    if (h->trace) CK(cudaEventRecord(sl.tr[5], h->cs));
    return 0;
}

static int mg_update(wfb_mg *h, MgSlot &sl, void *out, uint64_t *out_ts, uint32_t out_cap, uint32_t *n_out_dev, cudaStream_t s, bool append = false)
{
    const int n = h->nranks;
    CK(cudaStreamWaitEvent(s, sl.ev_a2a, 0));
    if (h->bucketed && n > 1) CK(cudaStreamWaitEvent(s, sl.ev_self, 0));
    if (h->trace) CK(cudaEventRecord(sl.tr[2], s));
    uint64_t items = 0;
    for (int p = 0; p < n; p++) items += sl.h_recv[2 * p];
    if (append && items != 0) { k_mg_pre_append<<<1, 1, 0, s>>>(h->ffat->ff.results_total, n_out_dev); CK(cudaGetLastError()); }
    int rc;
    if (h->bucketed) {
        rc = ffat_process_prebucketed(h->ffat, sl.recv, sl.recv_slots, sl.recv_bins, static_cast<uint32_t>(n), h->bps, sl.offs, sl.wms, h->shard_slots - 1u, h->shift,
                                      out, out_ts, out_cap, n_out_dev, s, append, static_cast<uint32_t>(items));
    } else {
        h->chunks.resize(n);
        for (int p = 0; p < n; p++) {
            wfb_batch_t &b = h->chunks[p];
            b.tuples = sl.recv + static_cast<size_t>(sl.offs[p]) * h->rb; b.ts = nullptr; b.watermark = sl.wms[p]; b.n = static_cast<uint32_t>(sl.h_recv[2 * p]); b.reserved = 0;
        }
        h->ffat->append_results = append;
        rc = wfb_ffat_process_cb(h->ffat, nullptr, h->chunks.data(), static_cast<uint32_t>(n), out, out_ts, out_cap, n_out_dev, s);
        h->ffat->append_results = false;
    }
    if (rc) return rc;
    CK(cudaEventRecord(sl.ev_done, s));
    h->last_done = sl.ev_done;
    if (h->trace) { CK(cudaEventRecord(sl.tr[3], s)); sl.tr_valid = true; }
    sl.done_recorded = true;
    return 0;
}

int wfb_mg_step(wfb_mg_t *h, const wfb_functors_t *pre, const wfb_batch_t *batches_h, uint32_t nbatches, uint64_t watermark,
                void *out_results, uint64_t *out_ts, uint32_t out_capacity, uint32_t *n_out_dev, void *stream)
{
    if (!h || !n_out_dev || (nbatches && !batches_h)) return WFB_E_BADARG;
    cudaStream_t s = static_cast<cudaStream_t>(stream);
    MgSlot &cur = h->slot[h->step_no % 4];
    h->step_no++;
    MgSlot *ex = h->npend >= 2 ? h->pend[h->npend - 2] : nullptr, *upd = h->npend == 3 ? h->pend[0] : nullptr;
    int rc;
    const double t0 = h->trace ? host_now_us() : 0;
    if (ex != nullptr && !ex->exchanged) { rc = mg_exchange(h, *ex); if (rc) return rc; ex->exchanged = true; }
    const double t1 = h->trace ? host_now_us() : 0;
    rc = mg_source(h, cur, pre, batches_h, nbatches, watermark, s); if (rc) return rc;
    const double t2 = h->trace ? host_now_us() : 0;
    cur.exchanged = false;
    if (upd != nullptr) { h->pend[0] = h->pend[1]; h->pend[1] = h->pend[2]; h->pend[2] = &cur; } else h->pend[h->npend++] = &cur;
    if (upd == nullptr) { CK(cudaMemsetAsync(n_out_dev, 0, sizeof(uint32_t), s)); return 0; }
    rc = mg_update(h, *upd, out_results, out_ts, out_capacity, n_out_dev, s);
    upd->exchanged = false;
    if (h->trace) {
        const double t3 = host_now_us();
        h->host_acc[0] += t1 - t0; h->host_acc[1] += t2 - t1; h->host_acc[2] += t3 - t2;
        if (++h->host_n % 64 == 0) {
            std::fprintf(stderr, "[wfb_mg rank %d] host us/step over 64 steps: issue exchange %.0f | issue source + sizes %.0f | issue update %.0f\n", h->rank,
                         h->host_acc[0] / 64, h->host_acc[1] / 64, h->host_acc[2] / 64);
            h->host_acc[0] = h->host_acc[1] = h->host_acc[2] = 0;
        }
    }
    return rc;
}

int wfb_mg_flush(wfb_mg_t *h, void *out_results, uint64_t *out_ts, uint32_t out_capacity, uint32_t *n_out_dev, void *stream)
{
    if (!h || !n_out_dev) return WFB_E_BADARG;
    cudaStream_t s = static_cast<cudaStream_t>(stream);
    if (h->npend == 0) { CK(cudaMemsetAsync(n_out_dev, 0, sizeof(uint32_t), s)); return 0; }
    const int n = h->npend; h->npend = 0;
    int rc;
    for (int i = 0; i < n; i++) {
        MgSlot &sl = *h->pend[i];
        if (!sl.exchanged) { rc = mg_exchange(h, sl); if (rc) return rc; }
        rc = mg_update(h, sl, out_results, out_ts, out_capacity, n_out_dev, s, i != 0); if (rc) return rc;
        sl.exchanged = false;
        h->pend[i] = nullptr;
    }
    return 0;
}

uint64_t wfb_mg_launches(const wfb_mg_t *h) { return h ? wfb_engine_launches(h->eng) + wfb_ffat_launches(h->ffat) : 0; }

int wfb_mg_stats(wfb_mg_t *h, uint32_t *err_flags_h, uint64_t *results_total_h, void *stream)
{
    if (!h) return WFB_E_BADARG;
    uint32_t nk = 0, ef = 0; uint64_t tot = 0;
    int rc = wfb_ffat_stats(h->ffat, &nk, &ef, stream); if (rc) return rc;
    rc = wfb_ffat_results_total(h->ffat, &tot, stream); if (rc) return rc;
    if (err_flags_h) *err_flags_h = ef;
    if (results_total_h) *results_total_h = tot;
    return 0;
}

int wfb_gen_tuple64(uint64_t seed, uint64_t start, uint32_t n, int key_mode, uint64_t nkeys, const double *zipf_cdf,
                    void *tuples, uint64_t *ts, void *stream)
{
    int rc = device_ready(); if (rc) return rc;
    if ((n && !tuples) || nkeys == 0 || (key_mode == 2 && !zipf_cdf)) return WFB_E_BADARG;
    if (n == 0) return 0;
    const uint32_t grid = std::min((n + 255) / 256, static_cast<uint32_t>(g_num_sms) * 16u);
    k_gen_tuple64<<<grid, 256, 0, static_cast<cudaStream_t>(stream)>>>(seed, start, n, key_mode, nkeys, zipf_cdf,
                                                                       static_cast<wfb_tuple64_t *>(tuples), ts);
    CK(cudaGetLastError());
    return 0;
}

}

#ifdef WFB_BK_TRACE
extern "C" int wfb_debug_bk_trace(unsigned long long *out) { return cudaMemcpyFromSymbol(out, wfb::g_bk_trace, sizeof(unsigned long long) * 1024 * 8) == cudaSuccess ? 0 : -1; }
#endif
```

Measured before the change: 16.26 billion.

## Pack bucket key and position into one list word, process in ranges

The separate sorted slot and position arrays for the bucketed FFAT path are replaced by a single 32-bit list word holding the position in the high bits and the 6-bit local key in the low bits. This halves the scatter writes and the list reads in the bucket update kernel and drops the posA/posB scratch buffers. To keep positions within the word, the window phase and the prebucketed multi-GPU path now loop over ranges of at most 2^26 positions, with extra launches per range (n_trig reset, a results-total adjust, and a windows kernel). It adds launch overhead per range and a size limit on list sorting.

```diff
diff --git a/windflow_b200/csrc/wfb_kernels.cuh b/windflow_b200/csrc/wfb_kernels.cuh
--- a/windflow_b200/csrc/wfb_kernels.cuh
+++ b/windflow_b200/csrc/wfb_kernels.cuh
@@ -987,6 +987,13 @@
 constexpr uint32_t OSW_THREADS = 256, OSW_ITEMS = 16, OSW_TILE = OSW_THREADS * OSW_ITEMS;
 static_assert(OSW_TILE == OSW_TILE_POS, "the tile pass files its digit counts per wide tile");
 constexpr uint32_t OSR_GROUP = 4, OSR_GROUP_POS = OSR_GROUP * OSW_TILE;
+#ifndef WFB_BKL_RANGE_POS
+#define WFB_BKL_RANGE_POS (1u << 26)
+#endif
+constexpr uint32_t BKL_KEY_BITS = 6, BKL_RANGE_POS = WFB_BKL_RANGE_POS;
+static_assert(BKL_RANGE_POS <= (1u << (32 - BKL_KEY_BITS)) && BKL_RANGE_POS >= OSR_GROUP_POS && BKL_RANGE_POS % OSR_GROUP_POS == 0,
+              "a range is whole groups of wide tiles, and its positions fit the list word");
+__device__ __forceinline__ uint32_t bkl_word(uint32_t pos, uint32_t local_key) { return pos << BKL_KEY_BITS | local_key; }
 
 template <class K>
 __global__ void __launch_bounds__(OSW_THREADS) k_wide_tile_hist(const K *__restrict__ keys, const uint32_t *__restrict__ n_ptr, uint32_t n_host,
@@ -1094,8 +1101,8 @@
 
 constexpr uint32_t OSR_SMEM = OSR_GROUP_POS * 2u * 2u + OSW_DIGITS * 8u + OSW_DIGITS * 2u;
 static_assert(OSR_GROUP == 4 && OSR_GROUP_POS <= 0x8000u, "one ushort4 of part sizes per digit; 16-bit packed position compare");
-static __global__ void __launch_bounds__(OSW_THREADS, 3) k_wide_scatter_ranked(const uint32_t *__restrict__ packed, uint32_t *__restrict__ keys_out,
-                                                                            uint32_t *__restrict__ vals_out, uint32_t n, uint32_t shift, uint32_t chunk_shift,
+static __global__ void __launch_bounds__(OSW_THREADS, 3) k_wide_scatter_ranked(const uint32_t *__restrict__ packed, uint32_t *__restrict__ list_out,
+                                                                            uint32_t n, uint32_t shift, uint32_t chunk_shift,
                                                                             uint32_t tiles, const uint16_t *__restrict__ H, const uint32_t *__restrict__ Cx,
                                                                             const uint32_t *__restrict__ T)
 {
@@ -1176,8 +1183,7 @@
         for (; j + 1 < end; j += 2) less += __popc((mm - *reinterpret_cast<const uint32_t *>(lpos + j)) & 0x80008000u);
         if (j < end) less += lpos[j] < mine ? 1u : 0u;
         const uint32_t dst = __ldg(cbase + d) + __ldg(tbase + d) + before + less;
-        keys_out[dst] = slot;
-        vals_out[dst] = start + mine;
+        list_out[dst] = bkl_word(start + mine, slot - (d << shift));
     }
 }
 
@@ -1186,7 +1192,7 @@
 #endif
 template <int RBYTES>
 static __global__ void __launch_bounds__(OSW_THREADS, WFB_OSR_MINBLOCKS) k_wide_scatter_ranked_tile(const uint32_t *__restrict__ packed, uint32_t *__restrict__ keys_out,
-                                                                            uint32_t *__restrict__ vals_out, uint32_t n, uint32_t shift, uint32_t chunk_shift,
+                                                                            uint32_t list, uint32_t n, uint32_t shift, uint32_t chunk_shift,
                                                                             const uint16_t *__restrict__ H, const uint32_t *__restrict__ Cx, const uint32_t *__restrict__ T,
                                                                             const unsigned char *__restrict__ payload_in, unsigned char *__restrict__ payload_out)
 {
@@ -1250,8 +1256,7 @@
         uint32_t less = 0;
         for (uint32_t j = 0; j < cnt; j += 2) less += __popc((mm - cell[j >> 1]) & 0x80008000u);
         const uint32_t dst = bin_base[d] + less;
-        keys_out[dst] = slot;
-        if (RBYTES == 0 || vals_out != nullptr) vals_out[dst] = start + mine;
+        keys_out[dst] = (RBYTES == 0 || list) ? bkl_word(start + mine, slot - (d << shift)) : slot;
         if constexpr (RBYTES != 0) {
             static_assert(RBYTES % 8 == 0, "record size");
             using W = typename std::conditional<RBYTES % 16 == 0, uint4, uint2>::type;
@@ -1279,6 +1284,11 @@
 }
 
 struct MgRuns { uint32_t off[MAX_SHARDS + 1]; };
+__device__ __forceinline__ void mg_clip(uint32_t p0, uint32_t m, uint32_t lo, uint32_t hi, uint32_t *i0, uint32_t *i1)
+{
+    *i0 = min(m, max(p0, lo) - p0);
+    *i1 = min(m, max(p0, hi) - p0);
+}
 constexpr uint32_t MG_THREADS = 256;
 __device__ __forceinline__ uint32_t mg_run_start(const uint32_t *__restrict__ cnt, uint32_t s, uint32_t bps, uint32_t b, uint32_t *sh)
 {
@@ -1297,7 +1307,7 @@
 static __global__ void __launch_bounds__(MG_THREADS) k_mg_count(const uint32_t *__restrict__ cnt, uint32_t nsrc, uint32_t bps, const MgRuns runs,
                                                                 const uint32_t *__restrict__ recv_slots, uint32_t slot_mask, uint32_t shift2, uint32_t nsub,
                                                                 uint32_t *__restrict__ cnt3, uint32_t *__restrict__ run_starts,
-                                                                uint32_t *__restrict__ n_trig, uint32_t *__restrict__ n_heavy)
+                                                                uint32_t *__restrict__ n_trig, uint32_t *__restrict__ n_heavy, uint32_t lo, uint32_t hi)
 {
     __shared__ uint32_t sh[8], c[MAX_SHARDS];
     const uint32_t b = blockIdx.x, s = blockIdx.y, tid = threadIdx.x, lane = tid & 31;
@@ -1306,9 +1316,11 @@
     const uint32_t rs = mg_run_start(cnt, s, bps, b, sh), m = cnt[s * bps + b];
     if (tid == 0) run_starts[s * bps + b] = rs;
     const uint32_t *sl = recv_slots + runs.off[s] + rs;
-    for (uint32_t i0 = 0; i0 < m; i0 += MG_THREADS) {
+    uint32_t ib, ie;
+    mg_clip(runs.off[s] + rs, m, lo, hi, &ib, &ie);
+    for (uint32_t i0 = ib; i0 < ie; i0 += MG_THREADS) {
         const uint32_t i = i0 + tid;
-        const uint32_t j = i < m ? ((sl[i] & slot_mask) >> shift2) & (nsub - 1u) : nsub;
+        const uint32_t j = i < ie ? ((sl[i] & slot_mask) >> shift2) & (nsub - 1u) : nsub;
         for (uint32_t jj = 0; jj < nsub; jj++) { const uint32_t bal = __ballot_sync(FULL, j == jj); if (lane == 0 && bal) atomicAdd(&c[jj], __popc(bal)); }
     }
     __syncthreads();
@@ -1343,27 +1355,29 @@
 static __global__ void __launch_bounds__(MG_THREADS) k_mg_split(const uint32_t *__restrict__ cnt, uint32_t nsrc, uint32_t bps, const MgRuns runs,
                                                                 const uint32_t *__restrict__ recv_slots, uint32_t slot_mask, uint32_t shift2, uint32_t nsub,
                                                                 const uint32_t *__restrict__ off3, const uint32_t *__restrict__ run_starts,
-                                                                uint32_t *__restrict__ out_slots, uint32_t *__restrict__ out_pos)
+                                                                uint32_t *__restrict__ out_list, uint32_t lo, uint32_t hi)
 {
     __shared__ uint32_t wc[MG_THREADS / 32][MAX_SHARDS], fill[MAX_SHARDS];
     const uint32_t b = blockIdx.x, s = blockIdx.y, tid = threadIdx.x, lane = tid & 31, warp = tid >> 5;
     const uint32_t m = cnt[s * bps + b], src0 = runs.off[s] + run_starts[s * bps + b];
+    uint32_t ib, ie;
+    mg_clip(src0, m, lo, hi, &ib, &ie);
     if (tid < nsub) fill[tid] = off3[(b * nsub + tid) * nsrc + s];
     __syncthreads();
-    for (uint32_t i0 = 0; i0 < m; i0 += MG_THREADS) {
+    for (uint32_t i0 = ib; i0 < ie; i0 += MG_THREADS) {
         const uint32_t i = i0 + tid;
         uint32_t slot = 0, j = nsub, before = 0;
-        if (i < m) { slot = recv_slots[src0 + i] & slot_mask; j = (slot >> shift2) & (nsub - 1u); }
+        if (i < ie) { slot = recv_slots[src0 + i] & slot_mask; j = (slot >> shift2) & (nsub - 1u); }
         for (uint32_t jj = 0; jj < nsub; jj++) {
             const uint32_t bal = __ballot_sync(FULL, j == jj);
             if (lane == 0) wc[warp][jj] = __popc(bal);
             if (j == jj) before = __popc(bal & lanemask_lt());
         }
         __syncthreads();
-        if (i < m) {
+        if (i < ie) {
             uint32_t dst = fill[j] + before;
             for (uint32_t w = 0; w < warp; w++) dst += wc[w][j];
-            out_slots[dst] = slot; out_pos[dst] = src0 + i;
+            out_list[dst] = bkl_word(src0 + i - lo, slot & ((1u << shift2) - 1u));
         }
         __syncthreads();
         if (tid < nsub) { uint32_t t = 0; for (uint32_t w = 0; w < MG_THREADS / 32; w++) t += wc[w][tid]; fill[tid] += t; }
@@ -1745,7 +1759,7 @@
 
 template <class P, bool LAZY>
 __global__ void __launch_bounds__(BK_THREADS, LAZY ? WFB_BK_MINBLOCKS_LAZY : WFB_BK_MINBLOCKS) k_ffat_update_buckets(const FfatDev ff, const unsigned char *__restrict__ lifted,
-                                                                       const uint32_t *__restrict__ bk_slots, const uint32_t *__restrict__ bk_pos,
+                                                                       const uint32_t *__restrict__ bk_list, uint32_t pos_base,
                                                                        const uint32_t *__restrict__ digit_counts, uint32_t shift, uint32_t moved,
                                                                        const uint32_t *__restrict__ batch_off, const DevBatch *__restrict__ batches,
                                                                        uint32_t nbatches, unsigned char *__restrict__ out_res,
@@ -1762,11 +1776,11 @@
     constexpr uint32_t CS = NCOL + 2;
     constexpr uint32_t CPB = (RB % 16 == 0) ? 16 : 8;
     constexpr uint32_t BK_SIBL = bk_sibl_levels<RB>();
-    static_assert(DPT % 4 == 0 && BK_KEYS == 64 && BK_THREADS == 128 && RB % 8 == 0, "layout");
+    static_assert(DPT % 4 == 0 && BK_KEYS == 64 && BK_KEYS == (1u << BKL_KEY_BITS) && BK_THREADS == 128 && RB % 8 == 0, "layout");
     static_assert(bk_fits<RB>(), "the arrays below exceed 48 KB of static shared memory (bk_smem_bytes)");
     __shared__ __align__(16) unsigned char s_rec[CAP * RB];
     __shared__ uint32_t s_idx[CAP];
-    __shared__ uint32_t s_lslot[CAP], s_lpos[CAP];
+    __shared__ uint32_t s_list[CAP];
     __shared__ __align__(16) uint16_t s_col[BK_KEYS][CS];
     __shared__ uint32_t kcnt[BK_KEYS], koff[BK_KEYS];
     __shared__ uint32_t kleft[BK_KEYS];
@@ -1828,10 +1842,7 @@
 #pragma unroll
         for (uint32_t r = 0; r < IT; r++) {
             const uint32_t i = r * BK_THREADS + tid;
-            if (at + i < end) {
-                cp_async<4>(s_lslot + i, bk_slots + at + i);
-                if (!moved) cp_async<4>(s_lpos + i, bk_pos + at + i);
-            }
+            if (at + i < end) cp_async<4>(s_list + i, bk_list + at + i);
         }
     };
     fetch_list(bbeg, bend);
@@ -1840,10 +1851,10 @@
 #pragma unroll
         for (uint32_t q = 0; q < BK_CNT_U; q++) {
             const uint32_t i = base + q * BK_THREADS + tid;
-            lk[q] = i < bend ? bk_slots[i] - key_lo : 0xffffffffu;
-        }
-#pragma unroll
-        for (uint32_t q = 0; q < BK_CNT_U; q++) if (lk[q] < kpc) atomicAdd(&kleft[lk[q]], 1u);
+            lk[q] = i < bend ? bk_list[i] & (BK_KEYS - 1u) : BK_KEYS;
+        }
+#pragma unroll
+        for (uint32_t q = 0; q < BK_CNT_U; q++) if (lk[q] < BK_KEYS) atomicAdd(&kleft[lk[q]], 1u);
     }
     __syncthreads();
     if (tid < BK_KEYS) {
@@ -1874,9 +1885,9 @@
             const uint32_t i = r * BK_THREADS + tid;
             ek[r] = BK_KEYS; ep[r] = cursor + i;
             if (i < nsel) {
-                const uint32_t lk = s_lslot[i] - key_lo;
-                if (!moved) ep[r] = s_lpos[i];
-                if (lk < kpc) ek[r] = lk;
+                const uint32_t w = s_list[i];
+                if (!moved) ep[r] = w >> BKL_KEY_BITS;
+                ek[r] = w & (BK_KEYS - 1u);
             }
         }
         {
@@ -2031,7 +2042,7 @@
                         sib_staged = false;
                         if (consumed == tt) {
                             const uint32_t lp = s_idx[koff[k] + consumed - 1];
-                            const uint32_t last_pos = moved ? bk_pos[lp] : lp;
+                            const uint32_t last_pos = pos_base + (moved ? bk_list[lp] >> BKL_KEY_BITS : lp);
                             const uint32_t obase = atomicAdd(n_out, ff.nb);
                             bool deferred = (kleft[k] - consumed) < ff.defer_items;
                             if (deferred) {
@@ -2111,7 +2122,8 @@
                             }
                             __syncwarp();
                             if (tt == 0) {
-                                const uint32_t last_pos = moved ? bk_pos[s_idx[off + j + hi - 1]] : s_idx[off + j + hi - 1];
+                                const uint32_t lp = s_idx[off + j + hi - 1];
+                                const uint32_t last_pos = pos_base + (moved ? bk_list[lp] >> BKL_KEY_BITS : lp);
                                 uint32_t obase = 0;
                                 if (lane == 0) obase = atomicAdd(n_out, ff.nb);
                                 obase = __shfl_sync(FULL, obase, 0);
diff --git a/windflow_b200/csrc/wfb_launch.cuh b/windflow_b200/csrc/wfb_launch.cuh
--- a/windflow_b200/csrc/wfb_launch.cuh
+++ b/windflow_b200/csrc/wfb_launch.cuh
@@ -59,7 +59,7 @@
     int (*ffat_update)(const FfatDev &ff, const unsigned char *lifted, const uint32_t *sorted_pos, const uint32_t *batch_off,
                        const DevBatch *batches, uint32_t nbatches, unsigned char *out_res, uint64_t *out_ts,
                        uint32_t out_cap, uint32_t *n_out, uint32_t grid, cudaStream_t s, const void *params, uint32_t lanes_grid);
-    int (*ffat_buckets)(const FfatDev &ff, const unsigned char *lifted, const uint32_t *bk_slots, const uint32_t *bk_pos,
+    int (*ffat_buckets)(const FfatDev &ff, const unsigned char *lifted, const uint32_t *bk_list, uint32_t pos_base,
                         const uint32_t *digit_counts, uint32_t shift, uint32_t moved, const uint32_t *batch_off, const DevBatch *batches,
                         uint32_t nbatches, unsigned char *out_res, uint64_t *out_ts, uint32_t out_cap, uint32_t *n_out, cudaStream_t s,
                         const void *params);
@@ -170,14 +170,14 @@
 }
 
 template <class P>
-int ffat_buckets_dispatch(const FfatDev &ff, const unsigned char *lifted, const uint32_t *bk_slots, const uint32_t *bk_pos,
+int ffat_buckets_dispatch(const FfatDev &ff, const unsigned char *lifted, const uint32_t *bk_list, uint32_t pos_base,
                           const uint32_t *digit_counts, uint32_t shift, uint32_t moved, const uint32_t *batch_off, const DevBatch *batches,
                           uint32_t nbatches, unsigned char *out_res, uint64_t *out_ts, uint32_t out_cap, uint32_t *n_out, cudaStream_t s,
                           const void *params)
 {
-    if (ff.lazy) k_ffat_update_buckets<P, true><<<OSW_DIGITS, BK_THREADS, 0, s>>>(ff, lifted, bk_slots, bk_pos, digit_counts, shift, moved, batch_off, batches,
+    if (ff.lazy) k_ffat_update_buckets<P, true><<<OSW_DIGITS, BK_THREADS, 0, s>>>(ff, lifted, bk_list, pos_base, digit_counts, shift, moved, batch_off, batches,
                                                                                  nbatches, out_res, out_ts, out_cap, n_out, load_params<P>(params));
-    else k_ffat_update_buckets<P, false><<<OSW_DIGITS, BK_THREADS, 0, s>>>(ff, lifted, bk_slots, bk_pos, digit_counts, shift, moved, batch_off, batches,
+    else k_ffat_update_buckets<P, false><<<OSW_DIGITS, BK_THREADS, 0, s>>>(ff, lifted, bk_list, pos_base, digit_counts, shift, moved, batch_off, batches,
                                                                           nbatches, out_res, out_ts, out_cap, n_out, load_params<P>(params));
     WFB_CK(cudaGetLastError());
     return 0;
diff --git a/windflow_b200/csrc/wfb_lib.cu b/windflow_b200/csrc/wfb_lib.cu
--- a/windflow_b200/csrc/wfb_lib.cu
+++ b/windflow_b200/csrc/wfb_lib.cu
@@ -182,7 +182,7 @@
     int sort_wide(const K *kin, K *kout, uint32_t *vout, const uint32_t *n_ptr, uint32_t n_host, uint32_t cap, uint32_t shift,
                   cudaStream_t s, uint32_t *ready_ctl, const uint32_t **counts, const unsigned char *payload_in = nullptr,
                   unsigned char *payload_out = nullptr, uint32_t payload_bytes = 0, bool skip_invalid = false, uint32_t region_stride = 0, uint32_t few_bins = 0,
-                  const uint16_t *h16_rows = nullptr)
+                  const uint16_t *h16_rows = nullptr, bool list = false)
     {
         if (payload_in && (payload_bytes == 0 || (payload_bytes & 7u))) return WFB_E_BADARG;
         CK(ctl.ensure(CTL_WORDS));
@@ -220,14 +220,14 @@
             }
         }
         if (ranked) {
-            if (sizeof(K) != 4 || !kout || (payload_in ? !payload_out || region_stride : !vout)) return WFB_E_UNSUPPORTED;
+            if (sizeof(K) != 4 || !kout || (payload_in ? !payload_out || region_stride : !list) || (list && n_host > BKL_RANGE_POS)) return WFB_E_UNSUPPORTED;
             if (!payload_in && osr_group(tiles, false) == OSR_GROUP) {
                 CK(osr_smem_attr());
                 k_wide_scatter_ranked<<<(tiles + OSR_GROUP - 1) / OSR_GROUP, OSW_THREADS, OSR_SMEM, s>>>(reinterpret_cast<const uint32_t *>(kin), reinterpret_cast<uint32_t *>(kout),
-                                                                                                       vout, n_host, shift, chunk_shift, tiles, rows, wideC, wideT);
+                                                                                                       n_host, shift, chunk_shift, tiles, rows, wideC, wideT);
             }
-#define WFB_WSRT(RB_) k_wide_scatter_ranked_tile<RB_><<<tiles, OSW_THREADS, 0, s>>>(reinterpret_cast<const uint32_t *>(kin), reinterpret_cast<uint32_t *>(kout), vout, n_host, shift, \
-                                                                                  chunk_shift, rows, wideC, wideT, payload_in, payload_out)
+#define WFB_WSRT(RB_) k_wide_scatter_ranked_tile<RB_><<<tiles, OSW_THREADS, 0, s>>>(reinterpret_cast<const uint32_t *>(kin), reinterpret_cast<uint32_t *>(kout), list ? 1u : 0u, \
+                                                                                  n_host, shift, chunk_shift, rows, wideC, wideT, payload_in, payload_out)
             else if (!payload_in) WFB_WSRT(0);
             else switch (payload_bytes) {
                 case 16: WFB_WSRT(16); break; case 24: WFB_WSRT(24); break; case 32: WFB_WSRT(32); break; case 48: WFB_WSRT(48); break; case 64: WFB_WSRT(64); break;
@@ -1448,7 +1448,8 @@
     const ScratchWaits w = h->s2 ? ScratchWaits(s, h->s2) : ScratchWaits(s);
     CK(g.slotsA.ensure(total, w));
     const size_t cap = g.slotsA.capacity(), RB = h->ops->result_bytes;
-    CK(g.slotsB.ensure(total, w, cap)); CK(g.posA.ensure(total, w, cap)); CK(g.posB.ensure(total, w, cap));
+    CK(g.slotsB.ensure(total, w, cap));
+    if (!h->buckets) { CK(g.posA.ensure(total, w, cap)); CK(g.posB.ensure(total, w, cap)); }
     CK(g.lifted.ensure(RB * total, w, RB * cap));
     if (h->bucket_move) CK(g.lifted_sorted.ensure(RB * total, w, RB * cap));
     const uint32_t trig_cap = ffat_trig_cap(h, static_cast<uint32_t>(cap), h->ff.max_keys);
@@ -1462,6 +1463,8 @@
     return 0;
 }
 
+__global__ void k_results_pre_append(unsigned long long *results_total, const uint32_t *n_out) { if (results_total) *results_total -= *n_out; }
+
 static int ffat_window_phase(wfb_ffat *h, SegScratch &g, const FfatDev &ff, unsigned char *out, uint64_t *out_ts, uint32_t out_cap,
                              uint32_t *n_out, cudaStream_t s)
 {
@@ -1469,18 +1472,33 @@
     const uint64_t before = h->sorter.launches;
     int rc;
     if (h->buckets) {
-        const uint32_t *counts = nullptr;
-        rc = h->sorter.sort_wide<uint32_t>(g.slotsA, g.slotsB, g.posB, nullptr, g.total, g.total, h->bucket_shift, s, g.sort_ctl, &counts,
-                                           h->bucket_move ? static_cast<unsigned char *>(g.lifted) : nullptr,
-                                           h->bucket_move ? static_cast<unsigned char *>(g.lifted_sorted) : nullptr,
-                                           static_cast<uint32_t>(h->ops->result_bytes), true, 0, 0, h->pipelined ? static_cast<uint16_t *>(g.h16) : nullptr);
-        if (rc) return rc;
-        h->launches += h->sorter.launches - before;
-        h->mark(2, s);
-        rc = h->ops->ffat_buckets(ff, h->bucket_move ? g.lifted_sorted : g.lifted_src, g.slotsB, g.posB, counts, h->bucket_shift, h->bucket_move ? 1u : 0u, g.batch_off, g.d_batches, g.nbatches, out, out_ts,
-                                  out_cap, n_out, s, h->pp());
-        if (rc) return rc;
-        h->launches += 1;
+        const size_t RB = h->ops->result_bytes;
+        const uint16_t *rows = h->pipelined ? static_cast<const uint16_t *>(g.h16) : static_cast<const uint16_t *>(h->sorter.wideH);
+        for (uint32_t base = 0; base < g.total; base += BKL_RANGE_POS) {
+            const uint32_t n = std::min(BKL_RANGE_POS, g.total - base);
+            if (base != 0) {
+                CK(cudaMemsetAsync(g.n_trig, 0, sizeof(uint32_t), s));
+                k_results_pre_append<<<1, 1, 0, s>>>(ff.results_total, n_out);
+                CK(cudaGetLastError());
+                h->launches++;
+            }
+            const uint32_t *counts = nullptr;
+            const uint64_t before_r = h->sorter.launches;
+            rc = h->sorter.sort_wide<uint32_t>(g.slotsA + base, g.slotsB, nullptr, nullptr, n, n, h->bucket_shift, s, g.sort_ctl, &counts,
+                                               h->bucket_move ? static_cast<unsigned char *>(g.lifted) + base * RB : nullptr,
+                                               h->bucket_move ? static_cast<unsigned char *>(g.lifted_sorted) : nullptr,
+                                               static_cast<uint32_t>(RB), true, 0, 0, rows + static_cast<size_t>(base / OSW_TILE) * OSW_DIGITS, true);
+            if (rc) return rc;
+            h->launches += h->sorter.launches - before_r;
+            h->mark(2, s);
+            rc = h->ops->ffat_buckets(ff, h->bucket_move ? static_cast<const unsigned char *>(g.lifted_sorted) : g.lifted_src + base * RB, g.slotsB, base, counts,
+                                      h->bucket_shift, h->bucket_move ? 1u : 0u, g.batch_off, g.d_batches, g.nbatches, out, out_ts, out_cap, n_out, s, h->pp());
+            if (rc) return rc;
+            rc = h->ops->ffat_windows(ff, g.batch_off, g.d_batches, g.nbatches, out, out_ts, out_cap, static_cast<uint32_t>(g_num_sms) * 4u, s, h->pp(), n_out);
+            if (rc) return rc;
+            h->launches += 2;
+        }
+        return 0;
     } else {
         rc = h->sorter.sort<uint32_t>(g.slotsA, g.slotsB, g.posA, g.posB, g.n_total, 0, g.total, h->sort_passes, s, &sorted_slots,
                                       &sorted_pos, g.sort_ctl, ff.seg_off, ff.max_keys);
@@ -1676,19 +1694,24 @@
     CK(h->mg_scratch.ensure(3 * OSW_DIGITS * MAX_SHARDS));
     uint32_t *cnt3 = h->mg_scratch, *off3 = cnt3 + OSW_DIGITS * MAX_SHARDS, *run_starts = off3 + OSW_DIGITS * MAX_SHARDS;
     const dim3 grid(bps, nsrc);
-    k_mg_count<<<grid, MG_THREADS, 0, s>>>(bins, nsrc, bps, runs, recv_slots, slot_mask, shift2, nsub, cnt3, run_starts, g.n_trig, g.n_heavy);
-    k_mg_scan<<<1, 1024, 0, s>>>(cnt3, bps * nsub * nsrc, nsrc, off3, g.sort_ctl);
-    k_mg_split<<<grid, MG_THREADS, 0, s>>>(bins, nsrc, bps, runs, recv_slots, slot_mask, shift2, nsub, off3, run_starts, g.slotsB, g.posB);
-    CK(cudaGetLastError());
-    h->mark(2, s);
-    rc = h->ops->ffat_buckets(ff, records, g.slotsB, g.posB, g.sort_ctl, shift2, 0u, g.batch_off, g.d_batches, nsrc, static_cast<unsigned char *>(out_results), out_ts,
-                              out_capacity, n_out_dev, s, h->pp());
-    if (rc) return rc;
-    rc = h->ops->ffat_windows(ff, g.batch_off, g.d_batches, nsrc, static_cast<unsigned char *>(out_results), out_ts, out_capacity, static_cast<uint32_t>(g_num_sms) * 4u, s,
-                              h->pp(), n_out_dev);
-    if (rc) return rc;
+    const uint64_t npos = offs_h[nsrc];
+    for (uint64_t lo = 0; lo < npos; lo += BKL_RANGE_POS) {
+        const uint32_t lo32 = static_cast<uint32_t>(lo), hi32 = static_cast<uint32_t>(std::min<uint64_t>(npos, lo + BKL_RANGE_POS));
+        if (lo != 0) { k_results_pre_append<<<1, 1, 0, s>>>(ff.results_total, n_out_dev); h->launches++; }
+        k_mg_count<<<grid, MG_THREADS, 0, s>>>(bins, nsrc, bps, runs, recv_slots, slot_mask, shift2, nsub, cnt3, run_starts, g.n_trig, g.n_heavy, lo32, hi32);
+        k_mg_scan<<<1, 1024, 0, s>>>(cnt3, bps * nsub * nsrc, nsrc, off3, g.sort_ctl);
+        k_mg_split<<<grid, MG_THREADS, 0, s>>>(bins, nsrc, bps, runs, recv_slots, slot_mask, shift2, nsub, off3, run_starts, g.slotsB, lo32, hi32);
+        CK(cudaGetLastError());
+        h->mark(2, s);
+        rc = h->ops->ffat_buckets(ff, records + lo * h->ops->result_bytes, g.slotsB, lo32, g.sort_ctl, shift2, 0u, g.batch_off, g.d_batches, nsrc,
+                                  static_cast<unsigned char *>(out_results), out_ts, out_capacity, n_out_dev, s, h->pp());
+        if (rc) return rc;
+        rc = h->ops->ffat_windows(ff, g.batch_off, g.d_batches, nsrc, static_cast<unsigned char *>(out_results), out_ts, out_capacity, static_cast<uint32_t>(g_num_sms) * 4u, s,
+                                  h->pp(), n_out_dev);
+        if (rc) return rc;
+        h->launches += 5;
+    }
     h->mark(3, s);
-    h->launches += 5;
     if (h->timing && h->tev_used < wfb_ffat::TEV_MAX) h->tev_used++;
     h->call_no++;
     return 0;
@@ -1798,7 +1821,6 @@
     if (d < nranks) { send_meta[2 * d] = counts[d]; send_meta[2 * d + 1] = watermark; }
 }
 
-__global__ void k_mg_pre_append(unsigned long long *results_total, const uint32_t *n_out) { if (results_total) *results_total -= *n_out; }
 
 struct MgSlot {
     Scratch<unsigned char> regions;
@@ -2248,7 +2270,7 @@
     if (h->trace) CK(cudaEventRecord(sl.tr[2], s));
     uint64_t items = 0;
     for (int p = 0; p < n; p++) items += sl.h_recv[2 * p];
-    if (append && items != 0) { k_mg_pre_append<<<1, 1, 0, s>>>(h->ffat->ff.results_total, n_out_dev); CK(cudaGetLastError()); }
+    if (append && items != 0) { k_results_pre_append<<<1, 1, 0, s>>>(h->ffat->ff.results_total, n_out_dev); CK(cudaGetLastError()); }
     int rc;
     if (h->bucketed) {
         rc = ffat_process_prebucketed(h->ffat, sl.recv, sl.recv_slots, sl.recv_bins, static_cast<uint32_t>(n), h->bps, sl.offs, sl.wms, h->shard_slots - 1u, h->shift,
```

Measured after the change: 17.06 billion, median of 6. 1.05x the previous value.
